# DonsetPG/graph-physics

Hardware: AMD Instinct MI355X
Metric: training steps/sec, CylinderFlow 15-round MGN (batch 16 meshes per step) (higher is better)
Workload: dtype f32; 1 GPU; BASELINE.json configs[1], fp32: 16 x 1885-node CylinderFlow-like meshes per GPU (N=30160, E=180082), 15 rounds, latent 128, random init; global_batch_meshes=16, launch=eager, parallelism=single

## Files before the change

### graph-physics_amd/_capi.py

```python
from __future__ import annotations

import ctypes as C
import os
import subprocess
import threading

_HERE = os.path.dirname(os.path.abspath(__file__))
_CSRC = os.path.join(_HERE, "csrc")
_REPO = os.path.dirname(_HERE)
LIB_PATH = os.environ.get("MGN_LIB") or os.path.join(_CSRC, "libmgn_hip.so")
SOURCES = [os.path.join(_CSRC, "mgn_kernels.hip"), os.path.join(_CSRC, "mgn_prep.hip"), os.path.join(_CSRC, "mgn_attn.hip"),
           os.path.join(_CSRC, "mgn_dense.hip"), os.path.join(_CSRC, "mgn_loss.hip")]
DEPS = [os.path.join(_CSRC, "mgn_x6.inc"), os.path.join(_CSRC, "mgn_fused.inc"), os.path.join(_CSRC, "mgn_pp.inc"), os.path.join(_CSRC, "mgn_ppr.inc")]
HEADER = os.path.join(_REPO, "include", "mgn_hip.h")
DEVICE_FLAGS = ["-Xclang", "-target-feature", "-Xclang", "-packed-fp32-ops"]

MAX_LAYERS = 8
MAX_PHASES = 3
MAX_WGRAD_JOBS = 48

_f32p = C.c_void_p
_i32p = C.c_void_p


class MlpFwdArgs(C.Structure):
    _fields_ = [
        ("M", C.c_int64),
        ("H", C.c_int), ("NL", C.c_int), ("nphase", C.c_int),
        ("src", _f32p * MAX_PHASES),
        ("idx", _i32p * MAX_PHASES),
        ("kw", C.c_int * MAX_PHASES),
        ("W", _f32p * MAX_LAYERS),
        ("b", _f32p * MAX_LAYERS),
        ("scale", _f32p),
        ("eps", C.c_float),
        ("out_w", C.c_int),
        ("resid", _f32p),
        ("out", _f32p),
        ("y_out", _f32p),
        ("saveH", _f32p * MAX_LAYERS),
        ("saveU", _f32p),
        ("saveR", _f32p),
        ("ldw0", C.c_int), ("n_add", C.c_int),
        ("add_src", _f32p * 2), ("add_idx", _i32p * 2),
        ("n_post", C.c_int), ("post_ldw", C.c_int),
        ("post_W", _f32p * 2), ("post_out", _f32p * 2),
        ("wpk", C.c_void_p * 8),
        ("saveM", C.c_void_p * MAX_LAYERS),
        ("precision", C.c_int),
        ("out_relu", C.c_int),
        ("seg_key", C.c_void_p), ("seg_rowptr", C.c_void_p), ("seg_out", _f32p), ("seg_part", _f32p),
        ("act", C.c_int),
        ("saveZ", _f32p * MAX_LAYERS),
        ("add_rows", C.c_int64 * 2),
    ]


class MlpBwdArgs(C.Structure):
    _fields_ = [
        ("M", C.c_int64),
        ("H", C.c_int), ("NL", C.c_int),
        ("dOut", _f32p),
        ("dOut2", _f32p),
        ("idx2", _i32p),
        ("out_w", C.c_int),
        ("U", _f32p), ("R", _f32p), ("scale", _f32p), ("eps", C.c_float),
        ("Hs", _f32p * MAX_LAYERS),
        ("WT", _f32p * MAX_LAYERS),
        ("dZ", _f32p * MAX_LAYERS),
        ("n_din", C.c_int),
        ("WT0", _f32p * MAX_PHASES),
        ("din_resid", _f32p * MAX_PHASES),
        ("dIn", _f32p * MAX_PHASES),
        ("db", _f32p * MAX_LAYERS),
        ("dscale", _f32p),
        ("red_ws", C.c_void_p), ("red_ws_bytes", C.c_size_t),
        ("wpk", C.c_void_p * 8),
        ("Ms", C.c_void_p * MAX_LAYERS),
        ("precision", C.c_int),
        ("n_front", C.c_int),
        ("front_src", _f32p * MAX_PHASES),
        ("front_resid", _f32p),
        ("front_out", _f32p),
        ("defer_reduce", C.c_int),
        ("act", C.c_int),
        ("Zs", _f32p * MAX_LAYERS),
        ("seg_key", C.c_void_p), ("seg_rowptr", C.c_void_p), ("seg_out", _f32p), ("seg_part", _f32p),
        ("dOut2_rows", C.c_int64),
    ]


class ColredJob(C.Structure):
    _fields_ = [("red_ws", C.c_void_p), ("M", C.c_int64), ("H", C.c_int), ("NL", C.c_int), ("out_w", C.c_int), ("n_din", C.c_int),
                ("db", _f32p * MAX_LAYERS), ("dscale", _f32p)]


class WgradJob(C.Structure):
    _fields_ = [
        ("A", _f32p), ("B", _f32p), ("dW", _f32p),
        ("M", C.c_int64),
        ("lda", C.c_int), ("ldb", C.c_int), ("ldw", C.c_int),
        ("nja", C.c_int), ("nkb", C.c_int), ("kw", C.c_int),
        ("db", _f32p),
    ]


class WpackBlock(C.Structure):
    _fields_ = [("src", _f32p), ("dst", C.c_void_p), ("ld_src", C.c_int), ("transpose", C.c_int)]


WPACK_BYTES = 98304


class SimDesc(C.Structure):
    _fields_ = [
        ("N", C.c_int64), ("E", C.c_int64),
        ("x", _f32p), ("x_w", C.c_int),
        ("y", _f32p), ("y_w", C.c_int),
        ("edge_attr", _f32p), ("edge_w", C.c_int),
        ("feat_start", C.c_int), ("feat_end", C.c_int), ("out_start", C.c_int), ("out_w", C.c_int), ("type_idx", C.c_int),
        ("acc_sum", _f32p * 3), ("acc_sumsq", _f32p * 3), ("acc_count", _f32p * 3), ("num_acc", _f32p * 3),
        ("accumulate", C.c_int * 3),
        ("std_eps", C.c_float),
        ("node_out", _f32p), ("target_out", _f32p), ("edge_out", _f32p),
        ("norm_w", C.c_int * 3),
        ("max_accumulations", C.c_float),
        ("type_err", C.c_void_p),
    ]


class EdgeBwdFusedArgs(C.Structure):
    _fields_ = [
        ("M", C.c_int64), ("dOut", _f32p), ("dAgg", _f32p), ("idx", C.c_void_p), ("U", _f32p), ("R", _f32p), ("scale", _f32p),
        ("eps", C.c_float), ("X", _f32p * 4), ("Ms", C.c_void_p * 3), ("wpk", C.c_void_p * 4), ("dIn", _f32p), ("dZ0", _f32p),
        ("dW", _f32p * 4), ("ldw", C.c_int * 4), ("db", _f32p * 4), ("dscale", _f32p), ("ws", C.c_void_p), ("ws_bytes", C.c_size_t),
        ("precision", C.c_int),
    ]


class LinearArgs(C.Structure):
    _fields_ = [
        ("M", C.c_int64), ("x", _f32p), ("ldx", C.c_int), ("K1", C.c_int), ("x2", _f32p), ("ldx2", C.c_int), ("K2", C.c_int),
        ("x3", _f32p), ("ldx3", C.c_int), ("K3", C.c_int), ("idx", C.c_void_p), ("idx2", C.c_void_p), ("idx3", C.c_void_p),
        ("norm_scale", _f32p), ("eps", C.c_float), ("inv_out", _f32p), ("n_out", _f32p), ("W", _f32p), ("ldw", C.c_int), ("b", _f32p),
        ("W2", _f32p), ("b2", _f32p), ("act", C.c_int), ("N", C.c_int), ("resid", _f32p), ("ldr", C.c_int), ("out", _f32p),
        ("ldo", C.c_int), ("saveZ1", _f32p), ("saveZ2", _f32p), ("precision", C.c_int), ("w_transposed", C.c_int),
        ("gb_z1", _f32p), ("gb_z2", _f32p), ("out2", _f32p), ("norm_scale_outer", _f32p), ("inv_outer_out", _f32p), ("z16", C.c_int), ("x16", C.c_int), ("out16", C.c_int),
    ]


class RownormPhase(C.Structure):
    _fields_ = [("x", _f32p), ("ldx", C.c_int), ("K", C.c_int), ("idx", C.c_void_p), ("dx", _f32p), ("lddx", C.c_int), ("acc", _f32p)]


class OptTensor(C.Structure):
    _fields_ = [("p", _f32p), ("g", _f32p), ("m", _f32p), ("v", _f32p), ("n", C.c_int64)]


class TBlock(C.Structure):
    _fields_ = [("src", _f32p), ("dst", _f32p), ("ld_src", C.c_int), ("ld_dst", C.c_int)]


MAX_LOSS_TERMS = 8


class LossArgs(C.Structure):
    _fields_ = [
        ("N", C.c_int64), ("O", C.c_int), ("F", C.c_int), ("DX", C.c_int), ("method", C.c_int),
        ("net_out", _f32p), ("ld_out", C.c_int), ("target", _f32p), ("ld_tgt", C.c_int),
        ("u_out", _f32p), ("u_tgt", _f32p), ("type", _f32p), ("ldty", C.c_int),
        ("types", C.c_float * 4), ("ntypes", C.c_int),
        ("nterms", C.c_int), ("term_type", C.c_int * MAX_LOSS_TERMS), ("term_weight", C.c_float * MAX_LOSS_TERMS),
        ("rowptr", C.c_void_p), ("col", _i32p), ("coef", _f32p), ("inv", _f32p),
        ("M", C.c_int64), ("K", C.c_int), ("elems", _i32p), ("cv", _f32p), ("nptr", C.c_void_p), ("nent", _i32p),
        ("ge_out", _f32p), ("ge_tgt", _f32p),
        ("g_out", _f32p), ("a_out", _f32p), ("bu_out", _f32p), ("b_out", _f32p), ("part", _f32p),
        ("terms", _f32p), ("total", _f32p), ("invcount", _f32p),
    ]


SYMBOLS = {
    "mgn_version": (C.c_int, []),
    "mgn_last_error": (C.c_char_p, []),
    "mgn_csr_workspace_bytes": (C.c_size_t, [C.c_int64, C.c_int64]),
    "mgn_csr_build": (C.c_int, [C.c_void_p, C.c_int64, C.c_int64, C.c_void_p, C.c_void_p, C.c_void_p, C.c_size_t, C.c_void_p]),
    "mgn_topology_workspace_bytes": (C.c_size_t, [C.c_int64, C.c_int64]),
    "mgn_topology_build": (C.c_int, [C.c_void_p, C.c_void_p, C.c_int64, C.c_int64] + [C.c_void_p] * 6 + [C.POINTER(C.c_int32), C.c_void_p,
                                     C.c_size_t, C.c_void_p]),
    "mgn_topology_build_async": (C.c_int, [C.c_void_p, C.c_void_p, C.c_int64, C.c_int64] + [C.c_void_p] * 6 + [C.c_void_p, C.c_void_p,
                                           C.c_size_t, C.c_void_p]),
    "mgn_segsum": (C.c_int, [C.c_void_p, C.c_void_p, C.c_void_p, C.c_void_p, C.c_int64, C.c_int, C.c_void_p]),
# ... 186 lines not shown
```

### graph-physics_amd/csrc/mgn_kernels.hip

```cpp
#include <hip/hip_runtime.h>
#include <stdint.h>
#include <stdlib.h>
#include <type_traits>
#include "mgn_hip.h"

typedef float f32x4 __attribute__((ext_vector_type(4)));

#define MFMA16(a, b, c) __builtin_amdgcn_mfma_f32_16x16x4f32((a), (b), (c), 0, 0, 0)

typedef __attribute__((address_space(1))) const f32x4 g_cf32x4;
typedef __attribute__((address_space(1))) f32x4 g_f32x4;
typedef __attribute__((address_space(1))) const float g_cfloat;
typedef __attribute__((address_space(1))) float g_float;
#ifdef MGN_EXP_NOLOAD
__device__ __forceinline__ f32x4 ld4(const float* p) { return f32x4{1.f, 2.f, (float)(size_t)p, 0.5f}; }
#else
__device__ __forceinline__ f32x4 ld4(const float* p) { return *(g_cf32x4*)p; }
#endif
#ifdef MGN_EXP_NOSTORE
__device__ __forceinline__ void st4(float* p, f32x4 v) { if (v[0] != v[0]) *(g_f32x4*)p = v; }
#else
__device__ __forceinline__ void st4(float* p, f32x4 v) { *(g_f32x4*)p = v; }
#endif
#ifdef MGN_EXP_NOSTORE
// ... 1631 lines not shown
      }
    if (g == 0) *(f32x4*)(dst + H * H + 4 * c) = cs;
  };
  if (wv > 0) put(red[wv - 1]);
  __syncthreads();
  if (wv == 0) {
#pragma unroll
    for (int w = 0; w < 3; ++w) {
#pragma unroll
      for (int qa = 0; qa < 4; ++qa)
#pragma unroll
        for (int v = 0; v < 4; ++v) {
          const f32x4 o = *(const f32x4*)(red[w] + (16 * g + 4 * v + qa) * H + 4 * c);
#pragma unroll
          for (int qb = 0; qb < 4; ++qb) acc[qa][qb][v] += o[qb];
        }
      cs += *(const f32x4*)(red[w] + H * H + 4 * c);
    }
    float* P = L.partial + (size_t)pidx * (H * H + H);
#pragma unroll
    for (int qa = 0; qa < 4; ++qa)
#pragma unroll
      for (int v = 0; v < 4; ++v) {
        const f32x4 o = {acc[qa][0][v], acc[qa][1][v], acc[qa][2][v], acc[qa][3][v]};
        st4(P + (16 * g + 4 * v + qa) * H + 4 * c, o);
      }
    if (g == 0 && J.db != nullptr) st4(P + H * H + 4 * c, cs);
  }
}


template <int WRED_GROUPS>
__global__ void __launch_bounds__(64 * WRED_GROUPS) k_wgrad_red(const WgradLaunch L) {
  __shared__ float red[WRED_GROUPS][64];
  const int H = L.H;
  const size_t st = (size_t)H * H + H;
  const int j = blockIdx.y;
  const mgn_wgrad_job J = L.job[j];
  const int rows = 16 * J.nja, cols = 16 * J.nkb;
  const int i = blockIdx.x * 64 + (threadIdx.x & 63);
  const int pl = threadIdx.x >> 6;
  const int nwg = L.wg0[j + 1] - L.wg0[j];
  const float* P0 = L.partial + (size_t)L.wg0[j] * st;
  const bool is_w = i < rows * cols;
  const bool is_b = !is_w && i < rows * cols + rows && J.db != nullptr;
  int r = 0, k = 0;
  float s0 = 0.f, s1 = 0.f, s2 = 0.f, s3 = 0.f;
  if (is_w || is_b) {
    const float* P;
    if (is_w) {
      r = i / cols;
      k = i % cols;
      P = P0 + r * H + k;
    } else {
      r = i - rows * cols;
      P = P0 + (size_t)H * H + r;
    }
    int b = pl;
    for (; b + 3 * WRED_GROUPS < nwg; b += 4 * WRED_GROUPS) {
      s0 += P[(size_t)b * st];
      s1 += P[(size_t)(b + WRED_GROUPS) * st];
      s2 += P[(size_t)(b + 2 * WRED_GROUPS) * st];
      s3 += P[(size_t)(b + 3 * WRED_GROUPS) * st];
    }
    if (b < nwg) s0 += P[(size_t)b * st];
    if (b + WRED_GROUPS < nwg) s1 += P[(size_t)(b + WRED_GROUPS) * st];
    if (b + 2 * WRED_GROUPS < nwg) s2 += P[(size_t)(b + 2 * WRED_GROUPS) * st];
  }
  red[pl][threadIdx.x & 63] = (s0 + s1) + (s2 + s3);
  __syncthreads();
  if (pl == 0) {
    float v = 0.f;
#pragma unroll
    for (int q = 0; q < WRED_GROUPS; q += 4)
      v += (red[q][threadIdx.x] + red[q + 1][threadIdx.x]) + (red[q + 2][threadIdx.x] + red[q + 3][threadIdx.x]);
    if (is_w) {
      if (k < J.ldw) J.dW[(size_t)r * J.ldw + k] = v;
    } else if (is_b) {
      J.db[r] = v;
    }
  }
}

template <int HB>
__global__ void __launch_bounds__(256) k_segsum(const float* __restrict__ src, const int32_t* __restrict__ rowptr,
                                                const int32_t* __restrict__ perm, float* __restrict__ out, long N) {
  constexpr int H = 16 * HB;
  constexpr int LPR = H / 4;
  const long node = ((long)blockIdx.x * 256 + threadIdx.x) / LPR;
  const int l = threadIdx.x % LPR;
  if (node >= N) return;
  const int beg = rowptr[node], end = rowptr[node + 1];
  f32x4 s = {0.f, 0.f, 0.f, 0.f};
  const float* base = src + 4 * l;
  for (int k = beg; k < end; k += 8) {
    f32x4 v[8];
#pragma unroll
    for (int u = 0; u < 8; ++u) {
      const int kk = k + u;
      if (kk < end) {
        const long row = perm ? (long)perm[kk] : (long)kk;
        v[u] = ld4(base + row * H);
      } else {
        v[u] = f32x4{0.f, 0.f, 0.f, 0.f};
      }
    }
#pragma unroll
    for (int u = 0; u < 8; ++u)
      if (k + u < end) s += v[u];
  }
  st4(out + node * H + 4 * l, s);
}

template <int HB, bool SRC16 = false>
__global__ void __launch_bounds__(256) k_segsum2(const float* __restrict__ src, const int32_t* __restrict__ rowptr0,
                                                 const int32_t* __restrict__ perm0, float* __restrict__ out0,
                                                 const int32_t* __restrict__ rowptr1, const int32_t* __restrict__ perm1,
                                                 float* __restrict__ out1, long N, unsigned half) {
  constexpr int H = 16 * HB;
  constexpr int LPR = H / 4;
  const bool second = blockIdx.x >= half;
  const int32_t* rowptr = second ? rowptr1 : rowptr0;
  const int32_t* perm = second ? perm1 : perm0;
  float* out = second ? out1 : out0;
  const long node = ((long)(blockIdx.x - (second ? half : 0)) * 256 + threadIdx.x) / LPR;
  const int l = threadIdx.x % LPR;
  if (node >= N) return;
  const int beg = rowptr[node], end = rowptr[node + 1];
  f32x4 s = {0.f, 0.f, 0.f, 0.f};
  const float* base = src + 4 * l;
  for (int k = beg; k < end; k += 8) {
    f32x4 v[8];
#pragma unroll
    for (int u = 0; u < 8; ++u) {
      const int kk = k + u;
      if (kk < end) {
        const long row = perm ? (long)perm[kk] : (long)kk;
        if constexpr (SRC16) {
          const uint2 t = *(const uint2*)((const uint16_t*)src + row * H + 32 * (l >> 3) + 8 * (l & 3) + 4 * ((l >> 2) & 1));
          v[u] = f32x4{__builtin_bit_cast(float, t.x << 16), __builtin_bit_cast(float, t.x & 0xffff0000u),
                       __builtin_bit_cast(float, t.y << 16), __builtin_bit_cast(float, t.y & 0xffff0000u)};
        } else {
          v[u] = ld4(base + row * H);
        }
      } else {
        v[u] = f32x4{0.f, 0.f, 0.f, 0.f};
      }
    }
#pragma unroll
    for (int u = 0; u < 8; ++u)
      if (k + u < end) s += v[u];
  }
  st4(out + node * H + 4 * l, s);
}

__global__ void __launch_bounds__(256) k_seg_fix(const int32_t* __restrict__ rowptr, const float* __restrict__ part,
                                                 float* __restrict__ out, long N) {
  constexpr int H = 128, LPR = 32;
  const long node = ((long)blockIdx.x * 256 + threadIdx.x) / LPR;
  const int l = threadIdx.x % LPR;
  if (node >= N) return;
  const int b = rowptr[node], e = rowptr[node + 1];
  f32x4 s = {0.f, 0.f, 0.f, 0.f};
  if (b < e) {
    const int t0 = b >> 4, t1 = (e - 1) >> 4;
    if (t0 == t1) return;
// ... 55 lines not shown
    if (i < N) rowptr[i] = carry + woff + x - v;
    __syncthreads();
    if (tid == 1023) carry_s = carry + woff + x;
    __syncthreads();
  }
  if (tid == 0) rowptr[N] = carry_s;
}

__global__ void k_csr_fill(const int64_t* __restrict__ key, long E, long N, const int32_t* __restrict__ rowptr,
                           int* __restrict__ cursor, int32_t* __restrict__ perm) {
  const long e = (long)blockIdx.x * blockDim.x + threadIdx.x;
  if (e >= E) return;
  const int64_t k = key[e];
  if (k < 0 || k >= N) return;
  const int pos = atomicAdd(&cursor[k], 1);
  perm[rowptr[k] + pos] = (int32_t)e;
}

#define CSR_SMALL_SEG 48
__global__ void k_csr_sortseg(const int32_t* __restrict__ rowptr, long N, int32_t* __restrict__ perm,
                              int* __restrict__ worklist, int* __restrict__ nbig) {
  const long i = (long)blockIdx.x * blockDim.x + threadIdx.x;
  if (i >= N) return;
  const int beg = rowptr[i], end = rowptr[i + 1];
  if (end - beg > CSR_SMALL_SEG) {
    worklist[atomicAdd(nbig, 1)] = (int)i;
    return;
  }
  for (int a = beg + 1; a < end; ++a) {
    const int v = perm[a];
    int b = a - 1;
    while (b >= beg && perm[b] > v) {
      perm[b + 1] = perm[b];
      --b;
    }
    perm[b + 1] = v;
  }
}

__global__ void __launch_bounds__(256) k_csr_sortbig(const int32_t* __restrict__ rowptr, int32_t* __restrict__ perm,
                                                     const int* __restrict__ worklist, const int* __restrict__ nbig,
                                                     int32_t* __restrict__ tmp) {
  const int n = *nbig;
  for (int w = blockIdx.x; w < n; w += gridDim.x) {
    const int node = worklist[w];
    const int beg = rowptr[node], d = rowptr[node + 1] - beg;
    for (int i = threadIdx.x; i < d; i += 256) tmp[beg + i] = perm[beg + i];
    __syncthreads();
    for (int i = threadIdx.x; i < d; i += 256) {
      const int v = tmp[beg + i];
      int rank = 0;
      for (int j = 0; j < d; ++j) rank += (tmp[beg + j] < v) ? 1 : 0;
      perm[beg + rank] = v;
    }
    __syncthreads();
  }
}

static thread_local char g_err[256] = "";
static int fail(int code, const char* msg) {
  snprintf(g_err, sizeof(g_err), "%s", msg);
  return code;
}
static int check_launch(const char* what) {
  hipError_t e = hipGetLastError();
  if (e != hipSuccess) {
    snprintf(g_err, sizeof(g_err), "%s: %s", what, hipGetErrorString(e));
    return 2;
  }
  return 0;
}
static int pick_mt(int64_t M) {
  if (M >= (int64_t)64 * 2048) return 2;
  return 1;
}

struct MlpPlan {
  bool lds;
  int mt;
  unsigned grid;
  size_t smem;
};

static bool fwd_ragged(const mgn_mlp_fwd_args& a) {
  bool r = (a.out_w != a.H);
  for (int p = 0; p < a.nphase; ++p) r = r || (a.kw[p] != a.H);
  return r;
}

static MlpPlan plan_mlp(int64_t M, int H, int NL, bool ragged, bool bwd, int act = MGN_ACT_RELU) {
  MlpPlan p;
  p.lds = (H == 128) && !ragged && NL >= (bwd ? 2 : 1) && NL <= LDS_MAX_NL;
  if (getenv("MGN_NO_LDS") != nullptr) p.lds = false;
  if (act == MGN_ACT_GELU) p.lds = false;
  p.mt = (M >= (int64_t)64 * 2048) ? 2 : 1;
  if (p.lds) p.mt = 1;
  if (const char* e = getenv("MGN_MT")) p.mt = (atoi(e) == 2) ? 2 : 1;
  const int rows = 64 * p.mt;
  p.grid = (unsigned)((M + rows - 1) / rows);
  if (p.lds && p.grid > 512) p.grid = 512;
  if (const char* e = getenv("MGN_GRID")) { if (p.lds && !bwd && atoi(e) > 0 && (unsigned)atoi(e) < p.grid) p.grid = (unsigned)atoi(e); }
  p.smem = p.lds ? (bwd ? (size_t)2 * WBUF_BYTES + 512 + (size_t)4 * (NL + 1) * H * sizeof(float) : (size_t)FWD_LDS_BYTES) : 0;
  return p;
}

template <typename K>
static int set_smem(K kern, size_t bytes) {
  static thread_local const void* done[16];
  static thread_local int ndone = 0;
  for (int i = 0; i < ndone; ++i)
    if (done[i] == (const void*)kern) return 0;
  if (hipFuncSetAttribute((const void*)kern, hipFuncAttributeMaxDynamicSharedMemorySize, (int)(2 * WBUF_BYTES + 4 * 7 * 128 * 4)) != hipSuccess) return 1;
  (void)bytes;
  if (ndone < 16) done[ndone++] = (const void*)kern;
  return 0;
}

static bool fwd_x6(const mgn_mlp_fwd_args& a) {
  if (a.wpk[0] == nullptr || getenv("MGN_FP32_MFMA") != nullptr) return false;
  const int G = a.nphase + a.NL - 1 + a.n_post;
  if (G > X6_MAX_UNITS || a.NL > LDS_MAX_NL) return false;
  if (a.n_add > 0 && (a.nphase != 1 || (a.NL == 1 && a.resid != nullptr))) return false;
  if (a.seg_out != nullptr && (a.seg_key == nullptr || a.seg_rowptr == nullptr || a.seg_part == nullptr || a.n_post > 0)) return false;
  for (int u = 0; u < G; ++u)
    if (a.wpk[u] == nullptr) return false;
  return true;
}
template <int TERMS, int NW, int ACT, class SH = ShDyn>
static int set_fwd_x6_attr() {
  return hipFuncSetAttribute((const void*)k_mlp_fwd_x6<TERMS, NW, ACT, SH>, hipFuncAttributeMaxDynamicSharedMemorySize, X6_FWD_LDS_BYTES(NW)) != hipSuccess;
}
static int fwd_static_shape(const mgn_mlp_fwd_args& a) {
  const char* env = getenv("MGN_X6_STATIC");
  const int mode = env != nullptr ? atoi(env) : 1;
  if (mode == 0 || a.act != MGN_ACT_RELU || a.NL != 4 || a.resid == nullptr || a.scale == nullptr) return 0;
  if (a.nphase == 1 && a.n_add == 2 && a.n_post == 0 && a.idx[0] == nullptr && a.add_idx[0] != nullptr && a.add_idx[1] != nullptr &&
      a.seg_out != nullptr && a.seg_key == a.add_idx[0])
    return 1;
  if (mode != 2 && a.nphase == 2 && a.n_add == 0 && a.idx[0] == nullptr && a.idx[1] == nullptr && a.seg_out == nullptr && a.M >= 4 * 512 * 64) {
    if (a.n_post == 2) return 2;
    if (a.n_post == 0) return 3;
  }
  return 0;
}

static bool fwd_pp_ok(const mgn_mlp_fwd_args& a) {
  const char* env = getenv("MGN_PP");
  const int mode = (env == nullptr) ? -1 : atoi(env);
  if (mode == 0) return false;
  const int64_t min_rows = (mode == 2) ? 1 : 2 * 128 * 256;
  if (a.precision != 0 || a.y_out != nullptr || a.M < min_rows || a.M * 512 >= (int64_t)1 << 32) return false;
  for (int u = 1; u < 4; ++u)
    if ((const char*)a.wpk[u] != (const char*)a.wpk[0] + (size_t)u * MGN_WPACK_BYTES) return false;
  const bool all = a.saveU && a.saveR && a.saveH[0] && a.saveH[1] && a.saveH[2] && a.saveM[0] && a.saveM[1] && a.saveM[2];
  const bool none = !a.saveU && !a.saveR && !a.saveH[0] && !a.saveH[1] && !a.saveH[2] && !a.saveM[0] && !a.saveM[1] && !a.saveM[2];
  if (mode < 0 && !none) return false;
  return (all || none) && a.resid != nullptr && a.scale != nullptr && a.out != a.resid && a.out != a.src[0];
}

static bool fwd_ppr_ok(const mgn_mlp_fwd_args& a) {
  const char* env = getenv("MGN_PPR");
  const int mode = (env == nullptr) ? 1 : atoi(env);
  if (mode == 0) return false;
  const int64_t min_rows = (mode == 2) ? 1 : 65536;
  if (a.precision != 0 || a.y_out != nullptr || a.M < min_rows || a.M * 512 >= (int64_t)1 << 32) return false;
  for (int q = 0; q < 2; ++q)
    if (a.add_rows[q] <= 0 || a.add_rows[q] * 512 >= (int64_t)1 << 32) return false;
  for (int u = 1; u < 4; ++u)
    if ((const char*)a.wpk[u] != (const char*)a.wpk[0] + (size_t)u * MGN_WPACK_BYTES) return false;
  const bool all = a.saveU && a.saveR && a.saveH[0] && a.saveH[1] && a.saveH[2] && a.saveM[0] && a.saveM[1] && a.saveM[2];
  const bool none = !a.saveU && !a.saveR && !a.saveH[0] && !a.saveH[1] && !a.saveH[2] && !a.saveM[0] && !a.saveM[1] && !a.saveM[2];
  return (all || none) && a.resid != nullptr && a.scale != nullptr && a.out != a.resid && a.out != a.src[0];
}

template <int HB>
static int launch_fwd(const mgn_mlp_fwd_args& a, hipStream_t s) {
  const bool ragged = fwd_ragged(a);
  const MlpPlan p = plan_mlp(a.M, a.H, a.NL, ragged, false, a.act);
  if (p.lds && fwd_x6(a)) {
    int nw = (a.M >= 128 * 256) ? X6_FWD_NW_LARGE : 4;
    bool nw6 = false;
    if (const char* e = getenv("MGN_NW")) {
      nw = (atoi(e) == 8) ? 8 : 4;
      nw6 = atoi(e) == 6;
    }
    if (a.seg_out != nullptr) nw = 4;
    const bool silu = (a.act == MGN_ACT_SILU);
    if (silu) nw = 4;
    static thread_local bool attr_done = false;
    if (!attr_done) {
      if (set_fwd_x6_attr<6, 4, 0>() || set_fwd_x6_attr<1, 4, 0>() || set_fwd_x6_attr<6, 8, 0>() || set_fwd_x6_attr<1, 8, 0>() ||
          set_fwd_x6_attr<6, 4, 1>() || set_fwd_x6_attr<1, 4, 1>() || set_fwd_x6_attr<6, 4, 0, ShEdge>() ||
          set_fwd_x6_attr<6, 4, 0, ShNode<2>>() || set_fwd_x6_attr<6, 4, 0, ShNode<0>>() || set_fwd_x6_attr<1, 4, 0, ShEdge>() ||
          set_fwd_x6_attr<1, 4, 0, ShNode<2>>() || set_fwd_x6_attr<1, 4, 0, ShNode<0>>() || set_fwd_x6_attr<6, 6, 0, ShEdge>())
        return 1;
      attr_done = true;
    }
    const int rows = 16 * nw;
    unsigned grid = (unsigned)((a.M + rows - 1) / rows);
    const unsigned cap = (nw == 8) ? 256u : 512u;
    if (grid > cap) grid = cap;
    if (const char* e = getenv("MGN_GRID")) {
      if (atoi(e) > 0 && (unsigned)atoi(e) < grid) grid = (unsigned)atoi(e);
    }
    const int shape = (nw == 4 && !silu) ? fwd_static_shape(a) : 0;
    if (shape == 1 && !nw6 && fwd_ppr_ok(a)) {
      static thread_local bool ppr_attr = false;
      if (!ppr_attr) {
        if (hipFuncSetAttribute((const void*)k_edge_fwd_ppr<true, true>, hipFuncAttributeMaxDynamicSharedMemorySize, PPR_LDS_BYTES) != hipSuccess ||
            hipFuncSetAttribute((const void*)k_edge_fwd_ppr<false, true>, hipFuncAttributeMaxDynamicSharedMemorySize, PPR_LDS_BYTES) != hipSuccess ||
            hipFuncSetAttribute((const void*)k_edge_fwd_ppr<true, false>, hipFuncAttributeMaxDynamicSharedMemorySize, PPR_LDS_BYTES) != hipSuccess ||
            hipFuncSetAttribute((const void*)k_edge_fwd_ppr<false, false>, hipFuncAttributeMaxDynamicSharedMemorySize, PPR_LDS_BYTES) != hipSuccess)
          return 1;
        ppr_attr = true;
      }
      const int64_t ngroups = ((a.M + 15) / 16 + PPR_R - 1) / PPR_R;
      unsigned gp = (ngroups < 256) ? (unsigned)ngroups : 256u;
      const char* ex = getenv("MGN_PPR_XCD");
      const bool xcd = ex == nullptr || atoi(ex) != 0;
      if (a.saveU != nullptr) {
        if (xcd) hipLaunchKernelGGL((k_edge_fwd_ppr<true, true>), dim3(gp), dim3(512), PPR_LDS_BYTES, s, a);
        else hipLaunchKernelGGL((k_edge_fwd_ppr<true, false>), dim3(gp), dim3(512), PPR_LDS_BYTES, s, a);
      } else {
        if (xcd) hipLaunchKernelGGL((k_edge_fwd_ppr<false, true>), dim3(gp), dim3(512), PPR_LDS_BYTES, s, a);
        else hipLaunchKernelGGL((k_edge_fwd_ppr<false, false>), dim3(gp), dim3(512), PPR_LDS_BYTES, s, a);
      }
      return 0;
    }
    if (shape == 1 && !nw6 && fwd_pp_ok(a)) {
      static thread_local bool pp_attr = false;
      if (!pp_attr) {
        if (hipFuncSetAttribute((const void*)k_edge_fwd_pp<true>, hipFuncAttributeMaxDynamicSharedMemorySize, PP_LDS_BYTES) != hipSuccess ||
            hipFuncSetAttribute((const void*)k_edge_fwd_pp<false>, hipFuncAttributeMaxDynamicSharedMemorySize, PP_LDS_BYTES) != hipSuccess)
          return 1;
        pp_attr = true;
      }
      unsigned gp = (unsigned)((a.M + 127) / 128);
      if (gp > 256u) gp = 256u;
      if (a.saveU != nullptr)
        hipLaunchKernelGGL((k_edge_fwd_pp<true>), dim3(gp), dim3(512), PP_LDS_BYTES, s, a);
      else
        hipLaunchKernelGGL((k_edge_fwd_pp<false>), dim3(gp), dim3(512), PP_LDS_BYTES, s, a);
      return 0;
    }
    if (shape == 1 && nw6 && a.precision == 0) {
      unsigned g6 = (unsigned)((a.M + 95) / 96);
      if (g6 > 512u) g6 = 512u;
      hipLaunchKernelGGL((k_mlp_fwd_x6<6, 6, 0, ShEdge>), dim3(g6), dim3(384), X6_FWD_LDS_BYTES(6), s, a);
    } else if (shape == 1) {
      if (a.precision >= 1)
        hipLaunchKernelGGL((k_mlp_fwd_x6<1, 4, 0, ShEdge>), dim3(grid), dim3(256), X6_FWD_LDS_BYTES(4), s, a);
      else
        hipLaunchKernelGGL((k_mlp_fwd_x6<6, 4, 0, ShEdge>), dim3(grid), dim3(256), X6_FWD_LDS_BYTES(4), s, a);
    } else if (shape == 2) {
      if (a.precision >= 1)
        hipLaunchKernelGGL((k_mlp_fwd_x6<1, 4, 0, ShNode<2>>), dim3(grid), dim3(256), X6_FWD_LDS_BYTES(4), s, a);
      else
        hipLaunchKernelGGL((k_mlp_fwd_x6<6, 4, 0, ShNode<2>>), dim3(grid), dim3(256), X6_FWD_LDS_BYTES(4), s, a);
    } else if (shape == 3) {
      if (a.precision >= 1)
        hipLaunchKernelGGL((k_mlp_fwd_x6<1, 4, 0, ShNode<0>>), dim3(grid), dim3(256), X6_FWD_LDS_BYTES(4), s, a);
      else
        hipLaunchKernelGGL((k_mlp_fwd_x6<6, 4, 0, ShNode<0>>), dim3(grid), dim3(256), X6_FWD_LDS_BYTES(4), s, a);
    } else if (silu) {
      if (a.precision >= 1)
        hipLaunchKernelGGL((k_mlp_fwd_x6<1, 4, 1>), dim3(grid), dim3(256), X6_FWD_LDS_BYTES(4), s, a);
      else
        hipLaunchKernelGGL((k_mlp_fwd_x6<6, 4, 1>), dim3(grid), dim3(256), X6_FWD_LDS_BYTES(4), s, a);
    } else if (nw == 8) {
      if (a.precision >= 1)
        hipLaunchKernelGGL((k_mlp_fwd_x6<1, 8, 0>), dim3(grid), dim3(512), X6_FWD_LDS_BYTES(8), s, a);
      else
        hipLaunchKernelGGL((k_mlp_fwd_x6<6, 8, 0>), dim3(grid), dim3(512), X6_FWD_LDS_BYTES(8), s, a);
    } else {
      if (a.precision >= 1)
        hipLaunchKernelGGL((k_mlp_fwd_x6<1, 4, 0>), dim3(grid), dim3(256), X6_FWD_LDS_BYTES(4), s, a);
      else
        hipLaunchKernelGGL((k_mlp_fwd_x6<6, 4, 0>), dim3(grid), dim3(256), X6_FWD_LDS_BYTES(4), s, a);
    }
    return 0;
  }
  if (p.lds) {
    if (p.mt == 2) {
      if (set_smem(k_mlp_fwd_lds<2>, p.smem)) return 1;
      hipLaunchKernelGGL((k_mlp_fwd_lds<2>), dim3(p.grid), dim3(256), p.smem, s, a);
    } else {
      if (set_smem(k_mlp_fwd_lds<1>, p.smem)) return 1;
      hipLaunchKernelGGL((k_mlp_fwd_lds<1>), dim3(p.grid), dim3(256), p.smem, s, a);
    }
    return 0;
  }
  if (ragged) {
    if (p.mt == 2)
      hipLaunchKernelGGL((k_mlp_fwd<HB, 2, true>), dim3(p.grid), dim3(256), 0, s, a);
    else
      hipLaunchKernelGGL((k_mlp_fwd<HB, 1, true>), dim3(p.grid), dim3(256), 0, s, a);
  } else {
    if (p.mt == 2)
      hipLaunchKernelGGL((k_mlp_fwd<HB, 2, false>), dim3(p.grid), dim3(256), 0, s, a);
    else
      hipLaunchKernelGGL((k_mlp_fwd<HB, 1, false>), dim3(p.grid), dim3(256), 0, s, a);
  }
  return 0;
}

static bool bwd_x6(const mgn_mlp_bwd_args& a) {
  if (a.wpk[0] == nullptr || getenv("MGN_FP32_MFMA") != nullptr) return false;
  const int G = a.n_front + a.NL - 1 + a.n_din;
  if (G > 8 || G < 1 || a.n_front < 0 || a.n_front > MGN_MAX_PHASES) return false;
  if (a.n_front > 0 && a.dOut2 != nullptr) return false;
  for (int u = 0; u < G; ++u)
    if (a.wpk[u] == nullptr) return false;
  if (a.seg_out != nullptr && (a.seg_key == nullptr || a.seg_rowptr == nullptr || a.seg_part == nullptr || a.dZ[0] == nullptr ||
                               a.n_front > 0 || a.act != MGN_ACT_RELU || a.precision != 0 || a.NL < 2))
    return false;
  if (a.act == MGN_ACT_SILU) {
    if (a.n_front > 0 || (a.n_din == 0 && a.dOut2 != nullptr)) return false;
    for (int l = 1; l < a.NL; ++l)
      if (a.Zs[l - 1] == nullptr) return false;
    return true;
  }
  for (int l = 1; l < a.NL; ++l)
    if (a.Ms[l - 1] == nullptr) return false;
  return true;
}

static bool bwd_ppr_ok(const mgn_mlp_bwd_args& a) {
  const char* env = getenv("MGN_PPR");
  const int mode = (env == nullptr) ? 1 : atoi(env);
  const char* eb = getenv("MGN_PPR_BWD");
  if (mode == 0 || (eb != nullptr && atoi(eb) == 0)) return false;
  const int64_t min_rows = (mode == 2) ? 1 : 65536;
  if (a.precision != 0 || a.M < min_rows || a.M * 512 >= (int64_t)1 << 32 || a.dscale == nullptr) return false;
  if (a.dOut2_rows <= 0 || a.dOut2_rows * 512 >= (int64_t)1 << 32) return false;
  for (int u = 1; u < 4; ++u)
    if ((const char*)a.wpk[u] != (const char*)a.wpk[0] + (size_t)u * MGN_WPACK_BYTES) return false;
  for (int l = 0; l < 4; ++l)
    if (a.db[l] != nullptr || a.dZ[l] == nullptr) return false;
  if (a.dIn[0] == nullptr || a.Ms[0] == nullptr || a.Ms[1] == nullptr || a.Ms[2] == nullptr) return false;
  const void* ins[4] = {a.dOut, a.U, a.din_resid[0], a.dOut2};
  const void* outs[5] = {a.dZ[0], a.dZ[1], a.dZ[2], a.dZ[3], a.dIn[0]};
  for (const void* o : outs)
    for (const void* i : ins)
      if (o == i) return false;
  return true;
}

template <int HB>
static int launch_bwd(const mgn_mlp_bwd_args& a, hipStream_t s) {
  MlpPlan p = plan_mlp(a.M, a.H, a.NL, a.out_w != a.H || a.n_din > 1, true, a.act);
  if (p.lds && bwd_x6(a)) {
    static thread_local bool attr_done = false;
    if (!attr_done) {
      const int lds = X6_BWD_LDS_BYTES(LDS_MAX_NL + 1);
      if (hipFuncSetAttribute((const void*)k_mlp_bwd_x6<6, false, 0>, hipFuncAttributeMaxDynamicSharedMemorySize, lds) != hipSuccess ||
          hipFuncSetAttribute((const void*)k_mlp_bwd_x6<1, false, 0>, hipFuncAttributeMaxDynamicSharedMemorySize, lds) != hipSuccess ||
          hipFuncSetAttribute((const void*)k_mlp_bwd_x6<6, true, 0>, hipFuncAttributeMaxDynamicSharedMemorySize, lds) != hipSuccess ||
          hipFuncSetAttribute((const void*)k_mlp_bwd_x6<1, true, 0>, hipFuncAttributeMaxDynamicSharedMemorySize, lds) != hipSuccess ||
          hipFuncSetAttribute((const void*)k_mlp_bwd_x6<6, false, 1>, hipFuncAttributeMaxDynamicSharedMemorySize, lds) != hipSuccess ||
          hipFuncSetAttribute((const void*)k_mlp_bwd_x6<1, false, 1>, hipFuncAttributeMaxDynamicSharedMemorySize, lds) != hipSuccess ||
          hipFuncSetAttribute((const void*)k_mlp_bwd_x6<6, false, 0, true>, hipFuncAttributeMaxDynamicSharedMemorySize, lds) != hipSuccess ||
          hipFuncSetAttribute((const void*)k_mlp_bwd_x6<6, false, 0, false, SbEdge>, hipFuncAttributeMaxDynamicSharedMemorySize, lds) != hipSuccess ||
          hipFuncSetAttribute((const void*)k_mlp_bwd_x6<1, false, 0, false, SbEdge>, hipFuncAttributeMaxDynamicSharedMemorySize, lds) != hipSuccess)
        return 1;
      attr_done = true;
    }
    int nused = (a.scale != nullptr && a.dscale != nullptr) ? 1 : 0;
    for (int l = 0; l < a.NL; ++l) nused += (a.db[l] != nullptr) ? 1 : 0;
    const size_t lds = X6_BWD_LDS_BYTES(nused);
    const bool front = a.n_front > 0;
    const char* st_env = getenv("MGN_X6_STATIC");
    const bool static_off = st_env != nullptr && atoi(st_env) == 0;
    const bool sb_edge = !static_off && !front && a.seg_out == nullptr && a.act == MGN_ACT_RELU && a.NL == 4 &&
                         a.n_din == 1 && a.din_resid[0] != nullptr && a.scale != nullptr && a.R != nullptr && a.U != nullptr &&
                         a.dOut2 != nullptr && a.idx2 != nullptr;
    if (sb_edge && bwd_ppr_ok(a)) {
      static thread_local bool ppr_attr = false;
      if (!ppr_attr) {
        if (hipFuncSetAttribute((const void*)k_edge_bwd_ppr<true>, hipFuncAttributeMaxDynamicSharedMemorySize, PPB_LDS_BYTES) != hipSuccess ||
            hipFuncSetAttribute((const void*)k_edge_bwd_ppr<false>, hipFuncAttributeMaxDynamicSharedMemorySize, PPB_LDS_BYTES) != hipSuccess)
          return 1;
        ppr_attr = true;
      }
      const int64_t ngroups = ((a.M + 15) / 16 + PPR_R - 1) / PPR_R;
      unsigned gp = (ngroups < 256) ? (unsigned)ngroups : 256u;
      if (gp > p.grid) gp = p.grid;
      const char* ex = getenv("MGN_PPR_XCD");
      if (ex == nullptr || atoi(ex) != 0)
        hipLaunchKernelGGL((k_edge_bwd_ppr<true>), dim3(gp), dim3(512), PPB_LDS_BYTES, s, a, (int)p.grid);
      else
        hipLaunchKernelGGL((k_edge_bwd_ppr<false>), dim3(gp), dim3(512), PPB_LDS_BYTES, s, a, (int)p.grid);
    } else if (sb_edge) {
      if (a.precision >= 1)
        hipLaunchKernelGGL((k_mlp_bwd_x6<1, false, 0, false, SbEdge>), dim3(p.grid), dim3(256), lds, s, a);
      else
        hipLaunchKernelGGL((k_mlp_bwd_x6<6, false, 0, false, SbEdge>), dim3(p.grid), dim3(256), lds, s, a);
    } else if (a.seg_out != nullptr) {
      hipLaunchKernelGGL((k_mlp_bwd_x6<6, false, 0, true>), dim3(p.grid), dim3(256), lds, s, a);
    } else if (a.act == MGN_ACT_SILU) {
      if (a.precision >= 1)
        hipLaunchKernelGGL((k_mlp_bwd_x6<1, false, 1>), dim3(p.grid), dim3(256), lds, s, a);
      else
        hipLaunchKernelGGL((k_mlp_bwd_x6<6, false, 1>), dim3(p.grid), dim3(256), lds, s, a);
    } else if (a.precision >= 1) {
      if (front)
        hipLaunchKernelGGL((k_mlp_bwd_x6<1, true, 0>), dim3(p.grid), dim3(256), lds, s, a);
      else
        hipLaunchKernelGGL((k_mlp_bwd_x6<1, false, 0>), dim3(p.grid), dim3(256), lds, s, a);
    } else {
      if (front)
        hipLaunchKernelGGL((k_mlp_bwd_x6<6, true, 0>), dim3(p.grid), dim3(256), lds, s, a);
      else
        hipLaunchKernelGGL((k_mlp_bwd_x6<6, false, 0>), dim3(p.grid), dim3(256), lds, s, a);
    }
    return 0;
  }
  if (p.lds) {
    if (p.mt == 2) {
      if (set_smem(k_mlp_bwd_lds<2>, p.smem)) return 1;
      hipLaunchKernelGGL((k_mlp_bwd_lds<2>), dim3(p.grid), dim3(256), p.smem, s, a);
    } else {
      if (set_smem(k_mlp_bwd_lds<1>, p.smem)) return 1;
      hipLaunchKernelGGL((k_mlp_bwd_lds<1>), dim3(p.grid), dim3(256), p.smem, s, a);
    }
    return 0;
  }
  if (a.out_w != a.H) {
    if (p.mt == 2)
      hipLaunchKernelGGL((k_mlp_bwd<HB, 2, true>), dim3(p.grid), dim3(256), 0, s, a);
    else
      hipLaunchKernelGGL((k_mlp_bwd<HB, 1, true>), dim3(p.grid), dim3(256), 0, s, a);
  } else {
    if (p.mt == 2)
      hipLaunchKernelGGL((k_mlp_bwd<HB, 2, false>), dim3(p.grid), dim3(256), 0, s, a);
    else
      hipLaunchKernelGGL((k_mlp_bwd<HB, 1, false>), dim3(p.grid), dim3(256), 0, s, a);
  }
  return 0;
}

extern "C" {

int mgn_version(void) { return 136; }
const char* mgn_last_error(void) { return g_err; }

size_t mgn_csr_workspace_bytes(int64_t E, int64_t N) {
  return (size_t)(2 * N + E + 32) * sizeof(int);
}

static int csr_enqueue(const int64_t* key, int64_t E, int64_t N, int32_t* rowptr, int32_t* perm, void* ws, int* err_dev, hipStream_t s) {
  int* cnt = (int*)ws;
  if (hipMemsetAsync(ws, 0, (size_t)(N + 16) * sizeof(int), s) != hipSuccess) return fail(2, "mgn_csr_build: memset");
// ... 167 lines not shown
  return check_launch("mgn_seg_fix");
}

int mgn_segsum2(const float* src, const int32_t* rowptr0, const int32_t* perm0, float* out0, const int32_t* rowptr1,
                const int32_t* perm1, float* out1, int64_t N, int H, void* stream) {
  hipStream_t s = (hipStream_t)stream;
  if (N == 0) return 0;
  if (H != 128) return fail(1, "mgn_segsum2: H must be 128");
  const unsigned half = (unsigned)((N * (H / 4) + 255) / 256);
  hipLaunchKernelGGL(k_segsum2<8>, dim3(2 * half), dim3(256), 0, s, src, rowptr0, perm0, out0, rowptr1, perm1, out1, (long)N, half);
  return check_launch("mgn_segsum2");
}

int mgn_segsum2_b16(const uint16_t* src, const int32_t* rowptr0, const int32_t* perm0, float* out0, const int32_t* rowptr1,
                    const int32_t* perm1, float* out1, int64_t N, int H, void* stream) {
  hipStream_t s = (hipStream_t)stream;
  if (N == 0) return 0;
  if (H != 128) return fail(1, "mgn_segsum2_b16: H must be 128");
  const unsigned half = (unsigned)((N * (H / 4) + 255) / 256);
  hipLaunchKernelGGL((k_segsum2<8, true>), dim3(2 * half), dim3(256), 0, s, (const float*)src, rowptr0, perm0, out0, rowptr1, perm1, out1,
                     (long)N, half);
  return check_launch("mgn_segsum2_b16");
}

static int check_mlp_common(int H, int NL, int out_w, const char* who) {
  if (!(H == 16 || H == 32 || H == 64 || H == 128)) return fail(1, "H must be 16, 32, 64 or 128");
  if (NL < 1 || NL > MGN_MAX_LAYERS) return fail(1, "NL out of range");
  if (out_w < 1 || out_w > H) return fail(1, "out_w out of range");
  (void)who;
  return 0;
}


int mgn_mlp_fwd(const mgn_mlp_fwd_args* args, void* stream) {
  const mgn_mlp_fwd_args& a = *args;
  if (int rc = check_mlp_common(a.H, a.NL, a.out_w, "mgn_mlp_fwd")) return rc;
  if (a.precision < 0 || a.precision > 2) return fail(1, "mgn_mlp_fwd: precision must be 0 (fp32-grade), 1 (bf16) or 2 (bf16, two-byte saves)");
  if (a.precision == 2 && (!fwd_x6(a) || !plan_mlp(a.M, a.H, a.NL, fwd_ragged(a), false, a.act).lds || a.act != MGN_ACT_RELU))
    return fail(1, "mgn_mlp_fwd: precision 2 (two-byte saves) needs the packed split-bf16 path (H = 128, wpk[]) and ReLU");
  if (a.seg_out != nullptr && !(plan_mlp(a.M, a.H, a.NL, fwd_ragged(a), false).lds && fwd_x6(a)))
    return fail(1, "mgn_mlp_fwd: the fused segment sum needs the packed split-bf16 path (and seg_key / seg_rowptr / seg_part, no post-products)");
  if (a.out_relu && (a.scale != nullptr || a.resid != nullptr || a.wpk[0] != nullptr ||
                     plan_mlp(a.M, a.H, a.NL, fwd_ragged(a), false).lds))
    return fail(1, "mgn_mlp_fwd: out_relu is for a plain ragged-input launch (no norm / residual / packed path)");
  if (a.act != MGN_ACT_RELU && a.act != MGN_ACT_SILU && a.act != MGN_ACT_GELU) return fail(1, "mgn_mlp_fwd: act must be MGN_ACT_RELU, _SILU or _GELU");
  if (a.act == MGN_ACT_GELU && (a.wpk[0] != nullptr || a.precision != 0 || a.seg_out != nullptr || a.n_add > 0 || a.n_post > 0 || a.ldw0 > 0))
    return fail(1, "mgn_mlp_fwd: GELU runs on the generic kernels only (no packed weights / gathers / post-products)");
  if (a.act == MGN_ACT_SILU && plan_mlp(a.M, a.H, a.NL, fwd_ragged(a), false).lds && !fwd_x6(a) && a.NL > 1)
    return fail(1, "mgn_mlp_fwd: SiLU is not available on the exact-fp32 LDS generation (pass packed weights)");
  if (a.precision >= 1 && plan_mlp(a.M, a.H, a.NL, fwd_ragged(a), false, a.act).lds && !fwd_x6(a))
    return fail(1, "mgn_mlp_fwd: at H = 128 with full widths the bf16 matrix mode needs the packed split-bf16 path (wpk); other shapes run it on the generic kernels");
  if (a.nphase < 1 || a.nphase > MGN_MAX_PHASES) return fail(1, "mgn_mlp_fwd: nphase out of range");
  for (int p = 0; p < a.nphase; ++p)
    if (a.kw[p] < 1 || a.kw[p] > a.H) return fail(1, "mgn_mlp_fwd: phase width out of range");
  if (a.scale != nullptr && a.out_w != a.H) return fail(1, "mgn_mlp_fwd: RMSNorm needs out_w == H");
  if (a.n_add < 0 || a.n_add > 2 || a.n_post < 0 || a.n_post > 2) return fail(1, "mgn_mlp_fwd: n_add / n_post out of range");
  if ((a.n_add > 0 || a.n_post > 0 || a.ldw0 > 0) && !plan_mlp(a.M, a.H, a.NL, fwd_ragged(a), false).lds)
    return fail(1, "mgn_mlp_fwd: ldw0 / n_add / n_post need the H = 128 full-width kernel");
  if (a.M == 0) return 0;
  hipStream_t s = (hipStream_t)stream;
  int rc;
  switch (a.H) {
    case 128: rc = launch_fwd<8>(a, s); break;
    case 64: rc = launch_fwd<4>(a, s); break;
    case 32: rc = launch_fwd<2>(a, s); break;
    default: rc = launch_fwd<1>(a, s); break;
  }
  if (rc) return fail(2, "mgn_mlp_fwd: cannot reserve LDS");
  return check_launch("mgn_mlp_fwd");
}


size_t mgn_mlp_bwd_workspace_bytes(int64_t M, int H, int NL) {
  return (size_t)((M + 63) / 64 + 1) * (NL + 1) * H * sizeof(float);
}


int mgn_mlp_bwd(const mgn_mlp_bwd_args* args, void* stream) {
  const mgn_mlp_bwd_args& a = *args;
  if (int rc = check_mlp_common(a.H, a.NL, a.out_w, "mgn_mlp_bwd")) return rc;
  if (a.n_din < 0 || a.n_din > MGN_MAX_PHASES) return fail(1, "mgn_mlp_bwd: n_din out of range");
  if (a.n_din > 1 && a.dZ[0] == nullptr) return fail(1, "mgn_mlp_bwd: n_din > 1 needs dZ[0]");
  if (a.precision < 0 || a.precision > 3) return fail(1, "mgn_mlp_bwd: precision must be 0 (fp32-grade), 1 (bf16), 2 (bf16, two-byte dZ[1..]) or 3 (dZ[0] too)");
  if (a.precision >= 2 && (!bwd_x6(a) || !plan_mlp(a.M, a.H, a.NL, a.out_w != a.H || a.n_din > 1, true).lds || a.act != MGN_ACT_RELU || a.n_front != 0))
    return fail(1, "mgn_mlp_bwd: precision 2 (two-byte dZ rows) needs the packed split-bf16 path (H = 128, wpk, Ms), ReLU and no front stage");
  if (a.act != MGN_ACT_RELU && a.act != MGN_ACT_SILU && a.act != MGN_ACT_GELU) return fail(1, "mgn_mlp_bwd: act must be MGN_ACT_RELU, _SILU or _GELU");
  if (a.act == MGN_ACT_GELU && (a.wpk[0] != nullptr || a.precision != 0 || a.seg_out != nullptr || a.n_front != 0))
    return fail(1, "mgn_mlp_bwd: GELU runs on the generic kernels only");
  if (a.act != MGN_ACT_RELU) {
    for (int l = 1; l < a.NL; ++l)
      if (a.Zs[l - 1] == nullptr) return fail(1, "mgn_mlp_bwd: SiLU / GELU need the saved pre-activations Zs[]");
  }
  if (a.act == MGN_ACT_SILU) {
    if (plan_mlp(a.M, a.H, a.NL, a.out_w != a.H || a.n_din > 1, true).lds && !bwd_x6(a))
      return fail(1, "mgn_mlp_bwd: SiLU is not available on the exact-fp32 LDS generation (pass packed weights)");
  }
  if (a.n_front != 0 && !(plan_mlp(a.M, a.H, a.NL, a.out_w != a.H || a.n_din > 1, true).lds && bwd_x6(a)))
    return fail(1, "mgn_mlp_bwd: the front stage needs the packed split-bf16 path (H = 128, full widths, wpk, Ms, no dOut2)");
  if (a.precision >= 1 && plan_mlp(a.M, a.H, a.NL, a.out_w != a.H || a.n_din > 1, true, a.act).lds && !bwd_x6(a))
    return fail(1, "mgn_mlp_bwd: at H = 128 with full widths the bf16 matrix mode needs the packed split-bf16 path (wpk, Ms); other shapes run it on the generic kernels");
  if (a.seg_out != nullptr && !(plan_mlp(a.M, a.H, a.NL, a.out_w != a.H || a.n_din > 1, true).lds && bwd_x6(a)))
    return fail(1, "mgn_mlp_bwd: the fused segment sum of dZ[0] needs the packed split-bf16 path (fp32-grade, ReLU, dZ[0], no front stage)");
  if (a.M == 0) return 0;
  if (a.red_ws_bytes < mgn_mlp_bwd_workspace_bytes(a.M, a.H, a.NL)) return fail(1, "mgn_mlp_bwd: workspace too small");
  hipStream_t s = (hipStream_t)stream;
  int lrc;
  switch (a.H) {
    case 128: lrc = launch_bwd<8>(a, s); break;
    case 64: lrc = launch_bwd<4>(a, s); break;
    case 32: lrc = launch_bwd<2>(a, s); break;
    default: lrc = launch_bwd<1>(a, s); break;
  }
  if (lrc) return fail(2, "mgn_mlp_bwd: cannot reserve LDS");
  if (int rc = check_launch("mgn_mlp_bwd")) return rc;
  const unsigned grid = plan_mlp(a.M, a.H, a.NL, a.out_w != a.H || a.n_din > 1, true, a.act).grid;
  const int nslot = a.NL + 1;
  ColredOuts outs;
  bool any = false;
  for (int l = 0; l <= MGN_MAX_LAYERS; ++l) outs.o[l] = nullptr;
  for (int l = 0; l < a.NL; ++l) {
    outs.o[l] = a.db[l];
    any |= a.db[l] != nullptr;
  }
  outs.o[a.NL] = (a.scale != nullptr) ? a.dscale : nullptr;
  any |= outs.o[a.NL] != nullptr;
  if (!any || a.defer_reduce) return 0;
  const int n = nslot * a.H;
  hipLaunchKernelGGL(k_colred, dim3((n + 31) / 32), dim3(1024), 0, s, (const float*)a.red_ws, (int)grid, nslot, a.H, outs);
  return check_launch("mgn_mlp_bwd/colred");
}

int mgn_colred_batch(int n, const mgn_colred_job* jobs, void* stream) {
  if (n < 0) return fail(1, "mgn_colred_batch: bad arguments");
  hipStream_t s = (hipStream_t)stream;
  for (int i0 = 0; i0 < n; i0 += CR_MAX) {
    ColredBatch B;
    const int m = (n - i0 < CR_MAX) ? n - i0 : CR_MAX;
    int maxcol = 0;
    for (int i = 0; i < m; ++i) {
      const mgn_colred_job& q = jobs[i0 + i];
      if (q.red_ws == nullptr || q.NL < 1 || q.NL > MGN_MAX_LAYERS) return fail(1, "mgn_colred_batch: bad job");
      ColredJob& J = B.j[i];
      J.ws = (const float*)q.red_ws;
      J.nblocks = (int)plan_mlp(q.M, q.H, q.NL, q.out_w != q.H || q.n_din > 1, true).grid;
      J.nslot = q.NL + 1;
      J.H = q.H;
      for (int l = 0; l <= MGN_MAX_LAYERS; ++l) J.outs.o[l] = nullptr;
      for (int l = 0; l < q.NL; ++l) J.outs.o[l] = q.db[l];
      J.outs.o[q.NL] = q.dscale;
      if (J.nslot * J.H > maxcol) maxcol = J.nslot * J.H;
    }
    hipLaunchKernelGGL(k_colred_batch, dim3((maxcol + 31) / 32, m), dim3(1024), 0, s, B);
  }
  return check_launch("mgn_colred_batch");
}

static bool wgrad_job_row64(const mgn_wgrad_job& j) {
  return j.nja <= 4 && j.nkb <= 4 && j.kw <= 64 && (j.kw & 3) == 0 && (j.lda & 3) == 0 && (j.ldb & 3) == 0 &&
         (((uintptr_t)j.A | (uintptr_t)j.B) & 15) == 0;
}
static int wgrad_plan(int njobs, const mgn_wgrad_job* jobs, int* wg0, bool lds, int lds_budget = 512) {
  const int rows = lds ? WG_TILE_ROWS : 16;
  int budget = lds ? lds_budget : 512;
  if (!lds) {
    if (const char* e = getenv("MGN_WGRAD_GENERIC_BUDGET")) {
      const int b = atoi(e);
      if (b >= 64 && b <= 1024) budget = b;
    }
  }
  int64_t tiles[MGN_MAX_WGRAD_JOBS], tot = 0;
  int n[MGN_MAX_WGRAD_JOBS];
  for (int j = 0; j < njobs; ++j) {
    tiles[j] = (jobs[j].M + rows - 1) / rows;
    if (tiles[j] < 1) tiles[j] = 1;
    tot += tiles[j];
  }
  int used = 0;
  for (int j = 0; j < njobs; ++j) {
    int64_t s = tiles[j] * budget / tot;
    const int64_t cap = (tiles[j] + 3) / 4;
    if (s > cap) s = cap;
    if (s < 1) s = 1;
    n[j] = (int)s;
    used += n[j];
  }
  while (used < budget) {
    int best = -1;
    double load = 4.0;
    for (int j = 0; j < njobs; ++j) {
      const double l = (double)tiles[j] / n[j];
      if (l > load) {
        load = l;
        best = j;
      }
    }
    if (best < 0) break;
    ++n[best];
    ++used;
  }
  int acc = 0;
  for (int j = 0; j < njobs; ++j) {
    wg0[j] = acc;
    acc += n[j];
  }
  wg0[njobs] = acc;
  return acc;
}

size_t mgn_wgrad_workspace_bytes(int njobs, const mgn_wgrad_job* jobs) {
  if (njobs < 1 || njobs > MGN_MAX_WGRAD_JOBS) return 0;
  return (size_t)(512 + 1024 + 2 * MGN_MAX_WGRAD_JOBS) * (128 * 128 + 128) * sizeof(float);
}

static bool wgrad_job_full(const mgn_wgrad_job& j) {
  return j.nja == 8 && j.nkb == 8 && (j.lda == 128 || j.lda == -128) && (j.ldb == 128 || j.ldb == -128) && j.kw == 128 && j.M >= 1 && getenv("MGN_NO_LDS") == nullptr;
}

int mgn_wgrad(int njobs, const mgn_wgrad_job* jobs, void* ws, size_t ws_bytes, void* stream) {
  return mgn_wgrad_p(njobs, jobs, ws, ws_bytes, 0, stream);
}

int mgn_wgrad_p(int njobs, const mgn_wgrad_job* jobs, void* ws, size_t ws_bytes, int precision, void* stream) {
  if (precision != 0 && precision != 1) return fail(1, "mgn_wgrad: precision must be 0 (fp32-grade) or 1 (bf16)");
  if (njobs < 1 || njobs > MGN_MAX_WGRAD_JOBS) return fail(1, "mgn_wgrad: njobs out of range");
  for (int j = 0; j < njobs; ++j) {
    if (jobs[j].lda < 0 || jobs[j].ldb < 0) {
      const bool r64 = !wgrad_job_full(jobs[j]) && wgrad_job_row64(jobs[j]) && getenv("MGN_WGRAD_NO_ROW64") == nullptr &&
                       ((((uintptr_t)jobs[j].A | (uintptr_t)jobs[j].B) & 15) == 0);
      if (precision != 1 || !(wgrad_job_full(jobs[j]) || r64) || getenv("MGN_FP32_MFMA") != nullptr)
        return fail(1, "mgn_wgrad: a negative leading dimension (bf16 rows) needs precision 1 and a full 128 x 128 job with ld = -128 or a job of the row-vector kernel");
    }
  }
  hipStream_t s = (hipStream_t)stream;
  size_t ws_off = 0;
  for (int pass = 0; pass < 2; ++pass) {
    WgradLaunch L;
    L.njobs = 0;
    int maxb = 1;
    for (int j = 0; j < njobs; ++j) {
      if (jobs[j].nja < 1 || jobs[j].nkb < 1 || jobs[j].nja > 8 || jobs[j].nkb > 8) return fail(1, "mgn_wgrad: block counts out of range");
      if (wgrad_job_full(jobs[j]) != (pass == 0)) continue;
      L.job[L.njobs++] = jobs[j];
      if (jobs[j].nja > maxb) maxb = jobs[j].nja;
      if (jobs[j].nkb > maxb) maxb = jobs[j].nkb;
    }
    if (L.njobs == 0) continue;
    int HB = maxb <= 1 ? 1 : maxb <= 2 ? 2 : maxb <= 4 ? 4 : 8;
    bool row64 = pass == 1 && HB <= 4 && getenv("MGN_WGRAD_NO_ROW64") == nullptr;
    for (int j = 0; row64 && j < L.njobs; ++j) row64 = wgrad_job_row64(L.job[j]);
    if (row64) HB = 4;
    if (!row64 && pass == 1)
      for (int j = 0; j < L.njobs; ++j)
        if (L.job[j].lda < 0 || L.job[j].ldb < 0) return fail(1, "mgn_wgrad: bf16-row jobs below 128 x 128 need every job of the launch on the row-vector kernel");
    L.H = 16 * HB;
    bool pc = pass == 0 && precision == 0 && getenv("MGN_FP32_MFMA") == nullptr;
    if (pc) {
      const char* e = getenv("MGN_WGRAD_PC");
      pc = e == nullptr || atoi(e) != 0;
      for (int j = 0; pc && j < L.njobs; ++j) pc = L.job[j].lda == 128 && L.job[j].ldb == 128;
    }
    int total = wgrad_plan(L.njobs, L.job, L.wg0, pass == 0, pc ? 256 : 512);
    L.interleave = 0;
    if (row64 && L.njobs >= 2 && L.njobs <= 8 && getenv("MGN_WGRAD_NO_INTERLEAVE") == nullptr) {
      bool same = true;
      for (int j = 1; j < L.njobs; ++j) same = same && L.job[j].M == L.job[0].M;
      const int64_t tiles = (L.job[0].M + 15) / 16;
      int per = (512 / L.njobs) & ~7;
      while (per > 8 && (int64_t)per * 4 > tiles) per -= 8;
      if (same && per >= 8 && tiles >= 4 * per) {
        for (int j = 0; j <= L.njobs; ++j) L.wg0[j] = j * per;
        L.interleave = per;
        total = L.njobs * per;
      }
    }
    const size_t need = (size_t)total * (L.H * L.H + L.H) * sizeof(float);
    if (ws_bytes < ws_off + need) return fail(1, "mgn_wgrad: workspace too small");
    L.partial = (float*)((char*)ws + ws_off);
    ws_off += need;
    if (pc) {
      static thread_local bool attr_pc_done = false;
      if (!attr_pc_done) {
        if (hipFuncSetAttribute((const void*)k_wgrad_pc, hipFuncAttributeMaxDynamicSharedMemorySize, WPC_LDS_BYTES) != hipSuccess)
          return fail(2, "mgn_wgrad: cannot reserve LDS");
        attr_pc_done = true;
      }
      hipLaunchKernelGGL(k_wgrad_pc, dim3(total), dim3(512), WPC_LDS_BYTES, s, L);
    } else if (pass == 0) {
      const size_t smem = 4 * WG_TILE_BYTES;
      static thread_local bool attr_done = false;
      if (!attr_done) {
        if (hipFuncSetAttribute((const void*)k_wgrad_lds, hipFuncAttributeMaxDynamicSharedMemorySize, (int)smem) != hipSuccess)
          return fail(2, "mgn_wgrad: cannot reserve LDS");
        attr_done = true;
      }
      if (getenv("MGN_FP32_MFMA") == nullptr) {
        static thread_local bool attr6_done = false;
        if (!attr6_done) {
          if (hipFuncSetAttribute((const void*)k_wgrad_x6<6>, hipFuncAttributeMaxDynamicSharedMemorySize, (int)smem) != hipSuccess ||
              hipFuncSetAttribute((const void*)k_wgrad_x6<1>, hipFuncAttributeMaxDynamicSharedMemorySize, (int)smem) != hipSuccess)
            return fail(2, "mgn_wgrad: cannot reserve LDS");
          attr6_done = true;
        }
        if (precision == 1)
          hipLaunchKernelGGL(k_wgrad_x6<1>, dim3(total), dim3(256), smem, s, L);
        else
          hipLaunchKernelGGL(k_wgrad_x6<6>, dim3(total), dim3(256), smem, s, L);
      } else {
        hipLaunchKernelGGL(k_wgrad_lds, dim3(total), dim3(256), smem, s, L);
      }
    } else if (row64) {
      if (precision == 1) {
        const bool a16 = L.job[0].lda < 0, b16 = L.job[0].ldb < 0;
        for (int j = 1; j < L.njobs; ++j)
          if ((L.job[j].lda < 0) != a16 || (L.job[j].ldb < 0) != b16) return fail(1, "mgn_wgrad: the jobs of a row-vector launch must agree on which operand is bf16 rows");
        if (a16 && b16) hipLaunchKernelGGL((k_wgrad_row64<true, true, true>), dim3(total), dim3(256), 0, s, L);
        else if (a16) hipLaunchKernelGGL((k_wgrad_row64<true, true, false>), dim3(total), dim3(256), 0, s, L);
        else if (b16) hipLaunchKernelGGL((k_wgrad_row64<true, false, true>), dim3(total), dim3(256), 0, s, L);
        else hipLaunchKernelGGL((k_wgrad_row64<true>), dim3(total), dim3(256), 0, s, L);
      }
      else if (getenv("MGN_FP32_MFMA") == nullptr && getenv("MGN_WGRAD_ROW64_EXACT") == nullptr) {
        bool full = true;
        for (int j = 0; full && j < L.njobs; ++j) full = L.job[j].nja == 4 && L.job[j].kw == 64;
        if (full)
          hipLaunchKernelGGL(k_wgrad_row64x6<true>, dim3(total), dim3(256), 0, s, L);
        else
          hipLaunchKernelGGL(k_wgrad_row64x6<false>, dim3(total), dim3(256), 0, s, L);
      }
      else
        hipLaunchKernelGGL(k_wgrad_row64<false>, dim3(total), dim3(256), 0, s, L);
    } else {
      switch (HB) {
        case 8: hipLaunchKernelGGL(k_wgrad<8>, dim3(total), dim3(256), 0, s, L); break;
        case 4: hipLaunchKernelGGL(k_wgrad<4>, dim3(total), dim3(256), 0, s, L); break;
        case 2: hipLaunchKernelGGL(k_wgrad<2>, dim3(total), dim3(256), 0, s, L); break;
        default: hipLaunchKernelGGL(k_wgrad<1>, dim3(total), dim3(256), 0, s, L); break;
      }
    }
    if (int rc = check_launch("mgn_wgrad")) return rc;
    int max_nwg = 0;
    for (int j = 0; j < L.njobs; ++j) max_nwg = (L.wg0[j + 1] - L.wg0[j] > max_nwg) ? L.wg0[j + 1] - L.wg0[j] : max_nwg;
    if (max_nwg <= 64)
      hipLaunchKernelGGL(k_wgrad_red<4>, dim3((L.H * L.H + L.H + 63) / 64, L.njobs), dim3(64 * 4), 0, s, L);
    else
      hipLaunchKernelGGL(k_wgrad_red<16>, dim3((L.H * L.H + L.H + 63) / 64, L.njobs), dim3(64 * 16), 0, s, L);
    if (int rc = check_launch("mgn_wgrad/reduce")) return rc;
  }
  return 0;
}

int mgn_debug_occupancy(int* out) {
  int n = 0;
  if (hipFuncSetAttribute((const void*)k_mlp_fwd_x6<6, 4, 0>, hipFuncAttributeMaxDynamicSharedMemorySize, X6_FWD_LDS_BYTES(4)) != hipSuccess) return 1;
  if (hipFuncSetAttribute((const void*)k_mlp_fwd_x6<1, 4, 0>, hipFuncAttributeMaxDynamicSharedMemorySize, X6_FWD_LDS_BYTES(4)) != hipSuccess) return 1;
  if (hipFuncSetAttribute((const void*)k_mlp_fwd_x6<6, 8, 0>, hipFuncAttributeMaxDynamicSharedMemorySize, X6_FWD_LDS_BYTES(8)) != hipSuccess) return 1;
  if (hipFuncSetAttribute((const void*)k_mlp_bwd_x6<6, false, 0>, hipFuncAttributeMaxDynamicSharedMemorySize, X6_BWD_LDS_BYTES(LDS_MAX_NL + 1)) != hipSuccess) return 1;
  if (hipFuncSetAttribute((const void*)k_mlp_bwd_x6<1, false, 0>, hipFuncAttributeMaxDynamicSharedMemorySize, X6_BWD_LDS_BYTES(LDS_MAX_NL + 1)) != hipSuccess) return 1;
  if (hipFuncSetAttribute((const void*)k_wgrad_x6<6>, hipFuncAttributeMaxDynamicSharedMemorySize, 4 * WG_TILE_BYTES) != hipSuccess) return 1;
  if (hipOccupancyMaxActiveBlocksPerMultiprocessor(&n, k_mlp_fwd_x6<6, 4, 0>, 256, X6_FWD_LDS_BYTES(4)) != hipSuccess) return 2;
  out[0] = n;
  if (hipOccupancyMaxActiveBlocksPerMultiprocessor(&n, k_mlp_fwd_x6<1, 4, 0>, 256, X6_FWD_LDS_BYTES(4)) != hipSuccess) return 2;
  out[1] = n;
  if (hipOccupancyMaxActiveBlocksPerMultiprocessor(&n, k_mlp_bwd_x6<6, false, 0>, 256, X6_BWD_LDS_BYTES(1)) != hipSuccess) return 2;
  out[2] = n;
  if (hipOccupancyMaxActiveBlocksPerMultiprocessor(&n, k_mlp_bwd_x6<6, false, 0>, 256, X6_BWD_LDS_BYTES(5)) != hipSuccess) return 2;
  out[3] = n;
  if (hipOccupancyMaxActiveBlocksPerMultiprocessor(&n, k_wgrad_x6<6>, 256, 4 * WG_TILE_BYTES) != hipSuccess) return 2;
  out[4] = n;
  if (hipOccupancyMaxActiveBlocksPerMultiprocessor(&n, k_mlp_fwd_x6<6, 8, 0>, 512, X6_FWD_LDS_BYTES(8)) != hipSuccess) return 2;
  out[5] = n;
  return 0;
}

int mgn_wpack(int n, const mgn_wpack_block* blocks, void* stream) {
  if (n < 0) return fail(1, "mgn_wpack: bad arguments");
  hipStream_t s = (hipStream_t)stream;
  for (int i0 = 0; i0 < n; i0 += TB_MAX) {
    WpackLaunch T;
    const int m = (n - i0 < TB_MAX) ? n - i0 : TB_MAX;
    for (int i = 0; i < m; ++i) {
      T.b[i] = blocks[i0 + i];
      if (T.b[i].src == nullptr || T.b[i].dst == nullptr || ((size_t)T.b[i].dst & 15) != 0) return fail(1, "mgn_wpack: null / misaligned block");
    }
    hipLaunchKernelGGL(k_wpack, dim3(8, m), dim3(256), 0, s, T);
  }
  return check_launch("mgn_wpack");
}

int mgn_transpose_blocks(int n, const mgn_tblock* blocks, int H, void* stream) {
  if (n < 0 || H < 1 || H > 128) return fail(1, "mgn_transpose_blocks: bad arguments");
  hipStream_t s = (hipStream_t)stream;
  const int tiles = ((H + 31) / 32) * ((H + 31) / 32);
  for (int i0 = 0; i0 < n; i0 += TB_MAX) {
    TBlocks T;
    const int m = (n - i0 < TB_MAX) ? n - i0 : TB_MAX;
    for (int i = 0; i < m; ++i) T.b[i] = blocks[i0 + i];
    hipLaunchKernelGGL(k_transpose_blocks, dim3(tiles, m), dim3(256), 0, s, T, H);
  }
  return check_launch("mgn_transpose_blocks");
}

}
```

### graph-physics_amd/csrc/mgn_x6.inc

```

typedef unsigned u32;
typedef u32 u32x4 __attribute__((ext_vector_type(4)));
typedef u32 u32x2 __attribute__((ext_vector_type(2)));
typedef __bf16 bf16x8 __attribute__((ext_vector_type(8)));
typedef __attribute__((address_space(3))) const u32x4 lds_cu32x4;

#define X6_QBYTES 24576
#define X6_RING 3
#define X6_FWD_LDS_BYTES(NW) (((NW) == 8 ? 6 : 3) * X6_QBYTES + 5 * 512)
#define X6_MAX_UNITS 8
#ifndef MGN_GQ_DB
#define MGN_GQ_DB 0
#endif
#ifndef X6_FWD_NW_LARGE
#define X6_FWD_NW_LARGE 4
#endif

#define MFMA_BF(a, b, c) \
  __builtin_amdgcn_mfma_f32_16x16x32_bf16(__builtin_bit_cast(bf16x8, (a)), __builtin_bit_cast(bf16x8, (b)), (c), 0, 0, 0)

typedef float f32x2 __attribute__((ext_vector_type(2)));
typedef __bf16 bf16x2 __attribute__((ext_vector_type(2)));
__device__ __forceinline__ u32 pk_bf16(float a, float b) {
  const f32x2 v = {a, b};
// ... 27 lines not shown
  for (int d = 0; d < 4; ++d) {
    u32 w0 = 0, w1 = 0;
#pragma unroll
    for (int h = 0; h < 2; ++h) {
      const int i = 2 * d + h;
      const int f = 16 * (i >> 2) + 4 * g + (i & 3);
      if (f == c) w0 |= m1 << (16 * h);
      if (f == c + 16) w1 |= m1 << (16 * h);
    }
    S.s0[d] = w0, S.s1[d] = w1;
  }
  return S;
}
__device__ __forceinline__ void split_pair_mfma(const f32x4& b0, const f32x4& b1, u32x4 (&x)[3], const SplitSel& S) {
  x[0][0] = pk_bf16(b0[0], b0[1]), x[0][1] = pk_bf16(b0[2], b0[3]);
  x[0][2] = pk_bf16(b1[0], b1[1]), x[0][3] = pk_bf16(b1[2], b1[3]);
  const f32x4 r0 = MFMA_BF(S.s0, x[0], b0), r1 = MFMA_BF(S.s1, x[0], b1);
  x[1][0] = pk_bf16(r0[0], r0[1]), x[1][1] = pk_bf16(r0[2], r0[3]);
  x[1][2] = pk_bf16(r1[0], r1[1]), x[1][3] = pk_bf16(r1[2], r1[3]);
  const f32x4 t0 = MFMA_BF(S.s0, x[1], r0), t1 = MFMA_BF(S.s1, x[1], r1);
  x[2][0] = pk_bf16(t0[0], t0[1]), x[2][1] = pk_bf16(t0[2], t0[3]);
  x[2][2] = pk_bf16(t1[0], t1[1]), x[2][3] = pk_bf16(t1[2], t1[3]);
}

template <int TERMS, bool MF = true>
__device__ __forceinline__ void split_tile(const f32x4 (&v)[8], u32x4 (&xs)[4][3]) {
#if MGN_SPLIT_MFMA
  if (TERMS != 1 && MF) {
    const SplitSel S = split_sel();
#pragma unroll
    for (int j = 0; j < 4; ++j) split_pair_mfma(v[2 * j], v[2 * j + 1], xs[j], S);
    return;
  }
#endif
  u32 q1[16], q2[16], q3[16];
  float ra[16], rb[16];
#pragma unroll
  for (int i = 0; i < 16; ++i) q1[i] = pk_bf16(v[i >> 1][2 * (i & 1)], v[i >> 1][2 * (i & 1) + 1]);
  if (TERMS == 1) {
#pragma unroll
    for (int j = 0; j < 4; ++j)
#pragma unroll
      for (int d = 0; d < 4; ++d) xs[j][0][d] = q1[4 * j + d];
    return;
  }
#pragma unroll
  for (int i = 0; i < 16; ++i) {
    ra[i] = v[i >> 1][2 * (i & 1)] - bf_lo(q1[i]);
    rb[i] = v[i >> 1][2 * (i & 1) + 1] - bf_hi(q1[i]);
  }
#pragma unroll
  for (int i = 0; i < 16; ++i) q2[i] = pk_bf16(ra[i], rb[i]);
#pragma unroll
  for (int i = 0; i < 16; ++i) {
    ra[i] -= bf_lo(q2[i]);
    rb[i] -= bf_hi(q2[i]);
  }
#pragma unroll
  for (int i = 0; i < 16; ++i) q3[i] = pk_bf16(ra[i], rb[i]);
#pragma unroll
  for (int j = 0; j < 4; ++j)
#pragma unroll
    for (int d = 0; d < 4; ++d) {
      xs[j][0][d] = q1[4 * j + d];
      xs[j][1][d] = q2[4 * j + d];
      xs[j][2][d] = q3[4 * j + d];
    }
}

struct WpackLaunch {
  mgn_wpack_block b[TB_MAX];
};
__global__ void __launch_bounds__(256) k_wpack(const WpackLaunch T) {
  const mgn_wpack_block B = T.b[blockIdx.y];
  const int t = blockIdx.x * 256 + threadIdx.x;
  const int lane = t & 63, ob = (t >> 6) & 7, j = t >> 9;
  const int c = lane & 15, g = lane >> 4;
  const int o = 16 * ob + c;
  float v[8];
#pragma unroll
  for (int i = 0; i < 8; ++i) {
    const int f = 32 * j + 16 * (i >> 2) + 4 * g + (i & 3);
    v[i] = B.transpose ? B.src[(size_t)f * B.ld_src + o] : B.src[(size_t)o * B.ld_src + f];
  }
  u32x4 p1, p2, p3;
#pragma unroll
  for (int h = 0; h < 4; ++h) {
    u32 q1, q2, q3;
    split2(v[2 * h], v[2 * h + 1], q1, q2, q3);
    p1[h] = q1, p2[h] = q2, p3[h] = q3;
  }
  u32x4* dst = (u32x4*)((char*)B.dst + (size_t)j * X6_QBYTES) + ob * 64 + lane;
  dst[0] = p1;
  dst[512] = p2;
  dst[1024] = p3;
}

struct DmaQ {
  const char* su;
  unsigned lds;
  bool on;
};
__device__ __forceinline__ void glds16c(const char* sbase, unsigned voff, unsigned lds_addr) {
  glds16((const float*)sbase, voff, lds_addr);
}
__device__ __forceinline__ void dmaq_issue(const DmaQ& j, int i, unsigned lane16) {
  if (j.on) glds16c(j.su + i * 1024, lane16, j.lds + i * 1024);
}
template <int PAIR>
__device__ __forceinline__ void dmaq_issue2(const DmaQ& j, unsigned lane16) {
  if (!j.on) return;
  constexpr int BASE = (PAIR == 2) ? 4096 : 0;
  constexpr int O0 = (PAIR == 1) ? 2048 : 0, O1 = O0 + 1024;
  unsigned keep;
  asm volatile(
      "s_nop 4\n\t"
      "s_mov_b32 %0, m0\n\t"
      "s_mov_b32 m0, %3\n\t"
      "s_nop 0\n\t"
      "global_load_lds_dwordx4 %1, %2 offset:%4\n\t"
      "global_load_lds_dwordx4 %1, %2 offset:%5\n\t"
      "s_mov_b32 m0, %0"
      : "=&s"(keep)
      : "v"(lane16), "s"((const float*)(j.su + BASE)), "s"(j.lds + BASE), "n"(O0), "n"(O1)
      : "memory");
}

template <int TERMS, int PPW, typename Late>
__device__ __forceinline__ void gemm_q(f32x4 (&acc)[8], const u32x4 (&x)[3], lds_char* wq, unsigned lane16, const DmaQ& job, Late late) {
  if (TERMS == 1) {
    u32x4 w1[2][2];
    lds_char* wl = wq + lane16;
#pragma unroll
    for (int q = 0; q < 2; ++q) w1[0][q] = *(lds_cu32x4*)(wl + q * 1024);
#pragma unroll
    for (int s = 0; s < 4; ++s) {
      if (s + 1 < 4) {
#pragma unroll
        for (int q = 0; q < 2; ++q) w1[(s + 1) & 1][q] = *(lds_cu32x4*)(wl + (2 * (s + 1) + q) * 1024);
      }
#ifndef X6_B16_DMA_AT0
#define X6_B16_DMA_AT0 1
#endif
      if (X6_B16_DMA_AT0 && PPW != 6) {
        if (s == 0) {
#pragma unroll
          for (int i = 0; i < PPW; ++i) dmaq_issue(job, i, lane16);
        }
      } else if (s < 3) {
        if (PPW == 6) {
          if (s == 0) dmaq_issue2<0>(job, lane16);
          else if (s == 1) dmaq_issue2<1>(job, lane16);
          else dmaq_issue2<2>(job, lane16);
        } else {
#pragma unroll
          for (int i = s * PPW / 3; i < (s + 1) * PPW / 3; ++i) dmaq_issue(job, i, lane16);
        }
      }
      late(s);
      __builtin_amdgcn_sched_barrier(0);
#pragma unroll
      for (int q = 0; q < 2; ++q) acc[2 * s + q] = MFMA_BF(w1[s & 1][q], x[0], acc[2 * s + q]);
      __builtin_amdgcn_sched_barrier(0);
    }
    return;
  }
// ... 113 lines not shown
__device__ __forceinline__ void drain_allow(int n) {
#ifdef MGN_EXP_NODRAIN
  (void)n;
  return;
#endif
  if (n >= 38)
    dma_drain_counted<38>();
  else if (n >= 30)
    dma_drain_counted<30>();
  else if (n >= 22)
    dma_drain_counted<22>();
  else if (n >= 14)
    dma_drain_counted<14>();
  else if (n >= 6)
    dma_drain_counted<6>();
  else
    dma_drain();
}

struct QStream {
  long issued;
  long total;
  int du, dq;
  int dslot;
  int cslot;
  int young;
};

template <int S>
__device__ __forceinline__ void ld2u_at(f32x4& d0, f32x4& d1, const float* rowp) {
  asm volatile("global_load_dwordx4 %0, %2, off offset:%3\n\t"
               "global_load_dwordx4 %1, %2, off offset:%4"
               : "=&v"(d0), "=&v"(d1)
               : "v"(rowp), "n"(128 * S), "n"(128 * S + 64)
               : "memory");
}
__device__ __forceinline__ void ld2u(f32x4 (&dst)[8], const float* rowp, int s, int& n) {
  if (s == 0) ld2u_at<0>(dst[0], dst[1], rowp);
  else if (s == 1) ld2u_at<1>(dst[2], dst[3], rowp);
  else if (s == 2) ld2u_at<2>(dst[4], dst[5], rowp);
  else ld2u_at<3>(dst[6], dst[7], rowp);
  n += 2;
}
template <int B0, int NB>
__device__ __forceinline__ void ldnu_at(f32x4& d0, f32x4& d1, f32x4& d2, const float* rowp) {
  if (NB == 3)
    asm volatile("global_load_dwordx4 %0, %3, off offset:%4\n\t"
                 "global_load_dwordx4 %1, %3, off offset:%5\n\t"
                 "global_load_dwordx4 %2, %3, off offset:%6"
                 : "=&v"(d0), "=&v"(d1), "=&v"(d2)
                 : "v"(rowp), "n"(64 * B0), "n"(64 * B0 + 64), "n"(64 * B0 + 128)
                 : "memory");
  else
    asm volatile("global_load_dwordx4 %0, %2, off offset:%3\n\t"
                 "global_load_dwordx4 %1, %2, off offset:%4"
                 : "=&v"(d0), "=&v"(d1)
                 : "v"(rowp), "n"(64 * B0), "n"(64 * B0 + 64)
                 : "memory");
}
__device__ __forceinline__ void ld3u(f32x4 (&dst)[8], const float* rowp, int s, int& n) {
  if (s == 0) {
    ldnu_at<0, 3>(dst[0], dst[1], dst[2], rowp);
    n += 3;
  } else if (s == 1) {
    ldnu_at<3, 3>(dst[3], dst[4], dst[5], rowp);
    n += 3;
  } else if (s == 2) {
    ldnu_at<6, 2>(dst[6], dst[7], dst[7], rowp);
    n += 2;
  }
}
__device__ __forceinline__ int ldiu(const int32_t* p) {
  int v;
  asm volatile("global_load_dword %0, %1, off" : "=v"(v) : "v"(p) : "memory");
  return v;
}
__device__ __forceinline__ int landed(int v) {
  asm volatile("" : "+v"(v));
  return v;
}

struct ShDyn {
  static constexpr bool ST = false;
  static __device__ __forceinline__ int nphase(const mgn_mlp_fwd_args& a) { return a.nphase; }
  static __device__ __forceinline__ int NL(const mgn_mlp_fwd_args& a) { return a.NL; }
  static __device__ __forceinline__ int n_add(const mgn_mlp_fwd_args& a) { return a.n_add; }
  static __device__ __forceinline__ int n_post(const mgn_mlp_fwd_args& a) { return a.n_post; }
  static __device__ __forceinline__ bool resid(const mgn_mlp_fwd_args& a) { return a.resid != nullptr; }
  static __device__ __forceinline__ bool scale(const mgn_mlp_fwd_args& a) { return a.scale != nullptr; }
  static __device__ __forceinline__ bool seg(const mgn_mlp_fwd_args& a) { return a.seg_out != nullptr; }
  static __device__ __forceinline__ bool has_idx(const int32_t* p) { return p != nullptr; }
  static __device__ __forceinline__ bool has_addidx(const int32_t* p) { return p != nullptr; }
};
struct ShEdge {
  static constexpr bool ST = true;
  static __device__ __forceinline__ constexpr int nphase(const mgn_mlp_fwd_args&) { return 1; }
  static __device__ __forceinline__ constexpr int NL(const mgn_mlp_fwd_args&) { return 4; }
  static __device__ __forceinline__ constexpr int n_add(const mgn_mlp_fwd_args&) { return 2; }
  static __device__ __forceinline__ constexpr int n_post(const mgn_mlp_fwd_args&) { return 0; }
  static __device__ __forceinline__ constexpr bool resid(const mgn_mlp_fwd_args&) { return true; }
  static __device__ __forceinline__ constexpr bool scale(const mgn_mlp_fwd_args&) { return true; }
  static __device__ __forceinline__ constexpr bool seg(const mgn_mlp_fwd_args&) { return true; }
  static __device__ __forceinline__ constexpr bool has_idx(const int32_t*) { return false; }
  static __device__ __forceinline__ constexpr bool has_addidx(const int32_t*) { return true; }
};
template <int NPOST>
struct ShNode {
  static constexpr bool ST = true;
  static __device__ __forceinline__ constexpr int nphase(const mgn_mlp_fwd_args&) { return 2; }
  static __device__ __forceinline__ constexpr int NL(const mgn_mlp_fwd_args&) { return 4; }
  static __device__ __forceinline__ constexpr int n_add(const mgn_mlp_fwd_args&) { return 0; }
  static __device__ __forceinline__ constexpr int n_post(const mgn_mlp_fwd_args&) { return NPOST; }
  static __device__ __forceinline__ constexpr bool resid(const mgn_mlp_fwd_args&) { return true; }
  static __device__ __forceinline__ constexpr bool scale(const mgn_mlp_fwd_args&) { return true; }
  static __device__ __forceinline__ constexpr bool seg(const mgn_mlp_fwd_args&) { return false; }
  static __device__ __forceinline__ constexpr bool has_idx(const int32_t*) { return false; }
  static __device__ __forceinline__ constexpr bool has_addidx(const int32_t*) { return false; }
};

__device__ __forceinline__ void ld2(f32x4 (&dst)[8], const float* rowp, int s, int& n) {
  dst[2 * s] = ld4(rowp + 32 * s);
  dst[2 * s + 1] = ld4(rowp + 32 * s + 16);
  n += 2;
}

#ifdef MGN_EXP_PAIR_STAGGER
__device__ int g_pair_stagger = 0;
extern "C" int mgn_debug_set_stagger(int ticks) { return hipMemcpyToSymbol(HIP_SYMBOL(g_pair_stagger), &ticks, sizeof(int)) != hipSuccess; }
#endif
__device__ __forceinline__ void x6_stagger() {
#ifdef MGN_EXP_PAIR_STAGGER
  const int w = g_pair_stagger;
  if (w > 0 && blockIdx.x * 2 >= gridDim.x) {
    const unsigned long long t0 = __builtin_amdgcn_s_memrealtime();
    while (__builtin_amdgcn_s_memrealtime() - t0 < (unsigned long long)w) __builtin_amdgcn_s_sleep(8);
  }
#endif
#ifdef MGN_EXP_STAGGER4
  const unsigned long long wait = (unsigned long long)(blockIdx.x & 3) * MGN_EXP_STAGGER4;
  const unsigned long long t0 = __builtin_readcyclecounter();
  while (__builtin_readcyclecounter() - t0 < wait) __builtin_amdgcn_s_sleep(16);
#endif
}

struct TileWalk {
  long first, end, stride;
  long count;
};
__device__ __forceinline__ TileWalk tile_walk(long ntiles) {
  TileWalk w;
  const unsigned G = gridDim.x, b = blockIdx.x;
#ifdef MGN_XCD_WALK
  if ((G & 7u) == 0 && ntiles >= 64) {
#else
  if (false) {
#endif
    const long C = (ntiles + 7) / 8, x = b & 7u, per = G >> 3;
    const long lo = x * C;
    w.end = (lo + C < ntiles) ? lo + C : ntiles;
    w.first = lo + (b >> 3);
    w.stride = per;
  } else {
    w.first = b, w.end = ntiles, w.stride = G;
  }
  w.count = (w.first < w.end) ? (w.end - w.first + w.stride - 1) / w.stride : 0;
  return w;
}

__device__ __forceinline__ void seg_scan16(f32x4 (&v)[8], int key) {
  constexpr int HB = 8;
#pragma unroll
  for (int st = 0; st < 4; ++st) {
    int kd;
    if (st == 0) kd = __builtin_amdgcn_update_dpp(-2, key, 0x111, 0xf, 0xf, false);
    else if (st == 1) kd = __builtin_amdgcn_update_dpp(-2, key, 0x112, 0xf, 0xf, false);
    else if (st == 2) kd = __builtin_amdgcn_update_dpp(-2, key, 0x114, 0xf, 0xf, false);
    else kd = __builtin_amdgcn_update_dpp(-2, key, 0x118, 0xf, 0xf, false);
    const float same = (kd == key) ? 1.f : 0.f;
#define X6_FMAC_DPP4(N)                                                                                   \
  asm volatile("s_nop 1\n\t"                                                                               \
               "v_fmac_f32_dpp %0, %0, %4 row_shr:" #N " row_mask:0xf bank_mask:0xf bound_ctrl:1\n\t"      \
               "v_fmac_f32_dpp %1, %1, %4 row_shr:" #N " row_mask:0xf bank_mask:0xf bound_ctrl:1\n\t"      \
               "v_fmac_f32_dpp %2, %2, %4 row_shr:" #N " row_mask:0xf bank_mask:0xf bound_ctrl:1\n\t"      \
               "v_fmac_f32_dpp %3, %3, %4 row_shr:" #N " row_mask:0xf bank_mask:0xf bound_ctrl:1"            \
               : "+v"(v0), "+v"(v1), "+v"(v2), "+v"(v3)                                                     \
               : "v"(same))
#pragma unroll
    for (int ib = 0; ib < HB; ++ib) {
      float v0 = v[ib][0], v1 = v[ib][1], v2 = v[ib][2], v3 = v[ib][3];
      if (st == 0) X6_FMAC_DPP4(1);
      else if (st == 1) X6_FMAC_DPP4(2);
      else if (st == 2) X6_FMAC_DPP4(4);
      else X6_FMAC_DPP4(8);
      v[ib][0] = v0, v[ib][1] = v1, v[ib][2] = v2, v[ib][3] = v3;
    }
#undef X6_FMAC_DPP4
  }
}
template <bool PRE = false>
__device__ __forceinline__ void seg_scan_store(f32x4 (&v)[8], int key, long wtile, const int32_t* __restrict__ seg_rowptr,
                                               float* __restrict__ seg_out, float* __restrict__ seg_part, int g,
                                               int kprev = -1, int knext2 = -1) {
  constexpr int HB = 8, H = 128;
  seg_scan16(v, key);
  const int knext = __builtin_amdgcn_update_dpp(-3, key, 0x101, 0xf, 0xf, false);
  const int key0 = __builtin_amdgcn_readfirstlane(key);
  if (key >= 0 && knext != key) {
    const long r0 = wtile * 16;
    bool before, inside;
    if (PRE) {
      before = (key == key0) && (kprev == key0);
      inside = !before && !(knext == -3 && knext2 == key);
    } else {
      const int beg = seg_rowptr[key], end = seg_rowptr[key + 1];
      before = beg < r0;
      inside = beg >= r0 && end <= r0 + 16;
    }
    float* dst;
    if (inside)
      dst = seg_out + (long)key * H;
    else
      dst = seg_part + (wtile * 2 + (before ? 0 : 1)) * H;
#pragma unroll
    for (int ib = 0; ib < HB; ++ib) st4(dst + 4 * g + 16 * ib, v[ib]);
  }
}

template <int TERMS, int NW, int ACT, class SH = ShDyn>
__global__ void __launch_bounds__(64 * NW, (NW == 6 ? 3 : 2)) k_mlp_fwd_x6(const mgn_mlp_fwd_args a) {
  const int NPH = SH::nphase(a), NLL = SH::NL(a), NADD = SH::n_add(a), NPOST = SH::n_post(a);
  const bool HAS_RESID = SH::resid(a), HAS_SCALE = SH::scale(a), HAS_SEG = SH::seg(a);
  constexpr bool UT = SH::ST;
  constexpr bool UI = UT && NW != 6;
  constexpr int RING = (NW == 8) ? 6 : 3;
  constexpr int AHEAD = RING - 1;
  constexpr int PPW = (TERMS == 1) ? 8 / NW : 24 / NW;
  static_assert(24 % NW == 0 && (TERMS != 1 || 8 % NW == 0), "the quarter is shared out in whole 1 KB pieces");
  constexpr int WSHARE = PPW * 1024;
  constexpr int HB = 8, H = 128;
  extern __shared__ __attribute__((aligned(16))) char smem[];
  lds_char* ring = (lds_char*)smem;
  lds_char* cst = ring + RING * X6_QBYTES;
  const int lane = threadIdx.x & 63;
  const int wv = __builtin_amdgcn_readfirstlane(threadIdx.x >> 6);
  const int c = lane & 15, g = lane >> 4;
  const unsigned lane16 = 16u * lane;
  TL_DECL();
  const long ntiles = (a.M + 16 * NW - 1) / (16 * NW);
  const TileWalk tw = tile_walk(ntiles);
  long tile = tw.first;
  if (tw.count == 0) return;
  const long my_tiles = tw.count;
  x6_stagger();
  const int GL = NPH + NLL - 1;
  const int G = GL + NPOST;
  const char *U0 = (const char*)a.wpk[0], *U1 = (const char*)a.wpk[1], *U2 = (const char*)a.wpk[2], *U3 = (const char*)a.wpk[3];
  const char *U4 = (const char*)a.wpk[4], *U5 = (const char*)a.wpk[5], *U6 = (const char*)a.wpk[6], *U7 = (const char*)a.wpk[7];
  const bool contig = x6_contig(U0, U1, U2, U3, U4, U5, U6, U7, G);
  float *sH0 = a.saveH[0], *sH1 = a.saveH[1], *sH2 = a.saveH[2];
  uint32_t *sM0 = a.saveM[0], *sM1 = a.saveM[1], *sM2 = a.saveM[2];
  float *sZ0 = a.saveZ[0], *sZ1 = a.saveZ[1], *sZ2 = a.saveZ[2];
  const float *src0 = a.src[0], *src1 = a.src[1], *src2 = a.src[2];
  const int32_t *idx0 = a.idx[0], *idx1 = a.idx[1], *idx2 = a.idx[2];
  const float *as0 = a.add_src[0], *as1 = a.add_src[1];
  const int32_t *ai0 = a.add_idx[0], *ai1 = a.add_idx[1];
  const unsigned ring0 = __builtin_amdgcn_readfirstlane(lds_addr_of(ring));
  const bool I0 = SH::has_idx(idx0), I1 = NPH > 1 && SH::has_idx(idx1), I2 = NPH > 2 && SH::has_idx(idx2);
  const bool A0 = NADD > 0 && SH::has_addidx(ai0), A1 = NADD > 1 && SH::has_addidx(ai1);
  const int n_idx = (I0 ? 1 : 0) + (I1 ? 1 : 0) + (I2 ? 1 : 0) + (A0 ? 1 : 0) + (A1 ? 1 : 0);

  QStream qs;
  qs.issued = 0, qs.total = my_tiles * 4 * G, qs.du = 0, qs.dq = 0, qs.dslot = 0, qs.cslot = 0, qs.young = 0;
  auto next_job = [&]() -> DmaQ {
    DmaQ j;
    const char* up = contig ? U0 + (size_t)qs.du * MGN_WPACK_BYTES : pick8(U0, U1, U2, U3, U4, U5, U6, U7, qs.du);
    j.su = (const char*)uniform_ptr((const float*)(up + qs.dq * X6_QBYTES + wv * WSHARE));
    j.lds = ring0 + qs.dslot * X6_QBYTES + wv * WSHARE;
    j.on = qs.issued < qs.total;
    ++qs.issued;
    qs.dslot = (qs.dslot == RING - 1) ? 0 : qs.dslot + 1;
    if (++qs.dq == 4) {
      qs.dq = 0;
      qs.du = (qs.du + 1 == G) ? 0 : qs.du + 1;
    }
    return j;
  };
#pragma unroll
  for (int k = 0; k < AHEAD; ++k) {
    const DmaQ j0 = next_job();
#pragma unroll
    for (int i = 0; i < PPW; ++i) dmaq_issue(j0, i, lane16);
  }
  for (int i = threadIdx.x; i < 5 * H; i += 64 * NW) {
    const int l = i >> 7, jx = i & 127;
    const float* bp = (l == 4) ? a.scale : pick4(a.b[0], a.b[1], a.b[2], a.b[3], l);
    ((__attribute__((address_space(3))) float*)cst)[i] = (bp != nullptr && (l == 4 || l < NLL)) ? bp[jx] : 0.f;
  }
  auto lds_bias = [&](f32x4 (&acc)[HB], int l) {
#pragma unroll
    for (int ib = 0; ib < HB; ++ib) acc[ib] = *(lds_cf32x4*)(cst + l * 512 + 64 * ib + 16 * g);
  };
  auto rows_of = [&](long tl, long& mm, bool& valid, int (&rid)[5], auto U) {
    constexpr bool UL = decltype(U)::value;
    const long m = (tl * NW + wv) * 16 + c;
    valid = m < a.M;
    mm = valid ? m : a.M - 1;
    auto ldx = [&](const int32_t* ip) -> int {
      if constexpr (UL) return ldiu(ip + mm);
      else return ip[mm];
    };
    rid[0] = I0 ? ldx(idx0) : (int)mm;
    rid[1] = (NPH > 1) ? (I1 ? ldx(idx1) : (int)mm) : 0;
    rid[2] = (NPH > 2) ? (I2 ? ldx(idx2) : (int)mm) : 0;
    rid[3] = (NADD > 0) ? (A0 ? ldx(ai0) : (int)mm) : 0;
    rid[4] = (NADD > 1) ? (A1 ? ldx(ai1) : (int)mm) : 0;
  };
  auto LD2 = [&](f32x4 (&dst)[8], const float* rowp, int s, int& n) {
    if constexpr (UT) ld2u(dst, rowp, s, n);
    else ld2(dst, rowp, s, n);
  };
  auto LANDED = [&](int v) -> int {
    if constexpr (UT) return landed(v);
    else return v;
  };
  long mm;
  bool valid;
  int rid[5];
  int nbk = 0;
  rows_of(tile, mm, valid, rid, std::false_type{});
  f32x4 nin[HB], acc[HB], pr[HB];
  u32x4 xs[4][3];
#pragma unroll
  for (int kb = 0; kb < HB; ++kb) nin[kb] = ld4(src0 + (long)rid[0] * H + 4 * g + 16 * kb);
  dma_drain();
  __syncthreads();

  auto run_unit = [&](auto late) {
#pragma unroll
    for (int jq = 0; jq < 4; ++jq) {
      TL_STAMP(3);
      __syncthreads();
      TL_STAMP(4);
#ifdef MGN_EXP_PRIO
      __builtin_amdgcn_s_setprio(0);
#endif
      const DmaQ job = next_job();
      const int before = qs.young;
      qs.young = 0;
      int early = 0;
      gemm_q<TERMS, PPW>(acc, xs[jq], ring + qs.cslot * X6_QBYTES, lane16, job, [&](int s) { late(jq, s, (s < 3) ? early : qs.young); });
      qs.cslot = (qs.cslot == RING - 1) ? 0 : qs.cslot + 1;
      TL_STAMP(5);
      if (AHEAD == 2) {
        drain_allow(before + (job.on ? PPW : 0) + early + qs.young);
      } else {
        if (job.on)
          dma_drain_counted<PPW*(AHEAD - 1)>();
        else
          dma_drain();
      }
      TL_STAMP(6);
    }
#ifdef MGN_EXP_PRIO
    __builtin_amdgcn_s_setprio(3);
#endif
  };

  for (; tile < tw.end; tile += tw.stride) {
    const long ntile = tile + tw.stride;
    const bool has_next = ntile < tw.end;
    const bool wvalid = __builtin_amdgcn_readfirstlane((int)((tile * NW + wv) * 16 < a.M));
    long mmn;
    bool validn;
    int ridn[5];
    TL_STAMP(1);
#pragma unroll
    for (int p = 0; p < 5; ++p) rid[p] = LANDED(rid[p]);
    lds_bias(acc, 0);
    auto unit_body = [&](int u) {
      if (u < NPH) {
        split_tile<TERMS, NW != 6>(nin, xs);
      } else {
        const int l = u - NPH + 1;
        if (l == 1) {
          if (NADD > 0) {
#pragma unroll
            for (int ib = 0; ib < HB; ++ib) acc[ib] += pr[ib];
          }
          if (NADD > 1) {
#pragma unroll
            for (int ib = 0; ib < HB; ++ib) acc[ib] += nin[ib];
          }
        }
        if (ACT == MGN_ACT_SILU) {
          float* sz = pick3(sZ0, sZ1, sZ2, l - 1);
          if (sz != nullptr) {
            if (valid) {
#pragma unroll
              for (int ib = 0; ib < HB; ++ib) st4_stream(sz + mm * H + 4 * g + 16 * ib, acc[ib]);
            }
            if (wvalid) qs.young += 8;
          }
#pragma unroll
          for (int ib = 0; ib < HB; ++ib)
#pragma unroll
            for (int r = 0; r < 4; ++r) acc[ib][r] = silu_f(acc[ib][r]);
        } else {
#pragma unroll
          for (int ib = 0; ib < HB; ++ib)
#pragma unroll
            for (int r = 0; r < 4; ++r) {
              float v = acc[ib][r];
              asm("v_max_f32 %0, 0, %0" : "+v"(v));
              acc[ib][r] = v;
            }
        }
        float* sh = pick3(sH0, sH1, sH2, l - 1);
        const bool s16 = (TERMS == 1) && a.precision == 2;
        if (sh != nullptr && !s16) {
          if (valid) {
#pragma unroll
            for (int ib = 0; ib < HB; ++ib) st4_stream(sh + mm * H + 4 * g + 16 * ib, acc[ib]);
          }
          if (wvalid) qs.young += 8;
        }
        uint32_t* smk = (ACT == MGN_ACT_SILU) ? nullptr : pick3(sM0, sM1, sM2, l - 1);
        if (smk != nullptr) {
          u32 bits = 0;
#pragma unroll
          for (int ib = 0; ib < HB; ++ib)
#pragma unroll
            for (int r = 0; r < 4; ++r) {
              const float hval = acc[ib][r];
              int t = __builtin_bit_cast(int, hval);
              t = (t < 0) ? 0 : ((t > 1) ? 1 : t);
              bits |= (u32)t << (4 * ib + r);
            }
          if (valid) *(__attribute__((address_space(1))) u32*)(smk + mm * 4 + g) = bits;
          if (wvalid) qs.young += 1;
        }
        split_tile<TERMS, NW != 6>(acc, xs);
        if (TERMS == 1 && sh != nullptr && s16) {
          if (valid) {
#pragma unroll
            for (int pq = 0; pq < 4; ++pq)
              st4_stream((float*)((char*)sh + (size_t)(mm * H + 32 * pq + 8 * g) * 2), __builtin_bit_cast(f32x4, xs[pq][0]));
          }
          if (wvalid) qs.young += 4;
        }
        lds_bias(acc, l);
      }
      run_unit([&](int jq, int s, int& n) {
        if (jq == 0) {
          if (u == 0 && s == 0) {
            rows_of(has_next ? ntile : tile, mmn, validn, ridn, std::integral_constant<bool, UI>{});
            n += n_idx;
          }
          if (u == 0 && NADD > 0)
            LD2(pr, as0 + (long)rid[3] * H + 4 * g, s, n);
          else if (u == GL - 1 && NLL > 1 && HAS_RESID)
            LD2(pr, a.resid + mm * H + 4 * g, s, n);
        } else if (jq == 1) {
          if (u < NPH) {
            if (u + 1 < NPH)
              LD2(nin, pick3(src0, src1, src2, u + 1) + (long)((u == 0) ? rid[1] : rid[2]) * H + 4 * g, s, n);
            else if (NADD > 1)
              LD2(nin, as1 + (long)rid[4] * H + 4 * g, s, n);
          }
          if (u == GL - 1 && NLL > 1 && NPOST == 0 && (UT || has_next))
            LD2(nin, src0 + (long)LANDED(ridn[0]) * H + 4 * g, s, n);
        } else if (jq == 2) {
          if (UT && HAS_SEG && u == GL - 1 && s == 0) {
            const long r0 = (tile * NW + wv) * 16;
            const long rk = (c < 8) ? ((r0 > 0) ? r0 - 1 : 0) : ((r0 + 16 < a.M) ? r0 + 16 : a.M - 1);
            if constexpr (UI) nbk = ldiu(a.seg_key + rk);
            else if constexpr (UT) nbk = a.seg_key[rk];
            n += 1;
          }
        }
      });
    };
    if constexpr (UT) {
#pragma unroll
      for (int u = 0; u < SH::nphase(a) + SH::NL(a) - 1; ++u) unit_body(u);
    } else {
      for (int u = 0; u < GL; ++u) unit_body(u);
    }
    if (NLL == 1) {
      if (NADD > 0) {
#pragma unroll
        for (int ib = 0; ib < HB; ++ib) acc[ib] += pr[ib];
      }
      if (NADD > 1) {
#pragma unroll
        for (int ib = 0; ib < HB; ++ib) acc[ib] += nin[ib];
      }
      if (HAS_RESID) {
#pragma unroll
        for (int kb = 0; kb < HB; ++kb) pr[kb] = ld4(a.resid + mm * H + 4 * g + 16 * kb);
      }
      if (NPOST == 0 && has_next) {
        const long rn = LANDED(ridn[0]);
#pragma unroll
        for (int kb = 0; kb < HB; ++kb) nin[kb] = ld4(src0 + rn * H + 4 * g + 16 * kb);
      }
    }
    TL_STAMP(7);
    {
      float inv = 1.f;
      if (HAS_SCALE) {
        float ss = 0.f;
#pragma unroll
        for (int ib = 0; ib < HB; ++ib)
#pragma unroll
          for (int r = 0; r < 4; ++r) ss = fmaf(acc[ib][r], acc[ib][r], ss);
        ss = rowsum4(ss);
        const float rms = sqrtf(ss) / sqrtf((float)H);
        inv = 1.0f / (rms + a.eps);
        if (a.saveR != nullptr && valid && g == 0) st1(a.saveR + mm, rms);
      }
      const long ro = mm * H + 4 * g;
#pragma unroll
      for (int ib = 0; ib < HB; ++ib) {
        f32x4 y = acc[ib];
        if (HAS_SCALE) {
          const f32x4 u = y * inv;
          if (a.saveU != nullptr && valid) st4_stream(a.saveU + ro + 16 * ib, u);
          y = *(lds_cf32x4*)(cst + 4 * 512 + 64 * ib + 16 * g) * u;
        }
        if (a.y_out != nullptr && valid) st4(a.y_out + ro + 16 * ib, y);
        f32x4 yo = y;
        if (HAS_RESID) yo = pr[ib] + y;
        if (valid) st4(a.out + ro + 16 * ib, yo);
        acc[ib] = HAS_SEG ? y : yo;
      }
      if (wvalid) qs.young += 8 + ((HAS_SCALE && a.saveU != nullptr) ? 8 : 0) + ((a.y_out != nullptr) ? 8 : 0);
    }
    TL_STAMP(9);
    if (HAS_SEG) {
      if constexpr (UT) {
        const long r0 = (tile * NW + wv) * 16;
        const int nb = landed(nbk);
        const int kprev = (r0 > 0) ? __builtin_amdgcn_readlane(nb, 0) : -1;
        const int knxt = (r0 + 16 < a.M) ? __builtin_amdgcn_readlane(nb, 15) : -1;
        TL_STAMP(10);
        seg_scan_store<true>(acc, valid ? rid[3] : -1, (tile * NW + wv), a.seg_rowptr, a.seg_out, a.seg_part, g, kprev, knxt);
      } else {
        seg_scan_store(acc, valid ? a.seg_key[mm] : -1, (tile * NW + wv), a.seg_rowptr, a.seg_out, a.seg_part, g);
      }
    }
    if (NPOST > 0) {
      split_tile<TERMS, NW != 6>(acc, xs);
      auto post_body = [&](int q) {
#pragma unroll
        for (int ib = 0; ib < HB; ++ib) acc[ib] = f32x4{0.f, 0.f, 0.f, 0.f};
        run_unit([&](int jq, int s, int& n) {
          if (jq == 0 && q == NPOST - 1 && (UT || has_next)) LD2(nin, src0 + (long)LANDED(ridn[0]) * H + 4 * g, s, n);
        });
        float* po = (q == 0) ? a.post_out[0] : a.post_out[1];
        if (valid) {
#pragma unroll
          for (int ib = 0; ib < HB; ++ib) st4(po + mm * H + 4 * g + 16 * ib, acc[ib]);
        }
        if (wvalid) qs.young += 8;
      };
      if constexpr (UT) {
#pragma unroll
        for (int q = 0; q < SH::n_post(a); ++q) post_body(q);
      } else {
        for (int q = 0; q < NPOST; ++q) post_body(q);
      }
    }
    mm = mmn;
    valid = validn;
#pragma unroll
    for (int p = 0; p < 5; ++p) rid[p] = ridn[p];
    TL_STAMP(8);
  }
  TL_DUMP();
}

#define X6_BWD_LDS_BYTES(NUSED) (X6_RING * X6_QBYTES + 512 + 4 * (NUSED) * 128 * 4)
template <int ST>
__device__ __forceinline__ void fold_step(float (&v)[32], int c) {
  constexpr int n = 16 >> ST;
  const bool up = (c >> ST) & 1;
#pragma unroll
  for (int i = 0; i < n; ++i) {
    const float lo = v[i], hi = v[i + n];
    const float keep = up ? hi : lo;
    const float send = up ? lo : hi;
    v[i] = keep + __shfl_xor(send, 1 << ST);
  }
}
struct SbDyn {
  static constexpr bool ST = false;
  static __device__ __forceinline__ int NL(const mgn_mlp_bwd_args& a) { return a.NL; }
  static __device__ __forceinline__ int n_din(const mgn_mlp_bwd_args& a) { return a.n_din; }
  static __device__ __forceinline__ bool scale(const mgn_mlp_bwd_args& a) { return a.scale != nullptr; }
  static __device__ __forceinline__ bool din_resid(const mgn_mlp_bwd_args& a) { return a.din_resid[0] != nullptr; }
};
struct SbEdge {
  static constexpr bool ST = true;
  static __device__ __forceinline__ constexpr int NL(const mgn_mlp_bwd_args&) { return 4; }
  static __device__ __forceinline__ constexpr int n_din(const mgn_mlp_bwd_args&) { return 1; }
  static __device__ __forceinline__ constexpr bool scale(const mgn_mlp_bwd_args&) { return true; }
  static __device__ __forceinline__ constexpr bool din_resid(const mgn_mlp_bwd_args&) { return true; }
};
__device__ __forceinline__ float ldfu(const float* p) {
  float v;
  asm volatile("global_load_dword %0, %1, off" : "=v"(v) : "v"(p) : "memory");
  return v;
}
__device__ __forceinline__ u32 ldwu(const uint32_t* p) {
  u32 v;
  asm volatile("global_load_dword %0, %1, off" : "=v"(v) : "v"(p) : "memory");
  return v;
}
template <int TERMS, bool FRONT, int ACT, bool SEG = false, class SB = SbDyn>
__global__ void __launch_bounds__(256, 2) k_mlp_bwd_x6(const mgn_mlp_bwd_args a) {
  constexpr int HB = 8, H = 128;
  constexpr bool UT = SB::ST;
  static_assert(!UT || (!FRONT && !SEG && ACT == MGN_ACT_RELU), "static backward shape: plain ReLU chain only");
  const int NLL = SB::NL(a), NDIN = SB::n_din(a);
  const bool HAS_SCALE = SB::scale(a), HAS_DRESID = SB::din_resid(a);
  extern __shared__ __attribute__((aligned(16))) char smem[];
  lds_char* ring = (lds_char*)smem;
  lds_char* cst = ring + X6_RING * X6_QBYTES;
  float* lds = (float*)(smem + X6_RING * X6_QBYTES + 512);
  const int lane = threadIdx.x & 63;
  const int wv = __builtin_amdgcn_readfirstlane(threadIdx.x >> 6);
  const int c = lane & 15, g = lane >> 4;
  const unsigned lane16 = 16u * lane;
  const int nslot = NLL + 1;
  const bool hb0 = a.db[0] != nullptr, hb1 = a.db[1] != nullptr, hb2 = a.db[2] != nullptr, hb3 = a.db[3] != nullptr;
  const bool hsc = HAS_SCALE && a.dscale != nullptr;
  auto lds_slot = [&](int l) -> int { return (int)(hb0 && l > 0) + (int)(hb1 && l > 1) + (int)(hb2 && l > 2) + (int)(hb3 && l > 3); };
  auto slot_used = [&](int l) -> bool { return (l == NLL) ? hsc : pick4(hb0, hb1, hb2, hb3, l); };
  const int nused = lds_slot(NLL) + (hsc ? 1 : 0);
  float* lds_w = lds + wv * nused * H;
  for (int i = lane; i < nused * H; i += 64) lds_w[i] = 0.f;
  for (int i = threadIdx.x; i < H; i += 256)
    ((__attribute__((address_space(3))) float*)cst)[i] = HAS_SCALE ? a.scale[i] : 0.f;
  const long ntiles = (a.M + 63) / 64;
  const TileWalk tw = tile_walk(ntiles);
  long tile = tw.first;
  const long my_tiles = tw.count;
  x6_stagger();
  const int nf = FRONT ? a.n_front : 0;
  const int G = nf + (NLL - 1) + NDIN;
  const char *U0 = (const char*)a.wpk[0], *U1 = (const char*)a.wpk[1], *U2 = (const char*)a.wpk[2], *U3 = (const char*)a.wpk[3];
  const char *U4 = (const char*)a.wpk[4], *U5 = (const char*)a.wpk[5], *U6 = (const char*)a.wpk[6], *U7 = (const char*)a.wpk[7];
  const bool contig = x6_contig(U0, U1, U2, U3, U4, U5, U6, U7, G);
  const float *F0 = a.front_src[0], *F1 = a.front_src[1], *F2 = a.front_src[2];
  const float* fres = a.front_resid;
  float* fout = a.front_out;
  const float* src_rows = (nf > 0) ? F0 : a.dOut;
  const float* add_rows = (nf > 0) ? fres : a.dOut2;
  const int32_t* add_idx = (nf > 0) ? nullptr : a.idx2;
  const uint32_t *Ms0 = a.Ms[0], *Ms1 = a.Ms[1], *Ms2 = a.Ms[2];
  const float *Zs0 = a.Zs[0], *Zs1 = a.Zs[1], *Zs2 = a.Zs[2];
  float *dZ0 = a.dZ[0], *dZ1 = a.dZ[1], *dZ2 = a.dZ[2], *dZ3 = a.dZ[3];
  float *db0 = a.db[0], *db1 = a.db[1], *db2 = a.db[2], *db3 = a.db[3];
  const float* dr0 = HAS_DRESID ? a.din_resid[0] : nullptr;
  float* dI0 = a.dIn[0];
  const unsigned ring0 = __builtin_amdgcn_readfirstlane(lds_addr_of(ring));

  constexpr int PPWB = (TERMS == 1) ? 2 : 6;
  QStream qs;
  qs.issued = 0, qs.total = my_tiles * 4 * G, qs.du = 0, qs.dq = 0, qs.dslot = 0, qs.cslot = 0, qs.young = 0;
  auto next_job = [&]() -> DmaQ {
    DmaQ j;
    const char* up = contig ? U0 + (size_t)qs.du * MGN_WPACK_BYTES : pick8(U0, U1, U2, U3, U4, U5, U6, U7, qs.du);
    j.su = (const char*)uniform_ptr((const float*)(up + qs.dq * X6_QBYTES + wv * (PPWB * 1024)));
    j.lds = ring0 + qs.dslot * X6_QBYTES + wv * (PPWB * 1024);
    j.on = qs.issued < qs.total;
    ++qs.issued;
    qs.dslot = (qs.dslot == X6_RING - 1) ? 0 : qs.dslot + 1;
    if (++qs.dq == 4) {
      qs.dq = 0;
      qs.du = (qs.du + 1 == G) ? 0 : qs.du + 1;
    }
    return j;
  };
  float dsum2[2] = {0.f, 0.f};

  if (my_tiles > 0) {
#pragma unroll
    for (int k = 0; k < 2; ++k) {
      const DmaQ j0 = next_job();
#pragma unroll
      for (int i = 0; i < PPWB; ++i) dmaq_issue(j0, i, lane16);
    }
    auto rows_of = [&](long tl, long& mm, bool& valid) {
      const long m = (tl * 4 + wv) * 16 + c;
      valid = m < a.M;
      mm = valid ? m : a.M - 1;
    };
    long mm;
    bool valid;
    rows_of(tile, mm, valid);
    f32x4 dz[HB], acc[HB], pu[HB], pd2[HB];
    u32x4 xs[4][3];
    float prms;
    long r2n = 0;
    int r2u = 0;
    u32 mbits = 0;
    auto LD2 = [&](f32x4 (&dst)[8], const float* rowp, int s, int& n) {
      if constexpr (UT) ld2u(dst, rowp, s, n);
      else ld2(dst, rowp, s, n);
    };
    {
      const long r2 = (add_rows != nullptr) ? (add_idx ? (long)add_idx[mm] : mm) : 0;
      prms = HAS_SCALE ? ld1(a.R + mm) : 0.f;
#pragma unroll
      for (int kb = 0; kb < HB; ++kb) {
        dz[kb] = ld4(src_rows + mm * H + 4 * g + 16 * kb);
        pd2[kb] = (add_rows != nullptr) ? ld4(add_rows + r2 * H + 4 * g + 16 * kb) : f32x4{0.f, 0.f, 0.f, 0.f};
        pu[kb] = HAS_SCALE ? ld4(a.U + mm * H + 4 * g + 16 * kb) : f32x4{0.f, 0.f, 0.f, 0.f};
      }
    }
    dma_drain();
    __syncthreads();

    auto run_unit = [&](auto late) {
#pragma unroll
      for (int jq = 0; jq < 4; ++jq) {
        __syncthreads();
        const DmaQ job = next_job();
        const int before = qs.young;
        qs.young = 0;
        int early = 0;
        gemm_q<TERMS, PPWB>(acc, xs[jq], ring + qs.cslot * X6_QBYTES, lane16, job, [&](int s) { late(jq, s, (s < 3) ? early : qs.young); });
        qs.cslot = (qs.cslot == X6_RING - 1) ? 0 : qs.cslot + 1;
        drain_allow(before + (job.on ? PPWB : 0) + early + qs.young);
      }
    };

    for (; tile < tw.end; tile += tw.stride) {
      const long ntile = tile + tw.stride;
      const bool has_next = ntile < tw.end;
      const bool wvalid = __builtin_amdgcn_readfirstlane((int)((tile * 4 + wv) * 16 < a.M));
      long mmn;
      bool validn;
      rows_of(has_next ? ntile : tile, mmn, validn);
      if (nf > 0) {
#pragma unroll
        for (int ib = 0; ib < HB; ++ib) acc[ib] = pd2[ib];
        for (int p = 0; p < nf; ++p) {
          split_tile<TERMS, !FRONT && !SEG>(dz, xs);
          const float* nxt = (p == 0) ? F1 : F2;
          run_unit([&](int jq, int s, int& n) {
            if (jq == 0 && p + 1 < nf) ld2(dz, nxt + mm * H + 4 * g, s, n);
          });
        }
        if (fout != nullptr) {
          if (valid) {
#pragma unroll
            for (int ib = 0; ib < HB; ++ib) st4(fout + mm * H + 4 * g + 16 * ib, acc[ib]);
          }
          if (wvalid) qs.young += 8;
        }
#pragma unroll
        for (int ib = 0; ib < HB; ++ib) dz[ib] = valid ? acc[ib] : f32x4{0.f, 0.f, 0.f, 0.f};
      } else {
#pragma unroll
        for (int ib = 0; ib < HB; ++ib) {
          const f32x4 extra = (add_rows != nullptr) ? pd2[ib] : f32x4{0.f, 0.f, 0.f, 0.f};
          dz[ib] = valid ? dz[ib] + extra : f32x4{0.f, 0.f, 0.f, 0.f};
        }
      }
      if (HAS_SCALE) {
        float dot = 0.f;
        if (a.dscale != nullptr) {
          float v[32];
#pragma unroll
          for (int ib = 0; ib < HB; ++ib)
#pragma unroll
            for (int r = 0; r < 4; ++r) v[4 * ib + r] = dz[ib][r] * pu[ib][r];
          fold_step<0>(v, c), fold_step<1>(v, c), fold_step<2>(v, c), fold_step<3>(v, c);
          dsum2[0] += v[0];
          dsum2[1] += v[1];
        }
#pragma unroll
        for (int ib = 0; ib < HB; ++ib) {
          const f32x4 gg = *(lds_cf32x4*)(cst + 64 * ib + 16 * g) * dz[ib];
#pragma unroll
          for (int r = 0; r < 4; ++r) dot = fmaf(gg[r], pu[ib][r], dot);
          dz[ib] = gg;
        }
        dot = rowsum4(dot);
        const float rms = prms;
        const float inv = 1.0f / (rms + a.eps);
        const float k2 = (rms > 0.f) ? dot / ((float)H * rms) : 0.f;
#pragma unroll
        for (int ib = 0; ib < HB; ++ib) dz[ib] = dz[ib] * inv - pu[ib] * k2;
      }
      const bool d16 = (TERMS == 1) && a.precision >= 2;
      float* dzl_top = pick4(dZ0, dZ1, dZ2, dZ3, NLL - 1);
      const bool top16 = d16 && (NLL - 1 >= 1 || a.precision == 3);
      {
        float* dzl = dzl_top;
        if (dzl != nullptr && !top16) {
          if (valid) {
#pragma unroll
            for (int ib = 0; ib < HB; ++ib) st4(dzl + mm * H + 4 * g + 16 * ib, dz[ib]);
          }
          if (wvalid) qs.young += 8;
        }
        if (pick4(db0, db1, db2, db3, NLL - 1) != nullptr) {
          const f32x4(&dz1)[1][HB] = *(const f32x4(*)[1][HB]) & dz;
          colsum_to_lds_add<HB, 1>(lds_w + lds_slot(NLL - 1) * H, dz1, c, g);
        }
      }
      split_tile<TERMS, !FRONT && !SEG>(dz, xs);
      if (TERMS == 1 && dzl_top != nullptr && top16) {
        if (valid) {
#pragma unroll
          for (int pq = 0; pq < 4; ++pq)
            st4((float*)((char*)dzl_top + (size_t)(mm * H + 32 * pq + 8 * g) * 2), __builtin_bit_cast(f32x4, xs[pq][0]));
        }
        if (wvalid) qs.young += 4;
      }
      auto pref = [&](int jq, int s, int& n) {
        if (jq == 1) {
          if (s == 0) {
            if (HAS_SCALE) {
              prms = ld1(a.R + mmn);
              n += 1;
            }
            r2n = mmn;
            if (add_rows != nullptr && add_idx != nullptr) {
              r2n = (long)add_idx[mmn];
              n += 1;
            }
          }
          if (HAS_SCALE) ld2(pu, a.U + mmn * H + 4 * g, s, n);
        } else if (jq == 2) {
          if (add_rows != nullptr) ld2(pd2, add_rows + r2n * H + 4 * g, s, n);
        }
      };
      auto pref_u = [&](int jq, int s, int& n) {
        if (jq == 0) {
          if (s == 0) {
            prms = ldfu(a.R + mmn);
            n += 1;
          }
          ld2u(pu, a.U + mmn * H + 4 * g, s, n);
        } else if (jq == 1) {
          ld2u(pd2, add_rows + (long)landed(r2u) * H + 4 * g, s, n);
        } else if (jq == 2) {
          ld3u(dz, src_rows + mmn * H + 4 * g, s, n);
        }
      };
      auto chain_unit = [&](int k) {
        const int l = NLL - 1 - k;
#pragma unroll
        for (int ib = 0; ib < HB; ++ib) acc[ib] = f32x4{0.f, 0.f, 0.f, 0.f};
        const bool fetch_resid = (k == NLL - 2) && NDIN == 1 && HAS_DRESID;
        const bool pref_here = (k == NLL - 2) && NDIN == 0 && has_next;
        run_unit([&](int jq, int s, int& n) {
          if (ACT == MGN_ACT_SILU) {
            if (jq == 0) ld2(pd2, pick3(Zs0, Zs1, Zs2, l - 1) + mm * H + 4 * g, s, n);
          } else if (jq == 0 && s == 0) {
            if constexpr (UT) mbits = ldwu(pick3(Ms0, Ms1, Ms2, l - 1) + mm * 4 + g);
            else mbits = *(__attribute__((address_space(1))) const u32*)(pick3(Ms0, Ms1, Ms2, l - 1) + mm * 4 + g);
            n += 1;
            if (UT && k == 0) {
              if constexpr (UT) r2u = ldiu(add_idx + mmn);
              n += 1;
            }
          }
          if (fetch_resid) {
            if (jq == 1) LD2(pu, dr0 + mm * H + 4 * g, s, n);
          } else if (pref_here) {
            pref(jq, s, n);
          }
        });
        if (ACT == MGN_ACT_SILU) {
#pragma unroll
          for (int ib = 0; ib < HB; ++ib)
#pragma unroll
            for (int r = 0; r < 4; ++r) dz[ib][r] = valid ? acc[ib][r] * dsilu_f(pd2[ib][r]) : 0.f;
        } else {
#pragma unroll
          for (int ib = 0; ib < HB; ++ib)
#pragma unroll
            for (int r = 0; r < 4; ++r) dz[ib][r] = (valid && ((mbits >> (4 * ib + r)) & 1u)) ? acc[ib][r] : 0.f;
        }
        float* dzp = pick3(dZ0, dZ1, dZ2, l - 1);
        const bool low16 = d16 && (l - 1 >= 1 || a.precision == 3);
        if (dzp != nullptr && !low16) {
          if (valid) {
#pragma unroll
            for (int ib = 0; ib < HB; ++ib) st4(dzp + mm * H + 4 * g + 16 * ib, dz[ib]);
          }
          if (wvalid) qs.young += 8;
        }
        if (pick3(db0, db1, db2, l - 1) != nullptr) {
          const f32x4(&dz1)[1][HB] = *(const f32x4(*)[1][HB]) & dz;
          colsum_to_lds_add<HB, 1>(lds_w + lds_slot(l - 1) * H, dz1, c, g);
        }
        if (k + 1 < G || low16) split_tile<TERMS, !FRONT && !SEG>(dz, xs);
        if (TERMS == 1 && dzp != nullptr && low16) {
          if (valid) {
#pragma unroll
            for (int pq = 0; pq < 4; ++pq)
              st4((float*)((char*)dzp + (size_t)(mm * H + 32 * pq + 8 * g) * 2), __builtin_bit_cast(f32x4, xs[pq][0]));
          }
          if (wvalid) qs.young += 4;
        }
        if (SEG && l == 1) {
          seg_scan_store(dz, valid ? a.seg_key[mm] : -1, (tile * 4 + wv), a.seg_rowptr, a.seg_out, a.seg_part, g);
        }
      };
      if constexpr (UT) {
#pragma unroll
        for (int k = 0; k < SB::NL(a) - 1; ++k) chain_unit(k);
      } else {
        for (int k = 0; k < NLL - 1; ++k) chain_unit(k);
      }
      if (NDIN == 1) {
        if (dr0 == nullptr) {
#pragma unroll
          for (int ib = 0; ib < HB; ++ib) acc[ib] = f32x4{0.f, 0.f, 0.f, 0.f};
        } else {
#pragma unroll
          for (int ib = 0; ib < HB; ++ib) acc[ib] = pu[ib];
        }
        run_unit([&](int jq, int s, int& n) {
          if constexpr (UT) {
            pref_u(jq, s, n);
          } else {
            if (jq == 0)
              ld2(dz, src_rows + mmn * H + 4 * g, s, n);
            else if (has_next)
              pref(jq, s, n);
          }
        });
        if (valid) {
#pragma unroll
          for (int ib = 0; ib < HB; ++ib) st4(dI0 + mm * H + 4 * g + 16 * ib, acc[ib]);
        }
        if (wvalid) qs.young += 8;
      }
      if (NDIN == 0 && has_next) {
#pragma unroll
        for (int kb = 0; kb < HB; ++kb) dz[kb] = ld4(src_rows + mmn * H + 4 * g + 16 * kb);
      }
      mm = mmn;
      valid = validn;
    }
  }
  if (HAS_SCALE && a.dscale != nullptr) {
    const int i0 = ((c & 1) << 4) | ((c & 2) << 2) | (c & 4) | ((c & 8) >> 2);
#pragma unroll
    for (int k = 0; k < 2; ++k) {
      const int i = i0 + k;
      lds_w[lds_slot(NLL) * H + 16 * (i >> 2) + 4 * g + (i & 3)] = dsum2[k];
    }
  }
  __syncthreads();
  float* ws = (float*)a.red_ws + (size_t)blockIdx.x * nslot * H;
  for (int i = threadIdx.x; i < nslot * H; i += 256) {
    const int l = i >> 7;
    if (slot_used(l)) {
      const int j = lds_slot(l) * H + (i & 127);
      ws[i] = ((lds[j] + lds[nused * H + j]) + lds[2 * nused * H + j]) + lds[3 * nused * H + j];
    }
  }
}

__device__ __forceinline__ void dma_row_piece4_bf(const uint16_t* __restrict__ X, long row0, long M, unsigned lds0, int wv, int lane, int i) {
  const int q = 2 * wv + i;
  const int r = 4 * q + (lane >> 4);
  long row = row0 + r;
  row = row < M ? row : M - 1;
  const int gch = (lane & 15) ^ (4 * ((r >> 3) & 1));
  const unsigned voff = (unsigned)((row - row0) * 256 + 16 * gch);
  glds16(uniform_ptr((const float*)(X + row0 * 128)), voff, lds0 + q * 1024);
}

__device__ __forceinline__ void dma_row_piece8(const float* __restrict__ X, long row0, long M, unsigned lds0, int wv, int lane, int i) {
  const int q = 4 * wv + i;
  const int r = 2 * q + (lane >> 5);
  long row = row0 + r;
  row = row < M ? row : M - 1;
  const int gch = (lane & 31) ^ (4 * ((r >> 3) & 1));
  const unsigned voff = (unsigned)((row - row0) * 512 + 16 * gch);
  glds16(uniform_ptr(X + row0 * 128), voff, lds0 + q * 1024);
}

__device__ __forceinline__ void split8(const float (&v)[8], u32x4& p1, u32x4& p2, u32x4& p3) {
  float ra[4], rb[4];
#pragma unroll
  for (int h = 0; h < 4; ++h) p1[h] = pk_bf16(v[2 * h], v[2 * h + 1]);
#pragma unroll
  for (int h = 0; h < 4; ++h) {
    ra[h] = v[2 * h] - bf_lo(p1[h]);
    rb[h] = v[2 * h + 1] - bf_hi(p1[h]);
  }
#pragma unroll
  for (int h = 0; h < 4; ++h) p2[h] = pk_bf16(ra[h], rb[h]);
#pragma unroll
  for (int h = 0; h < 4; ++h) {
    ra[h] -= bf_lo(p2[h]);
    rb[h] -= bf_hi(p2[h]);
  }
#pragma unroll
  for (int h = 0; h < 4; ++h) p3[h] = pk_bf16(ra[h], rb[h]);
}

#ifndef MGN_WGRAD_SPLIT_MFMA
#define MGN_WGRAD_SPLIT_MFMA 0
#endif
struct WgSel {
  u32x4 s0, s1;
};
__device__ __forceinline__ WgSel wg_sel(int c, int g) {
  WgSel S;
  const u32 m1 = 0xbf80u;
  const bool on = (g == (c >> 2));
#pragma unroll
  for (int d = 0; d < 4; ++d) {
    u32 w0 = 0, w1 = 0;
#pragma unroll
    for (int h = 0; h < 2; ++h) {
      const int e = 2 * d + h;
      if (on && e == (c & 3)) w0 |= m1 << (16 * h);
      if (on && e == 4 + (c & 3)) w1 |= m1 << (16 * h);
    }
// ... 616 lines not shown
```

### graph-physics_amd/ops.py

```python
from __future__ import annotations

import ctypes as C
from typing import List, Optional, Sequence, Tuple

import torch

from . import _capi

EPS = 1e-8
import os as _os
X6_ENABLED = _os.environ.get("MGN_FP32_MFMA") is None

_matrix_precision = "fp32"


def set_matrix_precision(p: str) -> None:
    global _matrix_precision
    if p not in ("fp32", "bf16"):
        raise ValueError("matrix precision must be 'fp32' or 'bf16'")
    if p == "bf16" and not X6_ENABLED:
        raise RuntimeError("bf16 matrix mode runs on the split-bf16 kernels; unset MGN_FP32_MFMA")
    _matrix_precision = p


# ... 380 lines not shown
    if front is not None:
        rows, fres, fout = front
        a.n_front = len(rows)
        for p_, t in enumerate(rows):
            a.front_src[p_] = _ptr(t)
        a.front_resid, a.front_out = _ptr(fres), _ptr(fout)
    dev = dOut.device
    nbytes = L.mgn_mlp_bwd_workspace_bytes(M, H, NL)
    ws = torch.empty(max(nbytes, 16), dtype=torch.uint8, device=dev)
    a.red_ws, a.red_ws_bytes = _ptr(ws), ws.numel()
    if defer is not None:
        a.defer_reduce = 1
        defer.append((ws, M, H, NL, out_w, len(din), list(db), dscale if scale is not None else None))
    with torch.cuda.device(dev):
        rc = L.mgn_mlp_bwd(C.byref(a), _stream(dev))
    _capi.check(rc, "mgn_mlp_bwd")


_fused_ws: dict = {}


def edge_bwd_fused(E: int, dOut, dAgg, idx, U, R, scale, X: Sequence[torch.Tensor], Ms: Sequence[torch.Tensor], wpk: Sequence[int],
                   dIn, dZ0, dW: Sequence[Tuple[torch.Tensor, int, int]], db: Sequence[Optional[torch.Tensor]], dscale, precision: int = 0):
    L = _capi.lib()
    a = _capi.EdgeBwdFusedArgs()
    a.M = E
    a.dOut, a.dAgg, a.idx, a.U, a.R, a.scale, a.eps = _ptr(dOut), _ptr(dAgg), _ptr(idx), _ptr(U), _ptr(R), _ptr(scale), EPS
    for l in range(4):
        a.X[l] = _ptr(X[l])
        a.wpk[l] = wpk[l]
        t, off, ld = dW[l]
        a.dW[l], a.ldw[l] = t.data_ptr() + 4 * off, ld
        a.db[l] = _ptr(db[l])
    for l in range(3):
        a.Ms[l] = _ptr(Ms[l])
    a.dIn, a.dZ0, a.dscale = _ptr(dIn), _ptr(dZ0), _ptr(dscale)
    dev = dOut.device
    key = (dev.type, dev.index, torch.cuda.current_stream(dev).cuda_stream)
    ws = _fused_ws.get(key)
    if ws is None:
        ws = torch.empty(L.mgn_edge_bwd_fused_workspace_bytes(), dtype=torch.uint8, device=dev)
        _fused_ws[key] = ws
    a.ws, a.ws_bytes, a.precision = _ptr(ws), ws.numel(), precision
    with torch.cuda.device(dev):
        rc = L.mgn_edge_bwd_fused(C.byref(a), _stream(dev))
    _capi.check(rc, "mgn_edge_bwd_fused")


def colred_batch(deferred: list, dev):
    if not deferred:
        return
    arr = (_capi.ColredJob * len(deferred))()
    for i, (ws, M, H, NL, out_w, n_din, db, dscale) in enumerate(deferred):
        arr[i].red_ws, arr[i].M, arr[i].H, arr[i].NL, arr[i].out_w, arr[i].n_din = _ptr(ws), M, H, NL, out_w, n_din
        for l in range(NL):
            arr[i].db[l] = _ptr(db[l])
        arr[i].dscale = _ptr(dscale)
    with torch.cuda.device(dev):
        rc = _capi.lib().mgn_colred_batch(len(deferred), arr, _stream(dev))
    _capi.check(rc, "mgn_colred_batch")
    deferred.clear()


def wgrad(jobs, dev, precision: int = 0):
    L = _capi.lib()
    for i0 in range(0, len(jobs), _capi.MAX_WGRAD_JOBS):
        chunk = jobs[i0:i0 + _capi.MAX_WGRAD_JOBS]
        arr = (_capi.WgradJob * len(chunk))()
        for j, job in enumerate(chunk):
            A, lda, nja, B, ldb, nkb, kw, dW, off, ldw = job[:10]
            arr[j].db = _ptr(job[10]) if len(job) > 10 else None
            arr[j].A, arr[j].B = _ptr(A), _ptr(B)
            arr[j].dW = dW.data_ptr() + 4 * off
            arr[j].M = A.shape[0]
            arr[j].lda, arr[j].ldb, arr[j].ldw = lda, ldb, ldw
            arr[j].nja, arr[j].nkb, arr[j].kw = nja, nkb, kw
        nbytes = L.mgn_wgrad_workspace_bytes(len(chunk), arr)
        ws = torch.empty(max(nbytes, 16), dtype=torch.uint8, device=dev)
        with torch.cuda.device(dev):
            rc = L.mgn_wgrad_p(len(chunk), arr, _ptr(ws), ws.numel(), precision, _stream(dev))
        _capi.check(rc, "mgn_wgrad")


def wpack(blocks: Sequence[Tuple[int, int, bool, int]], dev):
    if not blocks:
        return
    arr = (_capi.WpackBlock * len(blocks))()
    for i, (src, ld, tr, dst) in enumerate(blocks):
        arr[i].src, arr[i].ld_src, arr[i].transpose, arr[i].dst = src, ld, int(bool(tr)), dst
    with torch.cuda.device(dev):
        rc = _capi.lib().mgn_wpack(len(blocks), arr, _stream(dev))
    _capi.check(rc, "mgn_wpack")


def transpose_blocks(blocks: Sequence[Tuple[int, int, int, int]], H: int, dev):
    if not blocks:
        return
    arr = (_capi.TBlock * len(blocks))()
    for i, (src, lds, dst, ldd) in enumerate(blocks):
        arr[i].src, arr[i].ld_src, arr[i].dst, arr[i].ld_dst = src, lds, dst, ldd
    with torch.cuda.device(dev):
        rc = _capi.lib().mgn_transpose_blocks(len(blocks), arr, H, _stream(dev))
    _capi.check(rc, "mgn_transpose_blocks")


def gather_rows(src: torch.Tensor, idx: torch.Tensor, out: Optional[torch.Tensor] = None) -> torch.Tensor:
    n, H = int(idx.numel()), int(src.shape[1])
    if out is None:
        out = torch.empty(n, H, dtype=torch.float32, device=src.device)
    with torch.cuda.device(src.device):
        rc = _capi.lib().mgn_gather_rows(_ptr(src), _ptr(idx), n, H, _ptr(out), _stream(src.device))
    _capi.check(rc, "mgn_gather_rows", prep=True)
    return out


def halo_unpack_add(rows: torch.Tensor, nodes: torch.Tensor, rowptr: torch.Tensor, perm: torch.Tensor, dst: torch.Tensor):
    with torch.cuda.device(dst.device):
        rc = _capi.lib().mgn_halo_unpack_add(_ptr(rows), _ptr(nodes), _ptr(rowptr), _ptr(perm), int(nodes.numel()), int(dst.shape[1]),
                                             _ptr(dst), _stream(dst.device))
    _capi.check(rc, "mgn_halo_unpack_add", prep=True)


def gate_fwd(G, phi, gate_pos, agg, gate_out, agg_out):
    with torch.cuda.device(agg.device):
        rc = _capi.lib().mgn_gate_fwd(_ptr(G), _ptr(phi), _ptr(gate_pos), _ptr(agg), int(agg.shape[0]), int(agg.shape[1]),
                                      _ptr(gate_out), _ptr(agg_out), _stream(agg.device))
    _capi.check(rc, "mgn_gate_fwd", prep=True)


def gate_bwd(dAggG, agg, gate, dAgg, dG):
    with torch.cuda.device(agg.device):
        rc = _capi.lib().mgn_gate_bwd(_ptr(dAggG), _ptr(agg), _ptr(gate), int(agg.shape[0]), int(agg.shape[1]), _ptr(dAgg), _ptr(dG),
                                      _stream(agg.device))
    _capi.check(rc, "mgn_gate_bwd", prep=True)


def rope_gather(x, pos, inv_freq, topo: "Topology", axes: int, out):
    with torch.cuda.device(x.device):
        rc = _capi.lib().mgn_rope_gather(_ptr(x), _ptr(pos), int(pos.shape[1]), _ptr(inv_freq), int(inv_freq.numel()), axes,
                                         _ptr(topo.src_s), _ptr(topo.dst_s), topo.E, int(x.shape[1]), _ptr(out), _stream(x.device))
    _capi.check(rc, "mgn_rope_gather", prep=True)


def rope_scatter(T, pos, inv_freq, topo: "Topology", axes: int, resid, out):
    n = int(out.shape[0])
    with torch.cuda.device(T.device):
        rc = _capi.lib().mgn_rope_scatter(_ptr(T), _ptr(pos), int(pos.shape[1]), _ptr(inv_freq), int(inv_freq.numel()), axes,
                                          _ptr(topo.src_s), _ptr(topo.dst_s), _ptr(topo.rowptr_src), _ptr(topo.perm_src), n,
                                          int(T.shape[1]), _ptr(resid), _ptr(out), _stream(T.device))
    _capi.check(rc, "mgn_rope_scatter", prep=True)


import threading as _threading
from dataclasses import dataclass

_call = _threading.local()


def _saving() -> bool:
    return getattr(_call, "grad", True)


ACT_IDS = {"relu": 0, "silu": 1, "gelu": 2}


def mlp_apply(x, has_norm, *params, act: str = "relu"):
    _call.grad = torch.is_grad_enabled()
    try:
        return MlpFunction.apply(x, has_norm, ACT_IDS[act], *params)
    finally:
        _call.grad = True

# ... 46 lines not shown

def _bf16_rounded_many(ts):
    if not ts:
        return []
    src = [t.detach() for t in ts]
    lo = [torch.empty_like(t, dtype=torch.bfloat16) for t in src]
    out = [torch.empty_like(t) for t in src]
    torch._foreach_copy_(lo, src)
    torch._foreach_copy_(out, lo)
    return out


def set_grad_ready_hook(fn) -> None:
    global _grad_ready_hook
    _grad_ready_hook = fn


def _parse_recompute_env(v: str):
    v = v.strip()
    if v.isdigit():
        return int(v)
    if v not in ("off", "on", "auto"):
        raise ValueError(f"MGN_RECOMPUTE={v!r}: expected 'off', 'on', 'auto' or a number of rounds")
    return v


_recompute_mode = _parse_recompute_env(_os.environ.get("MGN_RECOMPUTE", "auto"))


def set_activation_recompute(mode) -> None:
    global _recompute_mode
    if not (mode in ("off", "on", "auto") or (isinstance(mode, int) and not isinstance(mode, bool) and mode >= 0)):
        raise ValueError("activation recompute mode must be 'off', 'on', 'auto' or a number of rounds")
    _recompute_mode = mode


def get_activation_recompute() -> str:
    return _recompute_mode


def saved_activation_bytes(E: int, Nn: int, H: int, NL: int, L: int, act: int, save16: bool = False) -> int:
    per_row = 4 * H * ((NL - 1) * (2 if act == 1 else 1) + 2) + 16 * (NL - 1) + 4
    per_edge = per_row - (2 * H * (NL - 1) if save16 else 0)
    return L * (E * per_edge + Nn * (per_row + 4 * H))


def recompute_rounds(E, Nn, H, NL, L, act, dev, save16: bool = False) -> int:
    if _recompute_mode == "on":
        return L
    if _recompute_mode == "off":
        return 0
    if isinstance(_recompute_mode, int):
        return min(_recompute_mode, L)
    try:
        free, _total = torch.cuda.mem_get_info(dev)
        free += torch.cuda.memory_reserved(dev) - torch.cuda.memory_allocated(dev)
    except Exception:
        return 0
    frac = float(_os.environ.get("MGN_RECOMPUTE_FRACTION", "0.65"))
    per_round = saved_activation_bytes(E, Nn, H, NL, 1, act, save16)
    fit = int(frac * free // max(per_round, 1))
    return max(0, L - fit)


class MlpFunction(torch.autograd.Function):

    @staticmethod
    def forward(ctx, x, has_norm, act, *params):
        _require_device(x, *params)
        x = _f32c(x)
        NL = (len(params) - (1 if has_norm else 0)) // 2
        Ws = [_f32c(params[2 * l]) for l in range(NL)]
        bs = [_f32c(params[2 * l + 1]) for l in range(NL)]
        scale = _f32c(params[2 * NL]) if has_norm else None
        if NL < 2:
            raise AssertionError("The MLP must have at least 2 layers (input and output).")
        M, kin = x.shape
        H = Ws[0].shape[0]
        out_w = Ws[-1].shape[0]
        if H not in SUPPORTED_H or kin > H or out_w > H:
            raise NotImplementedError(f"MLP widths (in={kin}, hidden={H}, out={out_w}) not supported by the MI355X engine")
        dev = x.device
        kp, op = pad16(kin), pad16(out_w)
        W0 = Ws[0]
        if kp != kin:
            W0 = torch.nn.functional.pad(W0, (0, kp - kin))
        Wl, bl = Ws[-1], bs[-1]
        if op != out_w:
            Wl = torch.nn.functional.pad(Wl, (0, 0, 0, op - out_w))
            bl = torch.nn.functional.pad(bl, (0, op - out_w))
        Wk = [W0] + Ws[1:-1] + [Wl]
        bk = bs[:-1] + [bl]
        prec = 1 if (_matrix_precision == "bf16" and not (H == 128 and out_w == H and X6_ENABLED and act != 2)) else 0
        if prec:
            Wk = [w.to(torch.bfloat16).to(torch.float32) for w in Wk]
            bk = [b.to(torch.bfloat16).to(torch.float32) for b in bk]
        need = any(ctx.needs_input_grad) and _saving()
        f = dict(dtype=torch.float32, device=dev)
        y = torch.empty(M, out_w, **f)
        x6 = H == 128 and out_w == H and X6_ENABLED and M > 0 and act != 2
        mode = "generic"
        if x6 and kin < H and 3 <= NL <= 4:
            mode = "enc"
        elif x6 and kin == H and NL <= 4:
            mode = "full"
        packed = mode != "generic"
        saveH = [torch.empty(M, H, **f) for _ in range(NL - 1)] if need else None
        U = torch.empty(M, H, **f) if (need and has_norm) else None
        R = torch.empty(M, **f) if (need and has_norm) else None
        Ms = [torch.empty(M, 4, dtype=torch.int32, device=dev) for _ in range(NL - 1)] if (need and packed and act == 0) else None
        Zs = [torch.empty(M, H, **f) for _ in range(NL - 1)] if (need and act != 0) else None
        if mode == "enc":
            h1 = saveH[0] if need else torch.empty(M, H, **f)
            mlp_fwd(M, H, [(x, None, kin)], [Wk[0]], [bk[0]], None, H, None, h1, Zs[0] if Zs else None, out_relu=True, act=act,
                    saveM=[Ms[0]] if Ms else None)
            pk = torch.empty((NL - 1) * _capi.WPACK_BYTES, dtype=torch.uint8, device=dev)
            units = [pk.data_ptr() + u * _capi.WPACK_BYTES for u in range(NL - 1)]
            wpack([(Wk[l + 1].data_ptr(), H, False, units[l]) for l in range(NL - 1)], dev)
            mlp_fwd(M, H, [(h1, None, H)], Wk[1:], bk[1:], scale, out_w, None, y, None,
                    saveH[1:] if need else None, U, R, wpk=units, saveM=Ms[1:] if Ms else None,
                    saveZ=Zs[1:] if Zs else None, act=act)
        elif mode == "full":
            pk = torch.empty(NL * _capi.WPACK_BYTES, dtype=torch.uint8, device=dev)
            units = [pk.data_ptr() + u * _capi.WPACK_BYTES for u in range(NL)]
            wpack([(Wk[l].data_ptr(), H, False, units[l]) for l in range(NL)], dev)
            mlp_fwd(M, H, [(x, None, H)], Wk, bk, scale, out_w, None, y, None, saveH, U, R, wpk=units, saveM=Ms, saveZ=Zs, act=act)
        else:
            mlp_fwd(M, H, [(x, None, kin)], Wk, bk, scale, out_w, None, y, None, saveH, U, R, act=act, saveZ=Zs, precision=prec)
        ctx.meta = (NL, H, kin, out_w, has_norm, kp != kin, op != out_w, act, mode)
        ctx.prec, ctx.Wk_rounded = prec, (Wk if prec else None)
        ctx.save_for_backward(x, *Ws, *([scale] if has_norm else []))
        ctx.pads = (W0 if kp != kin else None, Wl if op != out_w else None)
        ctx.saved_acts = (saveH, U, R, Ms, Zs)
        return y

    @staticmethod
    def backward(ctx, dy):
        NL, H, kin, out_w, has_norm, pad0, padl, act, mode = ctx.meta
        if ctx.saved_acts is None or ctx.saved_acts[0] is None:
            raise RuntimeError("MlpFunction: no saved activations -- backward ran a second time without retain_graph "
                               "support, or the forward ran under no_grad")
        t = ctx.saved_tensors
        x, Ws = t[0], list(t[1:1 + NL])
        scale = t[1 + NL] if has_norm else None
        Wk = [ctx.pads[0] if pad0 else Ws[0]] + Ws[1:-1] + [ctx.pads[1] if padl else Ws[-1]]
        prec = getattr(ctx, "prec", 0)
        if prec:
            Wk = ctx.Wk_rounded
        saveH, U, R, Ms, Zs = ctx.saved_acts
        dy = _f32c(dy)
        M, dev = x.shape[0], x.device
        kp, op = pad16(kin), pad16(out_w)
        f = dict(dtype=torch.float32, device=dev)
        widths = [H] * (NL - 1) + [op]
        zero = M == 0
        mk = torch.zeros if zero else torch.empty
        dZ = [mk(M, w, **f) for w in widths]
        db = [mk(w, **f) for w in widths]
        dscale = mk(H, **f) if has_norm else None
        dx = None
        want_dx = ctx.needs_input_grad[0]
        if want_dx and kin != H:
            raise NotImplementedError("input gradient of a ragged-width MLP input is not needed by the path")
        if want_dx:
            dx = mk(M, H, **f)
        if mode in ("enc", "full") and M > 0:
            tr = [Wk[l] for l in range(NL - 1, 0, -1)] + ([Wk[0]] if want_dx else [])
            pk = torch.empty(len(tr) * _capi.WPACK_BYTES, dtype=torch.uint8, device=dev)
            units = [pk.data_ptr() + u * _capi.WPACK_BYTES for u in range(len(tr))]
            wpack([(w.data_ptr(), H, True, units[u]) for u, w in enumerate(tr)], dev)
            din = [(None, None, dx)] if want_dx else []
            mlp_bwd(M, H, NL, dy, None, None, out_w, U, R, scale, saveH, [None] * NL, dZ, din, [None] * NL, dscale,
                    wpk=units, Ms=Ms, Zs=Zs, act=act)
        else:
            sq = [l for l in range(1, NL) if tuple(Wk[l].shape) == (H, H) and Wk[l].is_contiguous()]
            wt_buf = torch.empty(len(sq), H, H, **f) if sq else None
            if sq:
                transpose_blocks([(Wk[l].data_ptr(), H, wt_buf[k].data_ptr(), H) for k, l in enumerate(sq)], H, dev)
            WT = [None] + [wt_buf[sq.index(l)] if l in sq else Wk[l].t().contiguous() for l in range(1, NL)]
            din = [(Wk[0].t().contiguous(), None, dx)] if want_dx else []
            mlp_bwd(M, H, NL, dy, None, None, out_w, U, R, scale, saveH, WT, dZ, din, [None] * NL, dscale, act=act, Zs=Zs, precision=prec)
        ins = [x.to(torch.bfloat16).to(torch.float32) if prec else x] + list(saveH)
        in_w = [kin] + [H] * (NL - 1)
        dWs = [mk(widths[l], in_w[l], **f) for l in range(NL)]
        jobs = []
        for l in range(NL):
            jobs.append((dZ[l], widths[l], widths[l] // 16, ins[l], in_w[l], pad16(in_w[l]) // 16, in_w[l], dWs[l], 0, in_w[l], db[l]))
        if M > 0:
            wgrad(jobs, dev)
        grads = []
        for l in range(NL):
            dW, dbl = dWs[l], db[l]
            if l == NL - 1 and op != out_w:
                dW, dbl = dW[:out_w], dbl[:out_w]
            grads += [dW, dbl]
        if has_norm:
            grads.append(dscale)
        ctx.saved_acts = None
        return (dx, None, None, *grads)


def _split_block(q, spec: BlockSpec):
    NL, k = spec.nb_layers, spec.mlp_params
    We, be = [q[2 * l] for l in range(NL)], [q[2 * l + 1] for l in range(NL)]
    se = q[2 * NL] if spec.layer_norm else None
    Wn, bn = [q[k + 2 * l] for l in range(NL)], [q[k + 2 * l + 1] for l in range(NL)]
    sn = q[k + 2 * NL] if spec.layer_norm else None
    gp_ = tuple(q[2 * k: 2 * k + 3]) if spec.gate else None
    return We, be, se, Wn, bn, sn, gp_


class ProcessorFunction(torch.autograd.Function):

    @staticmethod
    def forward(ctx, x, e, topo: Topology, L: int, spec: BlockSpec, halo, pos, phi, rope_inv_freq, *params):
        _require_device(x, e, *params)
        x, e = _f32c(x), _f32c(e)
        Nn, H = x.shape
        N = topo.N
        E = e.shape[0]
        NL, act, PB = spec.nb_layers, spec.act_id, spec.per_block
        if H not in SUPPORTED_H:
            raise NotImplementedError(f"hidden_size={H} not supported by the MI355X engine (16/32/64/128)")
        if E != topo.E or (halo is None and Nn != N) or (halo is not None and (Nn != halo.n_own or N != halo.n_own + halo.n_ghost)):
            raise ValueError("x / edge_attr do not match the topology")
        if len(params) != L * PB:
            raise ValueError(f"expected {L} x {PB} block parameters, got {len(params)}")
        if NL < 2 or NL > _capi.MAX_LAYERS:
            raise AssertionError("The MLP must have at least 2 layers (input and output)." if NL < 2 else f"at most {_capi.MAX_LAYERS} layers per MLP")
        dev = x.device
        P = [_f32c(p) for p in params]
        P_params = P
        need = any(ctx.needs_input_grad) and _saving()
        f = dict(dtype=torch.float32, device=dev)
        _require_device(pos if spec.rope else None, phi, rope_inv_freq if spec.rope else None)
        if spec.rope:
            if pos is None:
                raise ValueError("Node positions `pos` must be provided when use_rope=True.")
            pos = _f32c(pos)
            if pos.dim() != 2 or pos.shape[1] < spec.rope_axes:
                raise ValueError("pos has fewer columns than rope_axes")
            if pos.shape[0] < N:
                raise IndexError(f"pos has {pos.shape[0]} rows for {N} nodes")
            if rope_inv_freq is None or rope_inv_freq.numel() != H // (2 * spec.rope_axes):
                raise ValueError("rope_inv_freq must hold hidden_size // (2 * rope_axes) frequencies")
            rope_inv_freq = _f32c(rope_inv_freq)
        if phi is not None:
            phi = _f32c(phi).reshape(-1)
            if phi.numel() != Nn:
                raise ValueError(f"phi holds {phi.numel()} values for {Nn} nodes")
        x6 = (H == 128) and X6_ENABLED and NL <= 4 and L > 0 and E > 0
        split = (H == 128) and NL <= 4 and not spec.rope and (x6 or act == 0) and L > 0 and E > 0
        prec = 1 if _matrix_precision == "bf16" else 0
        if prec and not x6 and L > 0 and E > 0:
            k_ = spec.mlp_params
            P = list(P)
            idx_ = [i_ * PB + j_ for i_ in range(L)
                    for j_ in list(range(2 * NL)) + list(range(k_, k_ + 2 * NL)) + ([2 * k_, 2 * k_ + 1] if spec.gate else [])]
            for i_, r_ in zip(idx_, _bf16_rounded_many([P_params[i_] for i_ in idx_])):
                P[i_] = r_
        if halo is not None and not (x6 and split):
            raise NotImplementedError("the partitioned path runs on the packed H = 128 kernels (no RoPE)")
        hubs = topo.begin_use()
        fuse_agg = x6 and _os.environ.get("MGN_NO_FUSED_AGG") is None and not hubs
        relu_bits = x6 and act == 0
        save16 = (relu_bits and prec == 1 and (split or spec.rope) and _os.environ.get("MGN_SAVE16", "1") != "0"
                  and _os.environ.get("MGN_FUSED_BWD", "0") != "1")
        ne = NL + (2 if spec.rope else 0)
        un0, up0 = ne, ne + NL + 1
        ug = up0 + 2
        NU = ug + (1 if spec.gate else 0)
        if x6:
            pk = torch.empty((L * NU + 2) * _capi.WPACK_BYTES, dtype=torch.uint8, device=dev)
            pk0 = pk.data_ptr()

            def unit(i, u):
                return pk0 + (i * NU + u) * _capi.WPACK_BYTES

            blocks = []
            for i in range(L):
                We, _, _, Wn, _, _, gpar = _split_block(P[PB * i: PB * (i + 1)], spec)
                We0, Wn0 = We[0].data_ptr(), Wn[0].data_ptr()
# ... 432 lines not shown
```

### include/mgn_hip.h

```cpp
#ifndef MGN_HIP_H
#define MGN_HIP_H

#include <stddef.h>
#include <stdint.h>

#ifdef __cplusplus
extern "C" {
#endif

#define MGN_MAX_LAYERS 8
#define MGN_MAX_PHASES 3
#define MGN_MAX_WGRAD_JOBS 48

int mgn_version(void);
const char* mgn_last_error(void);

size_t mgn_csr_workspace_bytes(int64_t E, int64_t N);
int mgn_csr_build(const int64_t* key, int64_t E, int64_t N, int32_t* rowptr, int32_t* perm,
                  void* ws, size_t ws_bytes, void* stream);

size_t mgn_topology_workspace_bytes(int64_t E, int64_t N);
int mgn_topology_build(const int64_t* src, const int64_t* dst, int64_t E, int64_t N, int32_t* rowptr_dst, int32_t* perm_dst,
                       int32_t* src_s, int32_t* dst_s, int32_t* rowptr_src, int32_t* perm_src, int32_t* max_degree_host,
                       void* ws, size_t ws_bytes, void* stream);
// ... 67 lines not shown
  int n_din;
  const float* WT0[MGN_MAX_PHASES];
  const float* din_resid[MGN_MAX_PHASES];
  float* dIn[MGN_MAX_PHASES];
  float* db[MGN_MAX_LAYERS];
  float* dscale;
  void* red_ws; size_t red_ws_bytes;
  const void* wpk[8];
  const uint32_t* Ms[MGN_MAX_LAYERS];
  int precision;
  int n_front;
  const float* front_src[MGN_MAX_PHASES];
  const float* front_resid;
  float* front_out;
  int defer_reduce;
  int act;
  const float* Zs[MGN_MAX_LAYERS];
  const int32_t* seg_key;
  const int32_t* seg_rowptr;
  float* seg_out;
  float* seg_part;
  int64_t dOut2_rows;
} mgn_mlp_bwd_args;
size_t mgn_mlp_bwd_workspace_bytes(int64_t M, int H, int NL);
int mgn_mlp_bwd(const mgn_mlp_bwd_args* args, void* stream);

typedef struct {
  const void* red_ws;
  int64_t M;
  int H, NL, out_w, n_din;
  float* db[MGN_MAX_LAYERS];
  float* dscale;
} mgn_colred_job;
int mgn_colred_batch(int n, const mgn_colred_job* jobs, void* stream);

typedef struct {
  const float* A; const float* B; float* dW;
  int64_t M;
  int lda, ldb, ldw;
  int nja, nkb, kw;
  float* db;
} mgn_wgrad_job;
size_t mgn_wgrad_workspace_bytes(int njobs, const mgn_wgrad_job* jobs);
int mgn_wgrad(int njobs, const mgn_wgrad_job* jobs, void* ws, size_t ws_bytes, void* stream);
int mgn_wgrad_p(int njobs, const mgn_wgrad_job* jobs, void* ws, size_t ws_bytes, int precision, void* stream);

typedef struct {
  int64_t M;
  const float* dOut;
  const float* dAgg;
  const int32_t* idx;
  const float* U;
  const float* R;
  const float* scale;
  float eps;
  const float* X[4];
  const uint32_t* Ms[3];
  const void* wpk[4];
  float* dIn;
  float* dZ0;
  float* dW[4];
  int ldw[4];
  float* db[4];
  float* dscale;
  void* ws;
  size_t ws_bytes;
  int precision;
} mgn_edge_bwd_fused_args;
size_t mgn_edge_bwd_fused_workspace_bytes(void);
int mgn_edge_bwd_fused(const mgn_edge_bwd_fused_args* args, void* stream);

int mgn_debug_occupancy(int* out);

typedef struct {
  const float* src; float* dst;
  int ld_src, ld_dst;
} mgn_tblock;
int mgn_transpose_blocks(int n, const mgn_tblock* blocks, int H, void* stream);

#define MGN_WPACK_BYTES 98304
typedef struct {
  const float* src; void* dst;
  int ld_src, transpose;
} mgn_wpack_block;
int mgn_wpack(int n, const mgn_wpack_block* blocks, void* stream);


size_t mgn_faces_to_edges_workspace_bytes(int64_t F, int K);
int mgn_faces_to_edges(const int64_t* face, int K, int64_t F, int64_t N, int64_t* src, int64_t* dst,
                       int64_t* n_edges, void* ws, size_t ws_bytes, void* stream);

#define MGN_NODE_OBSTACLE 1
size_t mgn_world_edges_workspace_bytes(int64_t E, int64_t max_world_pairs);
int mgn_add_world_edges(const float* x, int x_w, int pos_start, int D, int type_idx, int64_t N, double radius,
                        const int64_t* src_in, const int64_t* dst_in, int64_t E, int64_t max_world_pairs,
                        int64_t* src, int64_t* dst, int64_t* n_edges, void* ws, size_t ws_bytes, void* stream);

int mgn_edge_features(const float* pos, int D, const int64_t* src, const int64_t* dst, int64_t E,
                      float* edge_attr, void* stream);

size_t mgn_morton_order_workspace_bytes(int64_t N);
int mgn_morton_order(const float* pos, int ld, int D, int64_t N, int32_t* order, int32_t* rank, void* ws, size_t ws_bytes,
                     void* stream);

int mgn_add_noise(float* x, int x_w, int64_t N, int n_ranges, const int* starts, const int* ends, const float* scales,
                  int type_idx, uint64_t seed, uint32_t offset, void* stream);

#define MGN_NODE_TYPES 9
#define MGN_NODE_NORMAL 0
#define MGN_NODE_OUTFLOW 5
typedef struct {
  int64_t N, E;
  const float* x; int x_w;
  const float* y; int y_w;
  const float* edge_attr; int edge_w;
  int feat_start, feat_end, out_start, out_w, type_idx;
  float* acc_sum[3]; float* acc_sumsq[3]; float* acc_count[3]; float* num_acc[3];
  int accumulate[3];
  float std_eps;
  float* node_out; float* target_out; float* edge_out;
  int norm_w[3];
  float max_accumulations;
  int* type_err;
} mgn_sim_desc;
size_t mgn_sim_workspace_bytes(void);
int mgn_sim_pre(const mgn_sim_desc* desc, void* ws, size_t ws_bytes, void* stream);
int mgn_sim_post(const float* x, int x_w, int out_start, int type_idx, const float* y, int y_w,
                 const float* net_out, int O, const float* acc_sum, const float* acc_sumsq,
                 const float* acc_count, float std_eps, int mask_truth, int64_t N, float* pred, void* stream);
typedef struct {
  float* p; float* g; float* m; float* v;
  int64_t n;
} mgn_opt_tensor;
size_t mgn_clip_adamw_workspace_bytes(int n, const mgn_opt_tensor* tensors);
int mgn_clip_adamw(int n, const mgn_opt_tensor* tensors, float max_norm, const float* lr, float* step,
                   float beta1, float beta2, float eps, float weight_decay, float* grad_norm_out,
                   void* ws, size_t ws_bytes, void* stream);
int mgn_masked_mse_fwd(const float* out, int ldo, const float* target, int ldt, const float* type, int ldty, int64_t N, int O,
                       const float* types, int ntypes, float* part, float* loss, float* inv, void* stream);
int mgn_masked_mse_bwd(const float* out, int ldo, const float* target, int ldt, const float* type, int ldty, int64_t N, int O,
                       const float* types, int ntypes, const float* inv, const float* g, float* d_out, void* stream);
size_t mgn_clip_adamw_table_bytes(int n, const mgn_opt_tensor* tensors);
int mgn_clip_adamw_table(int n, const mgn_opt_tensor* tensors, void* table, size_t table_bytes);
int mgn_clip_adamw_t(int n, const mgn_opt_tensor* tensors, const void* table, float max_norm, const float* lr, float* step,
                     float beta1, float beta2, float eps, float weight_decay, float* grad_norm_out,
                     void* ws, size_t ws_bytes, void* stream);

int mgn_gather_rows(const float* src, const int32_t* idx, int64_t n, int H, float* out, void* stream);
int mgn_halo_unpack_add(const float* rows, const int32_t* nodes, const int32_t* rowptr, const int32_t* perm,
                        int64_t n_nodes, int H, float* dst, void* stream);

int mgn_gate_fwd(const float* G, const float* phi, const float* gate_pos, const float* agg, int64_t N, int H,
                 float* gate_out, float* agg_out, void* stream);
int mgn_gate_bwd(const float* dAggG, const float* agg, const float* gate, int64_t N, int H, float* dAgg, float* dG,
                 void* stream);
int mgn_rope_gather(const float* x, const float* pos, int pos_w, const float* inv_freq, int pair_count, int axes,
                    const int32_t* src, const int32_t* dst, int64_t E, int H, float* out, void* stream);
int mgn_rope_scatter(const float* T, const float* pos, int pos_w, const float* inv_freq, int pair_count, int axes,
                     const int32_t* src, const int32_t* dst, const int32_t* rowptr_src, const int32_t* perm_src,
                     int64_t N, int H, const float* resid, float* out, void* stream);

const char* mgn_prep_last_error(void);

int mgn_sparse_attn_fwd(const float* q, const float* k, const float* v, const int32_t* rowptr, const int32_t* col,
                        int64_t N, int H, int num_heads, float* y, float* lse, void* stream);
int mgn_sparse_attn_bwd(const float* q, const float* k, const float* v, const float* y, const float* lse, const float* dy,
// ... 121 lines not shown
```

Baseline: 82.59 steps/s.

## Route narrow-width MLP ends through fused x6 kernels with dedicated narrow wgrad

Adds a 'narrow' mode so MLPs whose output width is small (e.g. the decoder with out_w<=16) run on the packed x6 LDS forward/backward kernels, no longer taking the generic ragged path. Weight packing gains row/column extents so unpadded narrow weights can be packed with zero-fill. A specialised narrow weight-gradient kernel with a partial-sum reduction replaces the padded 128x128 wgrad tile for these jobs. The narrow input side (kin<128) stays disabled unless MGN_X6_NARROW=2. This adds complexity and workspace, and risks correctness in the new narrow code paths.

```diff
diff --git a/graph-physics_amd/_capi.py b/graph-physics_amd/_capi.py
--- a/graph-physics_amd/_capi.py
+++ b/graph-physics_amd/_capi.py
@@ -106,7 +106,8 @@
 
 
 class WpackBlock(C.Structure):
-    _fields_ = [("src", _f32p), ("dst", C.c_void_p), ("ld_src", C.c_int), ("transpose", C.c_int)]
+    _fields_ = [("src", _f32p), ("dst", C.c_void_p), ("ld_src", C.c_int), ("transpose", C.c_int),
+                ("src_rows", C.c_int), ("src_cols", C.c_int)]
 
 
 WPACK_BYTES = 98304
diff --git a/graph-physics_amd/csrc/mgn_kernels.hip b/graph-physics_amd/csrc/mgn_kernels.hip
--- a/graph-physics_amd/csrc/mgn_kernels.hip
+++ b/graph-physics_amd/csrc/mgn_kernels.hip
@@ -1737,6 +1737,123 @@
   }
 }
 
+struct WgradNarrow {
+  const float* wide;
+  const float* nar;
+  long M;
+  int ldn, nw;
+  float* partial;
+  int nparts;
+  float* dW;
+  int ldw;
+  float* db;
+  int a_wide;
+  int nrows_out;
+};
+template <int NWT>
+__global__ void __launch_bounds__(256) k_wgrad_narrow(const WgradNarrow L) {
+  constexpr int UN = NWT <= 4 ? 8 : (NWT <= 16 ? 4 : 2);
+  __shared__ float red[3][NWT + 2][128];
+  const int lane = threadIdx.x & 63;
+  const int wv = __builtin_amdgcn_readfirstlane(threadIdx.x >> 6);
+  const long r0 = L.M * (long)blockIdx.x / (long)gridDim.x, r1 = L.M * ((long)blockIdx.x + 1) / (long)gridDim.x;
+  float acc[NWT][2], cn[NWT], cw[2] = {0.f, 0.f};
+#pragma unroll
+  for (int j = 0; j < NWT; ++j) acc[j][0] = acc[j][1] = cn[j] = 0.f;
+  for (long row = r0 + wv; row < r1; row += 4 * UN) {
+    float w[UN][2], nv[UN][NWT];
+#pragma unroll
+    for (int u = 0; u < UN; ++u) {
+      const long rr = row + 4 * u;
+      const bool ok = rr < r1;
+      const long rc = ok ? rr : row;
+      const float* wp = L.wide + rc * 128 + 2 * lane;
+      const float* np = L.nar + rc * L.ldn;
+      w[u][0] = ok ? wp[0] : 0.f;
+      w[u][1] = ok ? wp[1] : 0.f;
+#pragma unroll
+      for (int j = 0; j < NWT; ++j) nv[u][j] = (ok && j < L.nw) ? np[j] : 0.f;
+    }
+#pragma unroll
+    for (int u = 0; u < UN; ++u) {
+#pragma unroll
+      for (int j = 0; j < NWT; ++j) {
+        acc[j][0] = fmaf(nv[u][j], w[u][0], acc[j][0]);
+        acc[j][1] = fmaf(nv[u][j], w[u][1], acc[j][1]);
+        cn[j] += nv[u][j];
+      }
+      cw[0] += w[u][0];
+      cw[1] += w[u][1];
+    }
+  }
+  if (wv > 0) {
+#pragma unroll
+    for (int j = 0; j < NWT; ++j) {
+      red[wv - 1][j][2 * lane] = acc[j][0];
+      red[wv - 1][j][2 * lane + 1] = acc[j][1];
+    }
+    red[wv - 1][NWT][2 * lane] = cw[0];
+    red[wv - 1][NWT][2 * lane + 1] = cw[1];
+    if (lane == 0) {
+#pragma unroll
+      for (int j = 0; j < NWT; ++j) red[wv - 1][NWT + 1][j] = cn[j];
+    }
+  }
+  __syncthreads();
+  if (wv == 0) {
+    float* P = L.partial + (size_t)blockIdx.x * (NWT + 2) * 128;
+#pragma unroll
+    for (int j = 0; j < NWT; ++j) {
+      P[j * 128 + 2 * lane] = ((acc[j][0] + red[0][j][2 * lane]) + red[1][j][2 * lane]) + red[2][j][2 * lane];
+      P[j * 128 + 2 * lane + 1] = ((acc[j][1] + red[0][j][2 * lane + 1]) + red[1][j][2 * lane + 1]) + red[2][j][2 * lane + 1];
+    }
+    P[NWT * 128 + 2 * lane] = ((cw[0] + red[0][NWT][2 * lane]) + red[1][NWT][2 * lane]) + red[2][NWT][2 * lane];
+    P[NWT * 128 + 2 * lane + 1] = ((cw[1] + red[0][NWT][2 * lane + 1]) + red[1][NWT][2 * lane + 1]) + red[2][NWT][2 * lane + 1];
+    if (lane == 0) {
+#pragma unroll
+      for (int j = 0; j < NWT; ++j) P[(NWT + 1) * 128 + j] = ((cn[j] + red[0][NWT + 1][j]) + red[1][NWT + 1][j]) + red[2][NWT + 1][j];
+    }
+  }
+}
+template <int NWT>
+__global__ void __launch_bounds__(1024) k_wgrad_narrow_red(const WgradNarrow L) {
+  __shared__ float red[16][64];
+  constexpr size_t st = (size_t)(NWT + 2) * 128;
+  const int e = blockIdx.x * 64 + (threadIdx.x & 63);
+  const int pl = threadIdx.x >> 6;
+  const int jr = e >> 7, i = e & 127;
+  const int nout = L.a_wide ? L.nw : L.nrows_out;
+  const bool is_w = jr < NWT && jr < nout;
+  const bool is_b = L.db != nullptr && (L.a_wide ? jr == NWT : (jr == NWT + 1 && i < nout));
+  float s0 = 0.f, s1 = 0.f, s2 = 0.f, s3 = 0.f;
+  if (is_w || is_b) {
+    const float* P = L.partial + e;
+    int b = pl;
+    for (; b + 48 < L.nparts; b += 64) {
+      s0 += P[(size_t)b * st];
+      s1 += P[(size_t)(b + 16) * st];
+      s2 += P[(size_t)(b + 32) * st];
+      s3 += P[(size_t)(b + 48) * st];
+    }
+    if (b < L.nparts) s0 += P[(size_t)b * st];
+    if (b + 16 < L.nparts) s1 += P[(size_t)(b + 16) * st];
+    if (b + 32 < L.nparts) s2 += P[(size_t)(b + 32) * st];
+  }
+  red[pl][threadIdx.x & 63] = (s0 + s1) + (s2 + s3);
+  __syncthreads();
+  if (pl == 0) {
+    float v = 0.f;
+#pragma unroll
+    for (int q = 0; q < 16; q += 4) v += (red[q][threadIdx.x] + red[q + 1][threadIdx.x]) + (red[q + 2][threadIdx.x] + red[q + 3][threadIdx.x]);
+    if (is_w) {
+      if (L.a_wide) L.dW[(size_t)i * L.ldw + jr] = v;
+      else L.dW[(size_t)jr * L.ldw + i] = v;
+    } else if (is_b) {
+      L.db[i] = v;
+    }
+  }
+}
+
 template <int HB>
 __global__ void __launch_bounds__(256) k_segsum(const float* __restrict__ src, const int32_t* __restrict__ rowptr,
                                                 const int32_t* __restrict__ perm, float* __restrict__ out, long N) {
@@ -1958,11 +2075,33 @@
   size_t smem;
 };
 
+static bool fwd_x6(const mgn_mlp_fwd_args& a);
+static bool bwd_x6(const mgn_mlp_bwd_args& a);
+static bool narrow_on() {
+  const char* env = getenv("MGN_X6_NARROW");
+  return env == nullptr || atoi(env) != 0;
+}
+static bool fwd_narrow(const mgn_mlp_fwd_args& a) {
+  if (a.H != 128 || a.act != MGN_ACT_RELU || a.precision != 0 || a.nphase != 1 || a.n_add != 0 || a.n_post != 0 || a.ldw0 != 0) return false;
+  if (a.idx[0] != nullptr || a.seg_out != nullptr || a.y_out != nullptr || a.out_relu) return false;
+  const bool k0 = a.kw[0] != a.H, no = a.out_w != a.H;
+  if (!k0 && !no) return false;
+  if (k0 && (a.kw[0] < 1 || a.kw[0] > 32 || a.NL < 3 || a.NL > 4)) return false;
+  if (no && (a.out_w < 1 || a.out_w > 16 || a.NL < 2 || a.NL > 4 || a.scale != nullptr || a.resid != nullptr)) return false;
+  return narrow_on() && fwd_x6(a);
+}
+static bool bwd_narrow(const mgn_mlp_bwd_args& a) {
+  if (a.H != 128 || a.act != MGN_ACT_RELU || a.precision != 0 || a.out_w == a.H || a.out_w < 1 || a.out_w > 16) return false;
+  if (a.NL < 2 || a.NL > 4 || a.n_din > 1 || a.n_front != 0 || a.scale != nullptr || a.dOut2 != nullptr || a.seg_out != nullptr) return false;
+  return narrow_on() && bwd_x6(a);
+}
+
 static bool fwd_ragged(const mgn_mlp_fwd_args& a) {
   bool r = (a.out_w != a.H);
   for (int p = 0; p < a.nphase; ++p) r = r || (a.kw[p] != a.H);
-  return r;
-}
+  return r && !fwd_narrow(a);
+}
+static bool bwd_ragged(const mgn_mlp_bwd_args& a) { return (a.out_w != a.H && !bwd_narrow(a)) || a.n_din > 1; }
 
 static MlpPlan plan_mlp(int64_t M, int H, int NL, bool ragged, bool bwd, int act = MGN_ACT_RELU) {
   MlpPlan p;
@@ -2078,6 +2217,17 @@
     if (grid > cap) grid = cap;
     if (const char* e = getenv("MGN_GRID")) {
       if (atoi(e) > 0 && (unsigned)atoi(e) < grid) grid = (unsigned)atoi(e);
+    }
+    if (fwd_narrow(a)) {
+      static thread_local bool nrw_attr = false;
+      if (!nrw_attr) {
+        if (set_fwd_x6_attr<6, 4, 0, ShNarrow>()) return 1;
+        nrw_attr = true;
+      }
+      unsigned gn = (unsigned)((a.M + 63) / 64);
+      if (gn > 512u) gn = 512u;
+      hipLaunchKernelGGL((k_mlp_fwd_x6<6, 4, 0, ShNarrow>), dim3(gn), dim3(256), X6_FWD_LDS_BYTES(4), s, a);
+      return 0;
     }
     const int shape = (nw == 4 && !silu) ? fwd_static_shape(a) : 0;
     if (shape == 1 && !nw6 && fwd_ppr_ok(a)) {
@@ -2224,7 +2374,7 @@
 
 template <int HB>
 static int launch_bwd(const mgn_mlp_bwd_args& a, hipStream_t s) {
-  MlpPlan p = plan_mlp(a.M, a.H, a.NL, a.out_w != a.H || a.n_din > 1, true, a.act);
+  MlpPlan p = plan_mlp(a.M, a.H, a.NL, bwd_ragged(a), true, a.act);
   if (p.lds && bwd_x6(a)) {
     static thread_local bool attr_done = false;
     if (!attr_done) {
@@ -2244,6 +2394,17 @@
     int nused = (a.scale != nullptr && a.dscale != nullptr) ? 1 : 0;
     for (int l = 0; l < a.NL; ++l) nused += (a.db[l] != nullptr) ? 1 : 0;
     const size_t lds = X6_BWD_LDS_BYTES(nused);
+    if (bwd_narrow(a)) {
+      static thread_local bool nrw_attr = false;
+      if (!nrw_attr) {
+        if (hipFuncSetAttribute((const void*)k_mlp_bwd_x6<6, false, 0, false, SbNarrow>, hipFuncAttributeMaxDynamicSharedMemorySize,
+                                X6_BWD_LDS_BYTES(LDS_MAX_NL + 1)) != hipSuccess)
+          return 1;
+        nrw_attr = true;
+      }
+      hipLaunchKernelGGL((k_mlp_bwd_x6<6, false, 0, false, SbNarrow>), dim3(p.grid), dim3(256), lds, s, a);
+      return 0;
+    }
     const bool front = a.n_front > 0;
     const char* st_env = getenv("MGN_X6_STATIC");
     const bool static_off = st_env != nullptr && atoi(st_env) == 0;
@@ -2577,7 +2738,7 @@
   if (a.n_din < 0 || a.n_din > MGN_MAX_PHASES) return fail(1, "mgn_mlp_bwd: n_din out of range");
   if (a.n_din > 1 && a.dZ[0] == nullptr) return fail(1, "mgn_mlp_bwd: n_din > 1 needs dZ[0]");
   if (a.precision < 0 || a.precision > 3) return fail(1, "mgn_mlp_bwd: precision must be 0 (fp32-grade), 1 (bf16), 2 (bf16, two-byte dZ[1..]) or 3 (dZ[0] too)");
-  if (a.precision >= 2 && (!bwd_x6(a) || !plan_mlp(a.M, a.H, a.NL, a.out_w != a.H || a.n_din > 1, true).lds || a.act != MGN_ACT_RELU || a.n_front != 0))
+  if (a.precision >= 2 && (!bwd_x6(a) || !plan_mlp(a.M, a.H, a.NL, bwd_ragged(a), true).lds || a.act != MGN_ACT_RELU || a.n_front != 0))
     return fail(1, "mgn_mlp_bwd: precision 2 (two-byte dZ rows) needs the packed split-bf16 path (H = 128, wpk, Ms), ReLU and no front stage");
   if (a.act != MGN_ACT_RELU && a.act != MGN_ACT_SILU && a.act != MGN_ACT_GELU) return fail(1, "mgn_mlp_bwd: act must be MGN_ACT_RELU, _SILU or _GELU");
   if (a.act == MGN_ACT_GELU && (a.wpk[0] != nullptr || a.precision != 0 || a.seg_out != nullptr || a.n_front != 0))
@@ -2587,14 +2748,14 @@
       if (a.Zs[l - 1] == nullptr) return fail(1, "mgn_mlp_bwd: SiLU / GELU need the saved pre-activations Zs[]");
   }
   if (a.act == MGN_ACT_SILU) {
-    if (plan_mlp(a.M, a.H, a.NL, a.out_w != a.H || a.n_din > 1, true).lds && !bwd_x6(a))
+    if (plan_mlp(a.M, a.H, a.NL, bwd_ragged(a), true).lds && !bwd_x6(a))
       return fail(1, "mgn_mlp_bwd: SiLU is not available on the exact-fp32 LDS generation (pass packed weights)");
   }
-  if (a.n_front != 0 && !(plan_mlp(a.M, a.H, a.NL, a.out_w != a.H || a.n_din > 1, true).lds && bwd_x6(a)))
+  if (a.n_front != 0 && !(plan_mlp(a.M, a.H, a.NL, bwd_ragged(a), true).lds && bwd_x6(a)))
     return fail(1, "mgn_mlp_bwd: the front stage needs the packed split-bf16 path (H = 128, full widths, wpk, Ms, no dOut2)");
-  if (a.precision >= 1 && plan_mlp(a.M, a.H, a.NL, a.out_w != a.H || a.n_din > 1, true, a.act).lds && !bwd_x6(a))
+  if (a.precision >= 1 && plan_mlp(a.M, a.H, a.NL, bwd_ragged(a), true, a.act).lds && !bwd_x6(a))
     return fail(1, "mgn_mlp_bwd: at H = 128 with full widths the bf16 matrix mode needs the packed split-bf16 path (wpk, Ms); other shapes run it on the generic kernels");
-  if (a.seg_out != nullptr && !(plan_mlp(a.M, a.H, a.NL, a.out_w != a.H || a.n_din > 1, true).lds && bwd_x6(a)))
+  if (a.seg_out != nullptr && !(plan_mlp(a.M, a.H, a.NL, bwd_ragged(a), true).lds && bwd_x6(a)))
     return fail(1, "mgn_mlp_bwd: the fused segment sum of dZ[0] needs the packed split-bf16 path (fp32-grade, ReLU, dZ[0], no front stage)");
   if (a.M == 0) return 0;
   if (a.red_ws_bytes < mgn_mlp_bwd_workspace_bytes(a.M, a.H, a.NL)) return fail(1, "mgn_mlp_bwd: workspace too small");
@@ -2608,7 +2769,7 @@
   }
   if (lrc) return fail(2, "mgn_mlp_bwd: cannot reserve LDS");
   if (int rc = check_launch("mgn_mlp_bwd")) return rc;
-  const unsigned grid = plan_mlp(a.M, a.H, a.NL, a.out_w != a.H || a.n_din > 1, true, a.act).grid;
+  const unsigned grid = plan_mlp(a.M, a.H, a.NL, bwd_ragged(a), true, a.act).grid;
   const int nslot = a.NL + 1;
   ColredOuts outs;
   bool any = false;
@@ -2704,9 +2865,15 @@
 
 size_t mgn_wgrad_workspace_bytes(int njobs, const mgn_wgrad_job* jobs) {
   if (njobs < 1 || njobs > MGN_MAX_WGRAD_JOBS) return 0;
-  return (size_t)(512 + 1024 + 2 * MGN_MAX_WGRAD_JOBS) * (128 * 128 + 128) * sizeof(float);
-}
-
+  return (size_t)(512 + 1024 + 2 * MGN_MAX_WGRAD_JOBS) * (128 * 128 + 128) * sizeof(float) + (size_t)njobs * 512 * 34 * 128 * sizeof(float);
+}
+
+static int wgrad_job_narrow(const mgn_wgrad_job& j) {
+  if (j.M < 1 || j.A == nullptr || j.B == nullptr || j.dW == nullptr || !narrow_on()) return 0;
+  if (j.nja == 8 && j.lda == 128 && j.kw >= 1 && j.kw <= 32 && j.nkb == (j.kw + 15) / 16 && j.ldb >= j.kw && j.ldw >= j.kw) return 1;
+  if (j.nja == 1 && j.lda == 16 && j.nkb == 8 && j.ldb == 128 && j.kw == 128 && j.ldw >= 128) return 2;
+  return 0;
+}
 static bool wgrad_job_full(const mgn_wgrad_job& j) {
   return j.nja == 8 && j.nkb == 8 && (j.lda == 128 || j.lda == -128) && (j.ldb == 128 || j.ldb == -128) && j.kw == 128 && j.M >= 1 && getenv("MGN_NO_LDS") == nullptr;
 }
@@ -2728,12 +2895,46 @@
   }
   hipStream_t s = (hipStream_t)stream;
   size_t ws_off = 0;
+  for (int j = 0; j < njobs && precision == 0; ++j) {
+    const int kind = wgrad_job_narrow(jobs[j]);
+    if (kind == 0) continue;
+    const mgn_wgrad_job& J = jobs[j];
+    WgradNarrow N;
+    N.a_wide = kind == 1;
+    N.wide = N.a_wide ? J.A : J.B;
+    N.nar = N.a_wide ? J.B : J.A;
+    N.M = (long)J.M;
+    N.ldn = N.a_wide ? J.ldb : J.lda;
+    N.nw = N.a_wide ? J.kw : 16;
+    N.nrows_out = 16;
+    N.dW = J.dW, N.ldw = J.ldw, N.db = J.db;
+    int64_t g = (J.M + 63) / 64;
+    N.nparts = (int)(g < 1 ? 1 : (g > 512 ? 512 : g));
+    const int nwt = N.nw <= 4 ? 4 : (N.nw <= 16 ? 16 : 32);
+    const size_t need = (size_t)N.nparts * (nwt + 2) * 128 * sizeof(float);
+    if (ws_bytes < ws_off + need) return fail(1, "mgn_wgrad: workspace too small");
+    N.partial = (float*)((char*)ws + ws_off);
+    ws_off += need;
+    const unsigned rb = (unsigned)(((nwt + 2) * 128 + 63) / 64);
+    if (nwt == 4) {
+      hipLaunchKernelGGL(k_wgrad_narrow<4>, dim3(N.nparts), dim3(256), 0, s, N);
+      hipLaunchKernelGGL(k_wgrad_narrow_red<4>, dim3(rb), dim3(1024), 0, s, N);
+    } else if (nwt == 16) {
+      hipLaunchKernelGGL(k_wgrad_narrow<16>, dim3(N.nparts), dim3(256), 0, s, N);
+      hipLaunchKernelGGL(k_wgrad_narrow_red<16>, dim3(rb), dim3(1024), 0, s, N);
+    } else {
+      hipLaunchKernelGGL(k_wgrad_narrow<32>, dim3(N.nparts), dim3(256), 0, s, N);
+      hipLaunchKernelGGL(k_wgrad_narrow_red<32>, dim3(rb), dim3(1024), 0, s, N);
+    }
+    if (int rc = check_launch("mgn_wgrad/narrow")) return rc;
+  }
   for (int pass = 0; pass < 2; ++pass) {
     WgradLaunch L;
     L.njobs = 0;
     int maxb = 1;
     for (int j = 0; j < njobs; ++j) {
       if (jobs[j].nja < 1 || jobs[j].nkb < 1 || jobs[j].nja > 8 || jobs[j].nkb > 8) return fail(1, "mgn_wgrad: block counts out of range");
+      if (precision == 0 && wgrad_job_narrow(jobs[j]) != 0) continue;
       if (wgrad_job_full(jobs[j]) != (pass == 0)) continue;
       L.job[L.njobs++] = jobs[j];
       if (jobs[j].nja > maxb) maxb = jobs[j].nja;
@@ -2876,7 +3077,15 @@
       T.b[i] = blocks[i0 + i];
       if (T.b[i].src == nullptr || T.b[i].dst == nullptr || ((size_t)T.b[i].dst & 15) != 0) return fail(1, "mgn_wpack: null / misaligned block");
     }
-    hipLaunchKernelGGL(k_wpack, dim3(8, m), dim3(256), 0, s, T);
+    bool ext = false;
+    for (int i = 0; i < m; ++i) {
+      if (T.b[i].src_rows < 0 || T.b[i].src_rows > 128 || T.b[i].src_cols < 0 || T.b[i].src_cols > 128) return fail(1, "mgn_wpack: extents out of range");
+      ext = ext || T.b[i].src_rows != 0 || T.b[i].src_cols != 0;
+    }
+    if (ext)
+      hipLaunchKernelGGL(k_wpack_ext, dim3(8, m), dim3(256), 0, s, T);
+    else
+      hipLaunchKernelGGL(k_wpack, dim3(8, m), dim3(256), 0, s, T);
   }
   return check_launch("mgn_wpack");
 }
diff --git a/graph-physics_amd/csrc/mgn_x6.inc b/graph-physics_amd/csrc/mgn_x6.inc
--- a/graph-physics_amd/csrc/mgn_x6.inc
+++ b/graph-physics_amd/csrc/mgn_x6.inc
@@ -133,6 +133,33 @@
   for (int i = 0; i < 8; ++i) {
     const int f = 32 * j + 16 * (i >> 2) + 4 * g + (i & 3);
     v[i] = B.transpose ? B.src[(size_t)f * B.ld_src + o] : B.src[(size_t)o * B.ld_src + f];
+  }
+  u32x4 p1, p2, p3;
+#pragma unroll
+  for (int h = 0; h < 4; ++h) {
+    u32 q1, q2, q3;
+    split2(v[2 * h], v[2 * h + 1], q1, q2, q3);
+    p1[h] = q1, p2[h] = q2, p3[h] = q3;
+  }
+  u32x4* dst = (u32x4*)((char*)B.dst + (size_t)j * X6_QBYTES) + ob * 64 + lane;
+  dst[0] = p1;
+  dst[512] = p2;
+  dst[1024] = p3;
+}
+
+__global__ void __launch_bounds__(256) k_wpack_ext(const WpackLaunch T) {
+  const mgn_wpack_block B = T.b[blockIdx.y];
+  const int t = blockIdx.x * 256 + threadIdx.x;
+  const int lane = t & 63, ob = (t >> 6) & 7, j = t >> 9;
+  const int c = lane & 15, g = lane >> 4;
+  const int o = 16 * ob + c;
+  const int nr = B.src_rows > 0 ? B.src_rows : 128, nc = B.src_cols > 0 ? B.src_cols : 128;
+  float v[8];
+#pragma unroll
+  for (int i = 0; i < 8; ++i) {
+    const int f = 32 * j + 16 * (i >> 2) + 4 * g + (i & 3);
+    const int r = B.transpose ? f : o, cc = B.transpose ? o : f;
+    v[i] = (r < nr && cc < nc) ? B.src[(size_t)r * B.ld_src + cc] : 0.f;
   }
   u32x4 p1, p2, p3;
 #pragma unroll
@@ -412,6 +439,7 @@
 
 struct ShDyn {
   static constexpr bool ST = false;
+  static constexpr bool NARROW = false;
   static __device__ __forceinline__ int nphase(const mgn_mlp_fwd_args& a) { return a.nphase; }
   static __device__ __forceinline__ int NL(const mgn_mlp_fwd_args& a) { return a.NL; }
   static __device__ __forceinline__ int n_add(const mgn_mlp_fwd_args& a) { return a.n_add; }
@@ -424,6 +452,7 @@
 };
 struct ShEdge {
   static constexpr bool ST = true;
+  static constexpr bool NARROW = false;
   static __device__ __forceinline__ constexpr int nphase(const mgn_mlp_fwd_args&) { return 1; }
   static __device__ __forceinline__ constexpr int NL(const mgn_mlp_fwd_args&) { return 4; }
   static __device__ __forceinline__ constexpr int n_add(const mgn_mlp_fwd_args&) { return 2; }
@@ -437,6 +466,7 @@
 template <int NPOST>
 struct ShNode {
   static constexpr bool ST = true;
+  static constexpr bool NARROW = false;
   static __device__ __forceinline__ constexpr int nphase(const mgn_mlp_fwd_args&) { return 2; }
   static __device__ __forceinline__ constexpr int NL(const mgn_mlp_fwd_args&) { return 4; }
   static __device__ __forceinline__ constexpr int n_add(const mgn_mlp_fwd_args&) { return 0; }
@@ -447,6 +477,18 @@
   static __device__ __forceinline__ constexpr bool has_idx(const int32_t*) { return false; }
   static __device__ __forceinline__ constexpr bool has_addidx(const int32_t*) { return false; }
 };
+
+struct ShNarrow : ShDyn {
+  static constexpr bool NARROW = true;
+};
+__device__ __forceinline__ void ld_narrow(f32x4& b0, f32x4& b1, const float* row, int kw, int g) {
+#pragma unroll
+  for (int r = 0; r < 4; ++r) {
+    const int f0 = 4 * g + r, f1 = 16 + 4 * g + r;
+    b0[r] = (f0 < kw) ? row[f0] : 0.f;
+    b1[r] = (f1 < kw) ? row[f1] : 0.f;
+  }
+}
 
 __device__ __forceinline__ void ld2(f32x4 (&dst)[8], const float* rowp, int s, int& n) {
   dst[2 * s] = ld4(rowp + 32 * s);
@@ -561,6 +603,9 @@
   const int NPH = SH::nphase(a), NLL = SH::NL(a), NADD = SH::n_add(a), NPOST = SH::n_post(a);
   const bool HAS_RESID = SH::resid(a), HAS_SCALE = SH::scale(a), HAS_SEG = SH::seg(a);
   constexpr bool UT = SH::ST;
+  constexpr bool NRW = SH::NARROW;
+  const int KW0 = NRW ? a.kw[0] : 128, OW = NRW ? a.out_w : 128;
+  const bool K0 = NRW && KW0 < 128;
   constexpr bool UI = UT && NW != 6;
   constexpr int RING = (NW == 8) ? 6 : 3;
   constexpr int AHEAD = RING - 1;
@@ -600,7 +645,7 @@
   const int n_idx = (I0 ? 1 : 0) + (I1 ? 1 : 0) + (I2 ? 1 : 0) + (A0 ? 1 : 0) + (A1 ? 1 : 0);
 
   QStream qs;
-  qs.issued = 0, qs.total = my_tiles * 4 * G, qs.du = 0, qs.dq = 0, qs.dslot = 0, qs.cslot = 0, qs.young = 0;
+  qs.issued = 0, qs.total = my_tiles * (4 * G - (K0 ? 3 : 0)), qs.du = 0, qs.dq = 0, qs.dslot = 0, qs.cslot = 0, qs.young = 0;
   auto next_job = [&]() -> DmaQ {
     DmaQ j;
     const char* up = contig ? U0 + (size_t)qs.du * MGN_WPACK_BYTES : pick8(U0, U1, U2, U3, U4, U5, U6, U7, qs.du);
@@ -609,7 +654,7 @@
     j.on = qs.issued < qs.total;
     ++qs.issued;
     qs.dslot = (qs.dslot == RING - 1) ? 0 : qs.dslot + 1;
-    if (++qs.dq == 4) {
+    if (++qs.dq == ((K0 && qs.du == 0) ? 1 : 4)) {
       qs.dq = 0;
       qs.du = (qs.du + 1 == G) ? 0 : qs.du + 1;
     }
@@ -624,7 +669,8 @@
   for (int i = threadIdx.x; i < 5 * H; i += 64 * NW) {
     const int l = i >> 7, jx = i & 127;
     const float* bp = (l == 4) ? a.scale : pick4(a.b[0], a.b[1], a.b[2], a.b[3], l);
-    ((__attribute__((address_space(3))) float*)cst)[i] = (bp != nullptr && (l == 4 || l < NLL)) ? bp[jx] : 0.f;
+    const bool past = NRW && l == NLL - 1 && jx >= OW;
+    ((__attribute__((address_space(3))) float*)cst)[i] = (bp != nullptr && (l == 4 || l < NLL) && !past) ? bp[jx] : 0.f;
   }
   auto lds_bias = [&](f32x4 (&acc)[HB], int l) {
 #pragma unroll
@@ -660,14 +706,21 @@
   rows_of(tile, mm, valid, rid, std::false_type{});
   f32x4 nin[HB], acc[HB], pr[HB];
   u32x4 xs[4][3];
-#pragma unroll
-  for (int kb = 0; kb < HB; ++kb) nin[kb] = ld4(src0 + (long)rid[0] * H + 4 * g + 16 * kb);
+  if (K0) {
+    ld_narrow(nin[0], nin[1], src0 + (long)rid[0] * KW0, KW0, g);
+#pragma unroll
+    for (int kb = 2; kb < HB; ++kb) nin[kb] = f32x4{0.f, 0.f, 0.f, 0.f};
+  } else {
+#pragma unroll
+    for (int kb = 0; kb < HB; ++kb) nin[kb] = ld4(src0 + (long)rid[0] * H + 4 * g + 16 * kb);
+  }
   dma_drain();
   __syncthreads();
 
-  auto run_unit = [&](auto late) {
+  auto run_unit = [&](auto late, int nq = 4) {
 #pragma unroll
     for (int jq = 0; jq < 4; ++jq) {
+      if (NRW && jq >= nq) break;
       TL_STAMP(3);
       __syncthreads();
       TL_STAMP(4);
@@ -797,7 +850,9 @@
             else if (NADD > 1)
               LD2(nin, as1 + (long)rid[4] * H + 4 * g, s, n);
           }
-          if (u == GL - 1 && NLL > 1 && NPOST == 0 && (UT || has_next))
+          if (K0) {
+            if (u == GL - 1 && has_next && s == 0) ld_narrow(nin[0], nin[1], src0 + (long)ridn[0] * KW0, KW0, g);
+          } else if (u == GL - 1 && NLL > 1 && NPOST == 0 && (UT || has_next))
             LD2(nin, src0 + (long)LANDED(ridn[0]) * H + 4 * g, s, n);
         } else if (jq == 2) {
           if (UT && HAS_SEG && u == GL - 1 && s == 0) {
@@ -808,7 +863,7 @@
             n += 1;
           }
         }
-      });
+      }, (K0 && u == 0) ? 1 : 4);
     };
     if constexpr (UT) {
 #pragma unroll
@@ -849,9 +904,16 @@
         inv = 1.0f / (rms + a.eps);
         if (a.saveR != nullptr && valid && g == 0) st1(a.saveR + mm, rms);
       }
+      const bool NOUT = NRW && OW < H;
+      if (NOUT && valid) {
+#pragma unroll
+        for (int r = 0; r < 4; ++r)
+          if (4 * g + r < OW) st1(a.out + mm * OW + 4 * g + r, acc[0][r]);
+      }
       const long ro = mm * H + 4 * g;
 #pragma unroll
       for (int ib = 0; ib < HB; ++ib) {
+        if (NOUT) break;
         f32x4 y = acc[ib];
         if (HAS_SCALE) {
           const f32x4 u = y * inv;
@@ -864,7 +926,7 @@
         if (valid) st4(a.out + ro + 16 * ib, yo);
         acc[ib] = HAS_SEG ? y : yo;
       }
-      if (wvalid) qs.young += 8 + ((HAS_SCALE && a.saveU != nullptr) ? 8 : 0) + ((a.y_out != nullptr) ? 8 : 0);
+      if (wvalid && !NOUT) qs.young += 8 + ((HAS_SCALE && a.saveU != nullptr) ? 8 : 0) + ((a.y_out != nullptr) ? 8 : 0);
     }
     TL_STAMP(9);
     if (HAS_SEG) {
@@ -925,6 +987,7 @@
 }
 struct SbDyn {
   static constexpr bool ST = false;
+  static constexpr bool NARROW = false;
   static __device__ __forceinline__ int NL(const mgn_mlp_bwd_args& a) { return a.NL; }
   static __device__ __forceinline__ int n_din(const mgn_mlp_bwd_args& a) { return a.n_din; }
   static __device__ __forceinline__ bool scale(const mgn_mlp_bwd_args& a) { return a.scale != nullptr; }
@@ -932,10 +995,14 @@
 };
 struct SbEdge {
   static constexpr bool ST = true;
+  static constexpr bool NARROW = false;
   static __device__ __forceinline__ constexpr int NL(const mgn_mlp_bwd_args&) { return 4; }
   static __device__ __forceinline__ constexpr int n_din(const mgn_mlp_bwd_args&) { return 1; }
   static __device__ __forceinline__ constexpr bool scale(const mgn_mlp_bwd_args&) { return true; }
   static __device__ __forceinline__ constexpr bool din_resid(const mgn_mlp_bwd_args&) { return true; }
+};
+struct SbNarrow : SbDyn {
+  static constexpr bool NARROW = true;
 };
 __device__ __forceinline__ float ldfu(const float* p) {
   float v;
@@ -954,6 +1021,8 @@
   static_assert(!UT || (!FRONT && !SEG && ACT == MGN_ACT_RELU), "static backward shape: plain ReLU chain only");
   const int NLL = SB::NL(a), NDIN = SB::n_din(a);
   const bool HAS_SCALE = SB::scale(a), HAS_DRESID = SB::din_resid(a);
+  constexpr bool NRW = SB::NARROW;
+  const int OW = NRW ? a.out_w : 128;
   extern __shared__ __attribute__((aligned(16))) char smem[];
   lds_char* ring = (lds_char*)smem;
   lds_char* cst = ring + X6_RING * X6_QBYTES;
@@ -1040,15 +1109,22 @@
       if constexpr (UT) ld2u(dst, rowp, s, n);
       else ld2(dst, rowp, s, n);
     };
+    auto ld_dout_narrow = [&](long row) {
+#pragma unroll
+      for (int r = 0; r < 4; ++r) dz[0][r] = (4 * g + r < OW) ? src_rows[row * OW + 4 * g + r] : 0.f;
+#pragma unroll
+      for (int kb = 1; kb < HB; ++kb) dz[kb] = f32x4{0.f, 0.f, 0.f, 0.f};
+    };
     {
       const long r2 = (add_rows != nullptr) ? (add_idx ? (long)add_idx[mm] : mm) : 0;
       prms = HAS_SCALE ? ld1(a.R + mm) : 0.f;
 #pragma unroll
       for (int kb = 0; kb < HB; ++kb) {
-        dz[kb] = ld4(src_rows + mm * H + 4 * g + 16 * kb);
+        if (!NRW) dz[kb] = ld4(src_rows + mm * H + 4 * g + 16 * kb);
         pd2[kb] = (add_rows != nullptr) ? ld4(add_rows + r2 * H + 4 * g + 16 * kb) : f32x4{0.f, 0.f, 0.f, 0.f};
         pu[kb] = HAS_SCALE ? ld4(a.U + mm * H + 4 * g + 16 * kb) : f32x4{0.f, 0.f, 0.f, 0.f};
       }
+      if (NRW) ld_dout_narrow(mm);
     }
     dma_drain();
     __syncthreads();
@@ -1131,7 +1207,10 @@
       const bool top16 = d16 && (NLL - 1 >= 1 || a.precision == 3);
       {
         float* dzl = dzl_top;
-        if (dzl != nullptr && !top16) {
+        if (NRW) {
+          if (dzl != nullptr && valid) st4(dzl + mm * 16 + 4 * g, dz[0]);
+          if (dzl != nullptr && wvalid) qs.young += 1;
+        } else if (dzl != nullptr && !top16) {
           if (valid) {
 #pragma unroll
             for (int ib = 0; ib < HB; ++ib) st4(dzl + mm * H + 4 * g + 16 * ib, dz[ib]);
@@ -1262,9 +1341,13 @@
           if constexpr (UT) {
             pref_u(jq, s, n);
           } else {
-            if (jq == 0)
-              ld2(dz, src_rows + mmn * H + 4 * g, s, n);
-            else if (has_next)
+            if (jq == 0) {
+              if (NRW) {
+                if (s == 0) ld_dout_narrow(mmn);
+              } else {
+                ld2(dz, src_rows + mmn * H + 4 * g, s, n);
+              }
+            } else if (has_next)
               pref(jq, s, n);
           }
         });
@@ -1275,8 +1358,12 @@
         if (wvalid) qs.young += 8;
       }
       if (NDIN == 0 && has_next) {
-#pragma unroll
-        for (int kb = 0; kb < HB; ++kb) dz[kb] = ld4(src_rows + mmn * H + 4 * g + 16 * kb);
+        if (NRW) {
+          ld_dout_narrow(mmn);
+        } else {
+#pragma unroll
+          for (int kb = 0; kb < HB; ++kb) dz[kb] = ld4(src_rows + mmn * H + 4 * g + 16 * kb);
+        }
       }
       mm = mmn;
       valid = validn;
diff --git a/graph-physics_amd/ops.py b/graph-physics_amd/ops.py
--- a/graph-physics_amd/ops.py
+++ b/graph-physics_amd/ops.py
@@ -486,12 +486,15 @@
         _capi.check(rc, "mgn_wgrad")
 
 
-def wpack(blocks: Sequence[Tuple[int, int, bool, int]], dev):
+def wpack(blocks: Sequence[Tuple[int, ...]], dev):
     if not blocks:
         return
     arr = (_capi.WpackBlock * len(blocks))()
-    for i, (src, ld, tr, dst) in enumerate(blocks):
+    for i, blk in enumerate(blocks):
+        src, ld, tr, dst = blk[:4]
         arr[i].src, arr[i].ld_src, arr[i].transpose, arr[i].dst = src, ld, int(bool(tr)), dst
+        if len(blk) > 4:
+            arr[i].src_rows, arr[i].src_cols = blk[4], blk[5]
     with torch.cuda.device(dev):
         rc = _capi.lib().mgn_wpack(len(blocks), arr, _stream(dev))
     _capi.check(rc, "mgn_wpack")
@@ -704,11 +707,20 @@
             raise NotImplementedError(f"MLP widths (in={kin}, hidden={H}, out={out_w}) not supported by the MI355X engine")
         dev = x.device
         kp, op = pad16(kin), pad16(out_w)
+        narrow = (H == 128 and X6_ENABLED and M > 0 and act == 0 and NL <= 4 and (kin < H or out_w < H)
+                  and (kin == H or (kin <= 32 and NL >= 3)) and (out_w == H or (out_w <= 16 and not has_norm))
+                  and not (_matrix_precision == "bf16" and out_w != H))
+        nmode = _os.environ.get("MGN_X6_NARROW", "1")
+        narrow = narrow and nmode != "0" and (kin == H or nmode == "2")
+        if narrow:
+            kp, op0 = kin, out_w
+        else:
+            op0 = op
         W0 = Ws[0]
         if kp != kin:
             W0 = torch.nn.functional.pad(W0, (0, kp - kin))
         Wl, bl = Ws[-1], bs[-1]
-        if op != out_w:
+        if op0 != out_w:
             Wl = torch.nn.functional.pad(Wl, (0, 0, 0, op - out_w))
             bl = torch.nn.functional.pad(bl, (0, op - out_w))
         Wk = [W0] + Ws[1:-1] + [Wl]
@@ -722,7 +734,9 @@
         y = torch.empty(M, out_w, **f)
         x6 = H == 128 and out_w == H and X6_ENABLED and M > 0 and act != 2
         mode = "generic"
-        if x6 and kin < H and 3 <= NL <= 4:
+        if narrow:
+            mode = "narrow"
+        elif x6 and kin < H and 3 <= NL <= 4:
             mode = "enc"
         elif x6 and kin == H and NL <= 4:
             mode = "full"
@@ -732,7 +746,12 @@
         R = torch.empty(M, **f) if (need and has_norm) else None
         Ms = [torch.empty(M, 4, dtype=torch.int32, device=dev) for _ in range(NL - 1)] if (need and packed and act == 0) else None
         Zs = [torch.empty(M, H, **f) for _ in range(NL - 1)] if (need and act != 0) else None
-        if mode == "enc":
+        if mode == "narrow":
+            pk = torch.empty(NL * _capi.WPACK_BYTES, dtype=torch.uint8, device=dev)
+            units = [pk.data_ptr() + u * _capi.WPACK_BYTES for u in range(NL)]
+            wpack([_wpack_block(Wk[l], False, units[l], H) for l in range(NL)], dev)
+            mlp_fwd(M, H, [(x, None, kin)], Wk, bk, scale, out_w, None, y, None, saveH, U, R, wpk=units, saveM=Ms)
+        elif mode == "enc":
             h1 = saveH[0] if need else torch.empty(M, H, **f)
             mlp_fwd(M, H, [(x, None, kin)], [Wk[0]], [bk[0]], None, H, None, h1, Zs[0] if Zs else None, out_relu=True, act=act,
                     saveM=[Ms[0]] if Ms else None)
@@ -749,10 +768,10 @@
             mlp_fwd(M, H, [(x, None, H)], Wk, bk, scale, out_w, None, y, None, saveH, U, R, wpk=units, saveM=Ms, saveZ=Zs, act=act)
         else:
             mlp_fwd(M, H, [(x, None, kin)], Wk, bk, scale, out_w, None, y, None, saveH, U, R, act=act, saveZ=Zs, precision=prec)
-        ctx.meta = (NL, H, kin, out_w, has_norm, kp != kin, op != out_w, act, mode)
+        ctx.meta = (NL, H, kin, out_w, has_norm, kp != kin, op0 != out_w, act, mode)
         ctx.prec, ctx.Wk_rounded = prec, (Wk if prec else None)
         ctx.save_for_backward(x, *Ws, *([scale] if has_norm else []))
-        ctx.pads = (W0 if kp != kin else None, Wl if op != out_w else None)
+        ctx.pads = (W0 if kp != kin else None, Wl if op0 != out_w else None)
         ctx.saved_acts = (saveH, U, R, Ms, Zs)
         return y
 
@@ -786,11 +805,11 @@
             raise NotImplementedError("input gradient of a ragged-width MLP input is not needed by the path")
         if want_dx:
             dx = mk(M, H, **f)
-        if mode in ("enc", "full") and M > 0:
+        if mode in ("enc", "full", "narrow") and M > 0:
             tr = [Wk[l] for l in range(NL - 1, 0, -1)] + ([Wk[0]] if want_dx else [])
             pk = torch.empty(len(tr) * _capi.WPACK_BYTES, dtype=torch.uint8, device=dev)
             units = [pk.data_ptr() + u * _capi.WPACK_BYTES for u in range(len(tr))]
-            wpack([(w.data_ptr(), H, True, units[u]) for u, w in enumerate(tr)], dev)
+            wpack([_wpack_block(w, True, units[u], H) for u, w in enumerate(tr)], dev)
             din = [(None, None, dx)] if want_dx else []
             mlp_bwd(M, H, NL, dy, None, None, out_w, U, R, scale, saveH, [None] * NL, dZ, din, [None] * NL, dscale,
                     wpk=units, Ms=Ms, Zs=Zs, act=act)
@@ -820,6 +839,11 @@
             grads.append(dscale)
         ctx.saved_acts = None
         return (dx, None, None, *grads)
+
+
+def _wpack_block(W: torch.Tensor, transpose: bool, dst: int, H: int):
+    r, c = W.shape
+    return (W.data_ptr(), c, transpose, dst, r if r < H else 0, c if c < H else 0)
 
 
 def _split_block(q, spec: BlockSpec):
diff --git a/include/mgn_hip.h b/include/mgn_hip.h
--- a/include/mgn_hip.h
+++ b/include/mgn_hip.h
@@ -173,6 +173,7 @@
 typedef struct {
   const float* src; void* dst;
   int ld_src, transpose;
+  int src_rows, src_cols;
 } mgn_wpack_block;
 int mgn_wpack(int n, const mgn_wpack_block* blocks, void* stream);
 
```

Result: no change. 82.76 steps/s, median of 2 (+0.2%).
